# chrischoy/DeepGlobalRegistration

Hardware: AMD Instinct MI355X
Metric: pair registrations/sec (FCGF x2 + 1-NN + 6-D inlier net + gate + weighted Procrustes + SE(3) refinement) (higher is better)
Workload: dtype f32 results via 2 x f16 split operands (3 f16 MFMA products per MAC, f32 accumulate); k = 1 convs, kNN re-evaluation and registration in exact f32, SVD in f64

## Files before the change

### deepglobalregistration_amd/csrc/conv.hip

```cpp
#include <stdlib.h>

#include <map>

#include "dgr_internal.h"
#include <algorithm>
#include "hash.h"
#include "split.h"

typedef float f32x16 __attribute__((ext_vector_type(16)));
typedef float f32x4 __attribute__((ext_vector_type(4)));
typedef _Float16 f16x4 __attribute__((ext_vector_type(4)));
typedef int i32x4 __attribute__((ext_vector_type(4)));
typedef unsigned int u32x2 __attribute__((ext_vector_type(2)));
typedef unsigned int u32x4 __attribute__((ext_vector_type(4)));

struct ConvKArgs {
  const float *in;
  float *out;
  float *y;
  const float *shift;
  const float *w;
  const int32_t *pair_in, *pair_out, *tile_ptr, *rule_ptr, *n_rows_dev;
  const int4 *tile_desc;
  int in_ld, out_ld, in_relu, y_ld;
// ... 104 lines not shown
    float *dst = As + (q & 1) * TM * LDA;
#pragma unroll
    for (int i = 0; i < NCH; ++i) {
      const int ch = tid + i * THREADS;
      f32x4 v = G[i];
      if (a.in_relu) { v.x = fmaxf(v.x, 0.f); v.y = fmaxf(v.y, 0.f); v.z = fmaxf(v.z, 0.f); v.w = fmaxf(v.w, 0.f); }
      const bool ok = (g_ok >> i) & 1u;
      v.x = ok ? v.x : 0.f;
      v.y = ok ? v.y : 0.f;
      v.z = ok ? v.z : 0.f;
      v.w = ok ? v.w : 0.f;
      *reinterpret_cast<f32x4 *>(dst + (ch / C4K) * LDA + (ch % C4K) * 4) = v;
    }
  };

  {
    const int i0 = load_idx(0), i1 = load_idx(1), i2 = load_idx(2);
    if (tid < TM) { idxbuf[tid] = i0; idxbuf[TM + tid] = i1; idxbuf[2 * TM + tid] = i2; }
  }
  int next_pub = 3;
  int idx_reg = load_idx(3);
  int k, pstart, count;
  locate(0, k, pstart, count);
  f32x4 b[RING][NB];
  {
    const f32x4 *w0 = reinterpret_cast<const f32x4 *>(a.w) + ((int64_t)k * S * NBLK + wn * NB) * 64 + lane;
#pragma unroll
    for (int r = 0; r < RING - 1; ++r)
      if (r < S) {
#pragma unroll
        for (int j = 0; j < NB; ++j) b[r][j] = w0[((int64_t)r * NBLK + j) * 64];
      }
  }
  __syncthreads();
  gather(0);
  land(0);
  if (1 < NQ) gather(1);
  __syncthreads();

  f32x16 acc[MB][NB];
  for (int q = 0; q < NQ; ++q) {
    const int h = q % PPT;
    if (q + 1 < NQ) land(q + 1);
    if (q + 2 < NQ) gather(q + 2);
    if ((q + 3) / PPT >= next_pub && next_pub < n_my) {
      if (tid < TM) idxbuf[(next_pub & 3) * TM + tid] = idx_reg;
      ++next_pub;
      idx_reg = load_idx(next_pub);
    }
    if (h == 0) {
#pragma unroll
      for (int i = 0; i < MB; ++i)
#pragma unroll
        for (int j = 0; j < NB; ++j)
#pragma unroll
          for (int e = 0; e < 16; ++e) acc[i][j][e] = 0.f;
    }
    const f32x4 *wk = reinterpret_cast<const f32x4 *>(a.w) + ((int64_t)k * S * NBLK + wn * NB) * 64 + lane;
    const float *arow = As + (q & 1) * TM * LDA + (32 * wm * MB + (lane & 31)) * LDA + 4 * (lane >> 5);
    const int s0 = h * SK;
#pragma unroll
    for (int s = 0; s < SK; ++s) {
      if (s0 + s + RING - 1 < S) {
#pragma unroll
        for (int j = 0; j < NB; ++j) b[(s + RING - 1) % RING][j] = wk[((int64_t)(s0 + s + RING - 1) * NBLK + j) * 64];
      }
      __builtin_amdgcn_sched_barrier(0);
      f32x4 av[MB];
#pragma unroll
      for (int i = 0; i < MB; ++i) av[i] = *reinterpret_cast<const f32x4 *>(arow + i * 32 * LDA + s * 8);
#pragma unroll
      for (int c = 0; c < 4; ++c)
#pragma unroll
        for (int i = 0; i < MB; ++i)
#pragma unroll
          for (int j = 0; j < NB; ++j)
            acc[i][j] = __builtin_amdgcn_mfma_f32_32x32x2f32(b[s % RING][j][c], av[i][c], acc[i][j], 0, 0, 0);
    }
    if (h == PPT - 1) {
      const int pst = pstart, cnt = count;
      const int i_next = q / PPT + 1;
      if (i_next < n_my) {
        locate(i_next, k, pstart, count);
        const f32x4 *w1 = reinterpret_cast<const f32x4 *>(a.w) + ((int64_t)k * S * NBLK + wn * NB) * 64 + lane;
#pragma unroll
        for (int r = 0; r < RING - 1; ++r)
          if (r < S) {
#pragma unroll
            for (int j = 0; j < NB; ++j) b[r][j] = w1[((int64_t)r * NBLK + j) * 64];
          }
      }
#pragma unroll
      for (int i = 0; i < MB; ++i) {
        const int r = 32 * (wm * MB + i) + (lane & 31);
        if (identity && a.l2_normalize) {
          float ss = 0.f;
#pragma unroll
          for (int g = 0; g < 4; ++g)
#pragma unroll
            for (int u = 0; u < 4; ++u) {
              const int col = 8 * g + 4 * (lane >> 5) + u;
              float v = acc[i][0][4 * g + u] + ((a.shift && col < a.cout) ? a.shift[col] : 0.f);
              if (col >= a.cout) v = 0.f;
              acc[i][0][4 * g + u] = v;
              ss += v * v;
            }
          ss += __shfl_xor(ss, 32, 64);
          const float den = sqrtf(ss) + 1e-8f;
#pragma unroll
          for (int e = 0; e < 16; ++e) acc[i][0][e] = acc[i][0][e] / den;
        }
        if (r < cnt) {
          float *dst = identity ? a.out + (int64_t)(pst + r) * a.out_ld : a.y + (int64_t)(pst + r) * a.y_ld;
#pragma unroll
          for (int j = 0; j < NB; ++j) {
#pragma unroll
            for (int g = 0; g < 4; ++g) {
              const int col = 32 * (wn * NB + j) + 8 * g + 4 * (lane >> 5);
              f32x4 v = {acc[i][j][4 * g], acc[i][j][4 * g + 1], acc[i][j][4 * g + 2], acc[i][j][4 * g + 3]};
              if (identity) {
                if (col + 3 < a.cout && (a.out_ld & 3) == 0) {
                  if (a.shift && !a.l2_normalize) v += *reinterpret_cast<const f32x4 *>(a.shift + col);
                  *reinterpret_cast<f32x4 *>(dst + col) = v;
                } else {
#pragma unroll
                  for (int u = 0; u < 4; ++u)
                    if (col + u < a.cout) dst[col + u] = v[u] + ((a.shift && !a.l2_normalize) ? a.shift[col + u] : 0.f);
                }
              } else if (col < a.cout) {
                *reinterpret_cast<f32x4 *>(dst + col) = v;
              }
            }
          }
        }
      }
    }
    __syncthreads();
  }
}

template <int CP, int WM, int WN, int MB, int NB, bool VEC>
static int launch_v2(const ConvKArgs &ka, int64_t tile_bound, int num_cus, hipStream_t stream) {
  constexpr int THREADS = 64 * WM * WN;
  constexpr int CKL = conv_phase_width(CP, MB * NB);
  const size_t lds_bytes = (size_t)2 * DGR_TILE_M * (CKL + 4) * sizeof(float) + 4 * DGR_TILE_M * sizeof(int);
  static int per_cu = 0;
  if (per_cu == 0) {
    DGR_HIP_CHECK(hipFuncSetAttribute((const void *)sparse_conv_mfma_v2<CP, WM, WN, MB, NB, VEC>,
                                      hipFuncAttributeMaxDynamicSharedMemorySize, 160 * 1024));
    int n = 0;
    DGR_HIP_CHECK(hipOccupancyMaxActiveBlocksPerMultiprocessor(&n, sparse_conv_mfma_v2<CP, WM, WN, MB, NB, VEC>,
                                                               THREADS, lds_bytes));
    per_cu = n < 1 ? 1 : (n > 2048 / THREADS ? 2048 / THREADS : n);
  }
  int64_t grid = (int64_t)num_cus * per_cu;
  if (tile_bound < grid) grid = tile_bound;
  grid = (grid + 7) / 8 * 8;
  if (grid < 8) grid = 8;
  sparse_conv_mfma_v2<CP, WM, WN, MB, NB, VEC><<<(int)grid, THREADS, lds_bytes, stream>>>(ka);
  DGR_LAUNCH_CHECK();
  return DGR_OK;
}

template <int CP, int NBLK>
__global__ void __launch_bounds__(256) identity_conv_kernel(ConvKArgs a) {
  constexpr int S = CP / 8;
  const int lane = threadIdx.x & 63;
  const int n_rows = *a.n_rows_dev;
  const int n_tiles = (n_rows + 31) >> 5;
  const int wave_id = (int)((blockIdx.x * blockDim.x + threadIdx.x) >> 6), n_waves = (int)((gridDim.x * blockDim.x) >> 6);
  f32x4 w[S][NBLK];
  {
    const f32x4 *wp = reinterpret_cast<const f32x4 *>(a.w) + lane;
#pragma unroll
    for (int s = 0; s < S; ++s)
#pragma unroll
      for (int j = 0; j < NBLK; ++j) w[s][j] = wp[(s * NBLK + j) * 64];
  }
  const int relu_lo = a.in_relu ? 0 : (int)0x80000000;
  auto request = [&](int t, f32x4 (&x)[S]) {
    const int64_t row = min((int64_t)t * 32 + (lane & 31), (int64_t)n_rows - 1);
    const float *src = a.in + row * a.in_ld + 4 * (lane >> 5);
#pragma unroll
    for (int s = 0; s < S; ++s) x[s] = *reinterpret_cast<const f32x4 *>(src + 8 * s);
  };
  f32x4 xa[S], xb[S];
  auto tile = [&](int t, f32x4 (&x)[S]) {
    f32x16 acc[NBLK];
#pragma unroll
    for (int j = 0; j < NBLK; ++j)
#pragma unroll
      for (int e = 0; e < 16; ++e) acc[j][e] = 0.f;
#pragma unroll
    for (int s = 0; s < S; ++s) {
      i32x4 v = __builtin_bit_cast(i32x4, x[s]);
      v.x = max(v.x, relu_lo); v.y = max(v.y, relu_lo); v.z = max(v.z, relu_lo); v.w = max(v.w, relu_lo);
      const f32x4 xv = __builtin_bit_cast(f32x4, v);
#pragma unroll
      for (int c = 0; c < 4; ++c)
#pragma unroll
        for (int j = 0; j < NBLK; ++j) acc[j] = __builtin_amdgcn_mfma_f32_32x32x2f32(w[s][j][c], xv[c], acc[j], 0, 0, 0);
    }
    const int64_t row = (int64_t)t * 32 + (lane & 31);
    if (a.l2_normalize) {
      float ss = 0.f;
#pragma unroll
      for (int g = 0; g < 4; ++g)
#pragma unroll
        for (int u = 0; u < 4; ++u) {
          const int col = 8 * g + 4 * (lane >> 5) + u;
          float v = acc[0][4 * g + u] + ((a.shift && col < a.cout) ? a.shift[col] : 0.f);
          if (col >= a.cout) v = 0.f;
          acc[0][4 * g + u] = v;
          ss += v * v;
        }
      ss += __shfl_xor(ss, 32, 64);
      const float den = sqrtf(ss) + 1e-8f;
#pragma unroll
      for (int e = 0; e < 16; ++e) acc[0][e] = acc[0][e] / den;
    }
    if (row < n_rows) {
      float *dst = a.out + row * a.out_ld;
#pragma unroll
      for (int j = 0; j < NBLK; ++j)
#pragma unroll
        for (int g = 0; g < 4; ++g) {
          const int col = 32 * j + 8 * g + 4 * (lane >> 5);
          f32x4 v = {acc[j][4 * g], acc[j][4 * g + 1], acc[j][4 * g + 2], acc[j][4 * g + 3]};
          if (col + 3 < a.cout && (a.out_ld & 3) == 0) {
            if (a.shift && !a.l2_normalize) v += *reinterpret_cast<const f32x4 *>(a.shift + col);
            *reinterpret_cast<f32x4 *>(dst + col) = v;
          } else {
#pragma unroll
            for (int u = 0; u < 4; ++u)
              if (col + u < a.cout) dst[col + u] = v[u] + ((a.shift && !a.l2_normalize) ? a.shift[col + u] : 0.f);
          }
        }
    }
  };
  int t = wave_id;
  if (t < n_tiles) request(t, xa);
  for (; t < n_tiles; t += 2 * n_waves) {
    const int t1 = t + n_waves;
    if (t1 < n_tiles) request(t1, xb);
    tile(t, xa);
    if (t1 < n_tiles) {
      if (t1 + n_waves < n_tiles) request(t1 + n_waves, xa);
      tile(t1, xb);
    }
  }
}

template <int CP, int NBLK>
static int launch_identity(const ConvKArgs &ka, int64_t rows_cap, int num_cus, hipStream_t stream) {
  int64_t blocks = std::min<int64_t>((int64_t)num_cus * 4, std::max<int64_t>(1, dgr_ceil_div(rows_cap, 32 * 4 * 2)));
  identity_conv_kernel<CP, NBLK><<<(int)blocks, 256, 0, stream>>>(ka);
  DGR_LAUNCH_CHECK();
  return DGR_OK;
}

int dgr_conv_launch(const DgrConvLaunch &a, int num_cus, hipStream_t stream, const char **kernel_name) {
  ConvKArgs ka;
  ka.in = a.in; ka.out = a.out; ka.w = a.w; ka.y = a.y; ka.shift = a.shift; ka.y_ld = a.cout;
  ka.pair_in = a.pair_in; ka.pair_out = a.pair_out; ka.tile_ptr = a.tile_ptr; ka.rule_ptr = a.rule_ptr;
  ka.n_rows_dev = a.n_rows_dev; ka.tile_desc = a.tile_desc;
  ka.in_ld = a.in_ld; ka.out_ld = a.out_ld; ka.in_relu = a.in_relu;
  ka.cin = a.cin; ka.cin_pad = a.cin_pad; ka.cout = a.cout; ka.K = a.K;
  ka.l2_normalize = a.l2_normalize;
  DGR_REQUIRE(!a.l2_normalize || (a.pair_in == nullptr && a.cout <= 32 && a.cout_pad == 32),
              "fused l2 normalisation needs an identity map and Cout <= 32 (got %d)", a.cout);
  DGR_REQUIRE(a.cin_pad % 8 == 0 && a.cin_pad >= a.cin && a.cin_pad <= 256, "bad cin_pad %d", a.cin_pad);
  const int64_t tile_bound = a.tile_bound > 0 ? a.tile_bound : (int64_t)num_cus * 4;
  const bool vec = ((a.cin | a.in_ld) & 3) == 0;
  if (a.pair_in == nullptr && vec && a.cin == a.cin_pad && a.tile_bound > 0) {
#define DGR_ID(CPV, NBV)                                                                          \
  if (a.cin_pad == CPV && a.cout_pad == 32 * NBV) {                                               \
    if (kernel_name) *kernel_name = "identity_conv_kernel<" #CPV ", " #NBV ">";                   \
    return launch_identity<CPV, NBV>(ka, a.tile_bound * DGR_TILE_M, num_cus, stream);             \
  }
    DGR_ID(64, 1) DGR_ID(64, 2) DGR_ID(96, 2)
#undef DGR_ID
  }
#define DGR_V2(CPV, WMV, WNV, MBV, NBV)                                                                        \
  if (a.cin_pad == CPV) {                                                                                       \
    if (kernel_name)                                                                                            \
      *kernel_name = vec ? "sparse_conv_mfma_v2<" #CPV ", " #WMV ", " #WNV ", " #MBV ", " #NBV ", true>"        \
                         : "sparse_conv_mfma_v2<" #CPV ", " #WMV ", " #WNV ", " #MBV ", " #NBV ", false>";      \
    return vec ? launch_v2<CPV, WMV, WNV, MBV, NBV, true>(ka, tile_bound, num_cus, stream)                     \
               : launch_v2<CPV, WMV, WNV, MBV, NBV, false>(ka, tile_bound, num_cus, stream);                   \
  }
  switch (a.cout_pad) {
    case 32: DGR_V2(8, 2, 1, 1, 1) DGR_V2(32, 2, 1, 1, 1) DGR_V2(64, 2, 1, 1, 1) break;
    case 64: DGR_V2(32, 2, 2, 1, 1) DGR_V2(64, 2, 2, 1, 1) DGR_V2(96, 2, 2, 1, 1) DGR_V2(128, 2, 2, 1, 1)
             DGR_V2(256, 2, 2, 1, 1) break;
    case 128: DGR_V2(64, 1, 4, 2, 1) DGR_V2(128, 1, 4, 2, 1) DGR_V2(256, 1, 4, 2, 1) break;
    case 256: DGR_V2(128, 1, 4, 2, 2) DGR_V2(256, 1, 4, 2, 2) break;
    default: break;
  }
#undef DGR_V2
  dgr_set_error("sparse conv: no kernel instantiation for Cin (padded) %d -> Cout (padded) %d", a.cin_pad, a.cout_pad);
  return DGR_EINVAL;
}

template <int LPR, bool SPLIT>
__global__ void __launch_bounds__(256)
    reduce_rows_kernel(const float *__restrict__ y, int y_ld, const int32_t *__restrict__ ptr,
                       const int32_t *__restrict__ pos, const int32_t *n_dev, float *__restrict__ out, int out_ld,
                       const float *__restrict__ shift, const float *__restrict__ res, int res_ld, int res_relu,
                       unsigned char *__restrict__ planes, float *__restrict__ scale_out, int out_relu) {
  constexpr int ROWS = 256 / LPR;
  const int n = *n_dev;
  const int sub = threadIdx.x / LPR, c = (threadIdx.x % LPR) * 4;
  for (int64_t row = (int64_t)blockIdx.x * ROWS + sub; row < n; row += (int64_t)gridDim.x * ROWS) {
    f32x4 acc = shift ? *reinterpret_cast<const f32x4 *>(shift + c) : f32x4{0.f, 0.f, 0.f, 0.f};
    if (res) {
      f32x4 r = *reinterpret_cast<const f32x4 *>(res + row * res_ld + c);
      if (res_relu) { r.x = fmaxf(r.x, 0.f); r.y = fmaxf(r.y, 0.f); r.z = fmaxf(r.z, 0.f); r.w = fmaxf(r.w, 0.f); }
      acc += r;
    }
    int j = ptr[row];
    const int end = ptr[row + 1];
    for (; j + 8 <= end; j += 8) {
      int p[8];
#pragma unroll
      for (int u = 0; u < 8; ++u) p[u] = pos[j + u];
      f32x4 v[8];
#pragma unroll
      for (int u = 0; u < 8; ++u) v[u] = dgr_y_load<LPR == 64>(y + (int64_t)p[u] * y_ld + c);
#pragma unroll
      for (int u = 0; u < 8; ++u) acc += v[u];
    }
    for (; j + 4 <= end; j += 4) {
      const int p0 = pos[j], p1 = pos[j + 1], p2 = pos[j + 2], p3 = pos[j + 3];
      const f32x4 v0 = dgr_y_load<LPR == 64>(y + (int64_t)p0 * y_ld + c);
      const f32x4 v1 = dgr_y_load<LPR == 64>(y + (int64_t)p1 * y_ld + c);
      const f32x4 v2 = dgr_y_load<LPR == 64>(y + (int64_t)p2 * y_ld + c);
      const f32x4 v3 = dgr_y_load<LPR == 64>(y + (int64_t)p3 * y_ld + c);
      acc += v0; acc += v1; acc += v2; acc += v3;
    }
    for (; j < end; ++j) acc += dgr_y_load<LPR == 64>(y + (int64_t)pos[j] * y_ld + c);
    if (!SPLIT || out) *reinterpret_cast<f32x4 *>(out + row * out_ld + c) = acc;
    if constexpr (SPLIT) {
      const int lo = out_relu ? 0 : (int)0x80000000;
      const i32x4 ab = __builtin_bit_cast(i32x4, acc);
      int xb[4];
      uint32_t mx = 0;
#pragma unroll
      for (int u = 0; u < 4; ++u) {
        xb[u] = max(ab[u], lo);
        mx = max(mx, (uint32_t)xb[u] & 0x7fffffffu);
      }
#pragma unroll
      for (int d = LPR / 2; d >= 1; d >>= 1) mx = max(mx, (uint32_t)__shfl_xor((int)mx, d, 64));
      const float sx = dgr_row_scale_of(mx);
      f16x4 h, m;
#pragma unroll
      for (int u = 0; u < 4; ++u) {
        _Float16 hh, mm;
        dgr_split2(__builtin_bit_cast(float, xb[u]), sx, hh, mm);
        h[u] = hh; m[u] = mm;
      }
      const bool odd = threadIdx.x & 1;
      const u32x2 hb = __builtin_bit_cast(u32x2, h), mb = __builtin_bit_cast(u32x2, m);
      const u32x2 give = odd ? hb : mb;
      u32x2 got;
      got.x = (uint32_t)__shfl_xor((int)give.x, 1, 64);
      got.y = (uint32_t)__shfl_xor((int)give.y, 1, 64);
      const u32x4 st = odd ? u32x4{got.x, got.y, mb.x, mb.y} : u32x4{hb.x, hb.y, got.x, got.y};
      unsigned char *dst = planes + row * (LPR * 16);
      *reinterpret_cast<u32x4 *>(dst + dgr_split_row_offset(c & ~7, odd ? 1 : 0)) = st;
      if (c == 0) scale_out[row] = sx;
    }
  }
}

int dgr_reduce_rows(const float *y, int cout, const int32_t *ptr, const int32_t *pos, const int32_t *n_dev,
                    int64_t n_cap, float *out, int out_ld, const float *shift, const float *res, int res_ld,
                    int res_relu, hipStream_t stream, const DgrSplitRows *split, int out_relu) {
  DGR_REQUIRE((out_ld & 3) == 0 && (res == nullptr || (res_ld & 3) == 0), "reduce_rows: row strides must be x4");
  DGR_REQUIRE(out || split, "reduce_rows: no output");
  DGR_REQUIRE(!split || (split->planes && split->scale && split->channels == cout && cout % 64 == 0),
              "reduce_rows: split rows need planes, scales and the layer's width (a multiple of 64)");
  const int lpr = cout / 4;
  const int64_t want = std::max<int64_t>(1, dgr_ceil_div(n_cap, 256 / lpr));
#define DGR_RR1(L, SP)                                                                                         \
  do {                                                                                                         \
    static int resident = 0;                                                                                   \
    if (resident == 0) {                                                                                       \
      int per_cu = 0, dev = 0, cus = 0;                                                                        \
      DGR_HIP_CHECK(hipOccupancyMaxActiveBlocksPerMultiprocessor(&per_cu, reduce_rows_kernel<L, SP>, 256, 0)); \
      DGR_HIP_CHECK(hipGetDevice(&dev));                                                                       \
      DGR_HIP_CHECK(hipDeviceGetAttribute(&cus, hipDeviceAttributeMultiprocessorCount, dev));                  \
      resident = (per_cu < 1 ? 1 : per_cu) * (cus < 1 ? 1 : cus);                                              \
    }                                                                                                          \
    const int64_t blocks = want > resident ? (int64_t)resident * std::min<int64_t>(4, want / resident) : want; \
    reduce_rows_kernel<L, SP><<<(int)blocks, 256, 0, stream>>>(y, cout, ptr, pos, n_dev, out, out_ld, shift,   \
                                                               res, res_ld, res_relu, split ? split->planes : nullptr, \
                                                               split ? split->scale : nullptr, out_relu);      \
  } while (0)
#define DGR_RR(L)                       \
  do {                                  \
    if (split) DGR_RR1(L, true);        \
    else DGR_RR1(L, false);             \
  } while (0)
  switch (cout) {
    case 32: DGR_RR1(8, false); break;
    case 64: DGR_RR(16); break;
    case 128: DGR_RR(32); break;
    case 256: DGR_RR(64); break;
    default:
      dgr_set_error("reduce_rows: unsupported width %d", cout);
      return DGR_EINVAL;
  }
#undef DGR_RR1
#undef DGR_RR
  DGR_LAUNCH_CHECK();
  return DGR_OK;
}

__global__ void __launch_bounds__(256)
    conv_small_cin_kernel(const float *__restrict__ in, int in_ld, int in_relu, int cin,
                          const float *__restrict__ w, const float *__restrict__ shift,
                          const int32_t *__restrict__ out_ptr, const int32_t *__restrict__ out_pos,
                          const int32_t *__restrict__ pair_in, const uint16_t *__restrict__ pair_k,
                          const int32_t *n_out_dev, float *__restrict__ out, int out_ld) {
  const int n = *n_out_dev;
  const int co = threadIdx.x & 31;
  for (int64_t o = (int64_t)blockIdx.x * 8 + (threadIdx.x >> 5); o < n; o += (int64_t)gridDim.x * 8) {
    float acc = shift ? shift[co] : 0.f;
    const int end = out_ptr[o + 1];
    int j = out_ptr[o];
    for (; j + 8 <= end; j += 8) {
      int pos[8], row[8], kk[8];
#pragma unroll
      for (int u = 0; u < 8; ++u) pos[u] = out_pos[j + u];
#pragma unroll
      for (int u = 0; u < 8; ++u) { row[u] = pair_in[pos[u]]; kk[u] = pair_k[pos[u]]; }
      float y[8];
#pragma unroll
      for (int u = 0; u < 8; ++u) {
        const float *wk = w + (int64_t)kk[u] * 256;
        float t = 0.f;
        for (int ci = 0; ci < cin; ++ci) {
          float x = in[(int64_t)row[u] * in_ld + ci];
          if (in_relu) x = fmaxf(x, 0.f);
          t = fmaf(x, wk[(32 * (ci >> 2) + co) * 4 + (ci & 3)], t);
        }
        y[u] = t;
      }
#pragma unroll
      for (int u = 0; u < 8; ++u) acc += y[u];
    }
    for (; j < end; ++j) {
      const int pos = out_pos[j];
      const int row = pair_in[pos];
      const float *wk = w + (int64_t)pair_k[pos] * 256;
      float y = 0.f;
      for (int ci = 0; ci < cin; ++ci) {
        float x = in[(int64_t)row * in_ld + ci];
        if (in_relu) x = fmaxf(x, 0.f);
        y = fmaf(x, wk[(32 * (ci >> 2) + co) * 4 + (ci & 3)], y);
      }
      acc += y;
    }
    out[o * out_ld + co] = acc;
  }
}

template <int CIN>
__global__ void __launch_bounds__(256)
    conv_small_cin_row_kernel(const float *__restrict__ in, int in_ld, int in_relu, const float *__restrict__ w,
                              const float *__restrict__ shift, const int32_t *__restrict__ out_ptr,
                              const int32_t *__restrict__ out_pos, const int32_t *__restrict__ pair_in,
                              const uint16_t *__restrict__ pair_k, const int32_t *n_out_dev, float *__restrict__ out,
                              int out_ld) {
  const int64_t o = (int64_t)blockIdx.x * blockDim.x + threadIdx.x;
  if (o >= *n_out_dev) return;
  float acc[32];
#pragma unroll
  for (int co = 0; co < 32; ++co) acc[co] = shift ? shift[co] : 0.f;
  const int end = out_ptr[o + 1];
  for (int j = out_ptr[o]; j < end; ++j) {
    const int pos = out_pos[j];
    const int row = pair_in[pos];
    const f32x4 *wk = reinterpret_cast<const f32x4 *>(w + (int64_t)pair_k[pos] * 256);
    float x[CIN];
#pragma unroll
    for (int ci = 0; ci < CIN; ++ci) {
      x[ci] = in[(int64_t)row * in_ld + ci];
      if (in_relu) x[ci] = fmaxf(x[ci], 0.f);
    }
#pragma unroll
    for (int co = 0; co < 32; ++co) {
      const f32x4 w0 = wk[co];
      float t = 0.f;
#pragma unroll
      for (int ci = 0; ci < (CIN < 4 ? CIN : 4); ++ci) t = fmaf(x[ci], w0[ci], t);
      if constexpr (CIN > 4) {
        const f32x4 w1 = wk[32 + co];
#pragma unroll
        for (int ci = 4; ci < CIN; ++ci) t = fmaf(x[ci], w1[ci - 4], t);
      }
      acc[co] += t;
    }
  }
  f32x4 *dst = reinterpret_cast<f32x4 *>(out + o * out_ld);
#pragma unroll
  for (int q = 0; q < 8; ++q) dst[q] = f32x4{acc[4 * q], acc[4 * q + 1], acc[4 * q + 2], acc[4 * q + 3]};
}

__global__ void __launch_bounds__(256)
    conv_cin6_quad_kernel(const float *__restrict__ in, int in_ld, int in_relu, const float *__restrict__ wq,
                          const float *__restrict__ shift, const int32_t *__restrict__ out_ptr,
                          const int32_t *__restrict__ out_pos, const int32_t *__restrict__ pair_in,
                          const uint16_t *__restrict__ pair_k, const int32_t *n_out_dev, float *__restrict__ out,
                          int out_ld) {
  const int64_t t = (int64_t)blockIdx.x * blockDim.x + threadIdx.x;
  const int64_t o = t >> 2;
  const int q = (int)(t & 3);
  if (o >= *n_out_dev) return;
  float acc[8];
#pragma unroll
  for (int e = 0; e < 8; ++e) acc[e] = shift ? shift[8 * q + e] : 0.f;
  const int end = out_ptr[o + 1];
  for (int j = out_ptr[o]; j < end; ++j) {
    const int pos = out_pos[j];
    const int row = pair_in[pos];
    const f32x4 *wk = reinterpret_cast<const f32x4 *>(wq + (int64_t)pair_k[pos] * 192) + q;
    float x[6];
#pragma unroll
    for (int ci = 0; ci < 6; ++ci) {
      x[ci] = in[(int64_t)row * in_ld + ci];
      if (in_relu) x[ci] = fmaxf(x[ci], 0.f);
    }
    float tt[8];
#pragma unroll
    for (int e = 0; e < 8; ++e) tt[e] = 0.f;
#pragma unroll
    for (int i = 0; i < 12; ++i) {
      const f32x4 wv = wk[4 * i];
#pragma unroll
      for (int e = 0; e < 4; ++e) tt[4 * (i & 1) + e] = fmaf(x[i >> 1], wv[e], tt[4 * (i & 1) + e]);
    }
#pragma unroll
    for (int e = 0; e < 8; ++e) acc[e] += tt[e];
  }
  f32x4 *dst = reinterpret_cast<f32x4 *>(out + o * out_ld + 8 * q);
  dst[0] = f32x4{acc[0], acc[1], acc[2], acc[3]};
  dst[1] = f32x4{acc[4], acc[5], acc[6], acc[7]};
}

int dgr_conv_small_cin(const float *in, int in_ld, int in_relu, int cin, const float *w_tiled, const float *w_quad,
                       const float *shift, const DgrKernelMap &km, const int32_t *n_out_dev, int64_t n_out_cap, float *out,
                       int out_ld, hipStream_t stream) {
  DGR_REQUIRE(cin >= 1 && cin <= 8, "small-Cin conv: cin=%d", cin);
  if ((out_ld & 3) == 0 && cin == 6 && w_quad) {
    conv_cin6_quad_kernel<<<(int)dgr_ceil_div(n_out_cap * 4, 256), 256, 0, stream>>>(
        in, in_ld, in_relu, w_quad, shift, km.out_ptr, km.out_pos, km.pair_in, km.pair_k, n_out_dev, out, out_ld);
    DGR_LAUNCH_CHECK();
    return DGR_OK;
  }
  if ((out_ld & 3) == 0 && (cin == 6 || cin == 1)) {
    const int rb = (int)dgr_ceil_div(n_out_cap, 256);
    if (cin == 6)
      conv_small_cin_row_kernel<6><<<rb, 256, 0, stream>>>(in, in_ld, in_relu, w_tiled, shift, km.out_ptr, km.out_pos, km.pair_in,
                                                         km.pair_k, n_out_dev, out, out_ld);
    else
      conv_small_cin_row_kernel<1><<<rb, 256, 0, stream>>>(in, in_ld, in_relu, w_tiled, shift, km.out_ptr, km.out_pos, km.pair_in,
                                                         km.pair_k, n_out_dev, out, out_ld);
    DGR_LAUNCH_CHECK();
    return DGR_OK;
  }
  int64_t blocks = dgr_ceil_div(n_out_cap, 8);
  if (blocks > 16384) blocks = 16384;
  conv_small_cin_kernel<<<(int)blocks, 256, 0, stream>>>(in, in_ld, in_relu, cin, w_tiled, shift, km.out_ptr,
                                                          km.out_pos, km.pair_in, km.pair_k, n_out_dev, out, out_ld);
  DGR_LAUNCH_CHECK();
  return DGR_OK;
}

__global__ void __launch_bounds__(256)
    conv1_probe_kernel(const int32_t *__restrict__ coords, const int32_t *n_dev, const int32_t *__restrict__ table,
                       uint32_t mask, int ks, const float *__restrict__ in, int in_ld, int cin,
                       const float *__restrict__ w, const float *__restrict__ shift, float *__restrict__ out,
                       int out_ld, int32_t *pair_count, const int32_t *skip_flag, uint32_t *__restrict__ out_amax) {
  if (skip_flag && *skip_flag) return;
  const int n = *n_dev;
  const int lane = threadIdx.x & 63;
  const int co = lane & 31;
  const int K = ks * ks * ks, half = ks >> 1;
  const int64_t wave_id = ((int64_t)blockIdx.x * blockDim.x + threadIdx.x) >> 6;
  const int64_t n_waves = ((int64_t)gridDim.x * blockDim.x) >> 6;
  int pairs = 0;
  for (int64_t o = wave_id; o < n; o += n_waves) {
    const int32_t b = coords[o * 4], x = coords[o * 4 + 1], y = coords[o * 4 + 2], z = coords[o * 4 + 3];
    float acc = shift ? shift[co] : 0.f;
    for (int k0 = 0; k0 < K; k0 += 64) {
      const int k = k0 + lane;
      int hit = -1;
      if (k < K) {
        int32_t q[4] = {b, x + (k % ks) - half, y + ((k / ks) % ks) - half, z + (k / (ks * ks)) - half};
        hit = dgr_lookup<4>(table, mask, coords, q);
      }
      float xv[8];
      const int64_t hrow = (int64_t)max(hit, 0) * in_ld;
#pragma unroll
      for (int ci = 0; ci < 8; ++ci) {
        xv[ci] = 0.f;
        if (ci < cin) xv[ci] = in[hrow + ci];
      }
      unsigned long long live = __ballot(hit >= 0);
      pairs += __popcll(live);
      while (live) {
        const int src = __ffsll((long long)live) - 1;
        live &= live - 1;
        float t = 0.f;
#pragma unroll
        for (int ci = 0; ci < 8; ++ci) {
          if (ci < cin) {
            const float xs = __builtin_bit_cast(float, __builtin_amdgcn_readlane(__builtin_bit_cast(int, xv[ci]), src));
            const float wv = w[(int64_t)(k0 + src) * 256 + (32 * (ci >> 2) + co) * 4 + (ci & 3)];
            t = fmaf(xs, wv, t);
          }
        }
        acc += t;
      }
    }
    if (lane < 32) out[o * out_ld + co] = acc;
    if (out_amax) {
      uint32_t mx = __builtin_bit_cast(uint32_t, acc) & 0x7fffffffu;
#pragma unroll
      for (int d = 16; d >= 1; d >>= 1) mx = max(mx, (uint32_t)__shfl_xor((int)mx, d, 64));
      if (lane == 0) atomicMax(out_amax + o, mx);
    }
  }
  if (lane == 0 && pair_count) atomicAdd(pair_count, pairs);
}

constexpr int GRID_MAXB = 64;
struct DgrGridMeta {
  int32_t ok, bad;
  long long total;
  int32_t mn[GRID_MAXB][3], mx[GRID_MAXB][3], dim[GRID_MAXB][3];
  long long base[GRID_MAXB];
};

__global__ void grid_init_kernel(DgrGridMeta *m, int32_t *pair_count) {
  const int b = threadIdx.x;
  if (b == 0) { m->ok = 0; m->bad = 0; m->total = 0; if (pair_count) *pair_count = 0; }
  if (b < GRID_MAXB) {
    for (int d = 0; d < 3; ++d) { m->mn[b][d] = INT32_MAX; m->mx[b][d] = INT32_MIN; m->dim[b][d] = 0; }
    m->base[b] = 0;
  }
}

__global__ void __launch_bounds__(256)
    grid_bbox_kernel(const int32_t *__restrict__ coords, const int32_t *n_dev, DgrGridMeta *m) {
  __shared__ int32_t red[6][256 / 64];
  __shared__ int32_t b0s, mixed;
  const int n = *n_dev;
  const int64_t o = (int64_t)blockIdx.x * 256 + threadIdx.x;
  if ((int64_t)blockIdx.x * 256 >= n) return;
  const bool live = o < n;
  const int4 c = live ? *reinterpret_cast<const int4 *>(coords + o * 4) : make_int4(0, 0, 0, 0);
  if (threadIdx.x == 0) { b0s = c.x; mixed = 0; }
  __syncthreads();
  if (live && c.x != b0s) mixed = 1;
  if (live && (c.x < 0 || c.x >= GRID_MAXB)) m->bad = 1;
  __syncthreads();
  auto wave_minmax = [&](bool mine, int32_t (&v)[6]) {
    v[0] = mine ? c.y : INT32_MAX; v[1] = mine ? c.z : INT32_MAX; v[2] = mine ? c.w : INT32_MAX;
    v[3] = mine ? c.y : INT32_MIN; v[4] = mine ? c.z : INT32_MIN; v[5] = mine ? c.w : INT32_MIN;
#pragma unroll
    for (int s = 32; s >= 1; s >>= 1) {
#pragma unroll
      for (int d = 0; d < 3; ++d) {
        v[d] = min(v[d], __shfl_xor(v[d], s, 64));
        v[3 + d] = max(v[3 + d], __shfl_xor(v[3 + d], s, 64));
      }
    }
  };
  int32_t v[6];
  if (mixed) {
    const bool ok = live && c.x >= 0 && c.x < GRID_MAXB;
    unsigned long long todo = __ballot(ok);
    while (todo) {
      const int leader = __ffsll((long long)todo) - 1;
      const int b = __shfl(c.x, leader, 64);
      const bool mine = ok && c.x == b;
      wave_minmax(mine, v);
      if ((int)(threadIdx.x & 63) == leader) {
#pragma unroll
        for (int d = 0; d < 3; ++d) { atomicMin(&m->mn[b][d], v[d]); atomicMax(&m->mx[b][d], v[3 + d]); }
      }
      todo &= ~__ballot(mine);
    }
    return;
  }
  wave_minmax(live, v);
  if ((threadIdx.x & 63) == 0)
    for (int d = 0; d < 6; ++d) red[d][threadIdx.x >> 6] = v[d];
  __syncthreads();
  if (threadIdx.x < 6) {
    const int d = threadIdx.x;
    int32_t r = red[d][0];
    for (int w = 1; w < 4; ++w) r = d < 3 ? min(r, red[d][w]) : max(r, red[d][w]);
    const int b = b0s;
    if (b >= 0 && b < GRID_MAXB) {
      if (d < 3) atomicMin(&m->mn[b][d], r); else atomicMax(&m->mx[b][d - 3], r);
    }
  }
}

__global__ void grid_layout_kernel(DgrGridMeta *m, int pad, long long cap) {
  static_assert(GRID_MAXB == 64, "one lane per batch element");
  const int b = threadIdx.x;
  long long vol = 0;
  if (m->mx[b][0] >= m->mn[b][0]) {
    vol = 1;
    for (int d = 0; d < 3; ++d) {
      const long long e = (long long)m->mx[b][d] - m->mn[b][d] + 1 + 2 * pad;
      m->dim[b][d] = (int32_t)(e < (1ll << 30) ? e : (1ll << 30));
      vol = (vol <= cap && e <= cap) ? vol * e : cap + 1;
    }
  }
  long long incl = vol;
#pragma unroll
  for (int s = 1; s < 64; s <<= 1) {
    const long long up = __shfl_up(incl, s, 64);
    if (b >= s) incl += up;
  }
  m->base[b] = incl - vol;
  const long long total = __shfl(incl, 63, 64);
  if (b == 0) {
    m->total = total <= cap ? total : cap + 1;
    m->ok = (!m->bad && total <= cap) ? 1 : 0;
  }
}

__global__ void grid_clear_kernel(const DgrGridMeta *m, int32_t *__restrict__ cells) {
  if (!m->ok) return;
  const long long total = m->total;
  for (long long i = ((long long)blockIdx.x * blockDim.x + threadIdx.x) * 4; i < total; i += (long long)gridDim.x * blockDim.x * 4)
    *reinterpret_cast<int4 *>(cells + i) = make_int4(-1, -1, -1, -1);
}

__device__ __forceinline__ long long grid_cell(const DgrGridMeta *m, int b, int x, int y, int z, int pad) {
  const long long dx = m->dim[b][0], dy = m->dim[b][1];
  return m->base[b] + ((long long)(z - m->mn[b][2] + pad) * dy + (y - m->mn[b][1] + pad)) * dx + (x - m->mn[b][0] + pad);
}

constexpr uint32_t GRID_EMPTY = 0xffffffffu;
__global__ void grid_fill_kernel(const int32_t *__restrict__ coords, const int32_t *n_dev, const DgrGridMeta *m, int pad,
                                 int32_t *__restrict__ cells, const float *__restrict__ values, int values_ld) {
  if (!m->ok) return;
  const int64_t o = (int64_t)blockIdx.x * blockDim.x + threadIdx.x;
  if (o >= *n_dev) return;
  const int4 c = *reinterpret_cast<const int4 *>(coords + o * 4);
  cells[grid_cell(m, c.x, c.y, c.z, c.w, pad)] = values ? __builtin_bit_cast(int32_t, values[o * values_ld]) : (int32_t)o;
}

constexpr int C1_MAXK = 343;
__global__ void __launch_bounds__(256)
    conv1_grid_kernel(const int32_t *__restrict__ coords, const int32_t *n_dev, const DgrGridMeta *__restrict__ m,
                      const int32_t *__restrict__ cells, int ks, const float *__restrict__ in, int in_ld, int cin,
                      const float *__restrict__ w, const float *__restrict__ shift, float *__restrict__ out,
                      int out_ld, int32_t *pair_count, uint32_t *__restrict__ out_amax) {
  __shared__ int2 lists[256 / 64][2][C1_MAXK + 1];
  if (!m->ok) return;
  const int n = *n_dev;
  const int lane = threadIdx.x & 63, wv = threadIdx.x >> 6;
  const int half = ks >> 1, ks2 = ks * ks;
  const int ky = lane % ks, kz = lane / ks;
  const int vsel = lane >> 5, co = lane & 31;
  const unsigned long long below = (1ull << lane) - 1ull;
  const int64_t wave_id = ((int64_t)blockIdx.x * blockDim.x + threadIdx.x) >> 6;
  const int64_t n_waves = ((int64_t)gridDim.x * blockDim.x) >> 6;
  int pairs = 0;
  for (int64_t o0 = wave_id * 2; o0 < n; o0 += n_waves * 2) {
    int nh[2] = {0, 0};
#pragma unroll
    for (int v = 0; v < 2; ++v) {
      const int64_t o = o0 + v;
      if (o >= n) break;
      const int4 c = *reinterpret_cast<const int4 *>(coords + o * 4);
      int hit[7];
#pragma unroll
      for (int kx = 0; kx < 7; ++kx) hit[kx] = -1;
      if (lane < ks2) {
        const long long c0 = grid_cell(m, c.x, c.y - half, c.z + ky - half, c.w + kz - half, half);
#pragma unroll
        for (int kx = 0; kx < 7; ++kx)
          if (kx < ks) hit[kx] = cells[c0 + kx];
      }
      unsigned long long mk[7];
      int before = 0;
#pragma unroll
      for (int kx = 0; kx < 7; ++kx) {
        mk[kx] = __ballot(hit[kx] >= 0);
        before += __popcll(mk[kx] & below);
        nh[v] += __popcll(mk[kx]);
      }
      int r = before;
#pragma unroll
      for (int kx = 0; kx < 7; ++kx)
        if (hit[kx] >= 0) lists[wv][v][r++] = make_int2(kx + ks * lane, hit[kx]);
    }
    __builtin_amdgcn_fence(__ATOMIC_RELEASE, "wavefront");
    __builtin_amdgcn_wave_barrier();
    __builtin_amdgcn_fence(__ATOMIC_ACQUIRE, "wavefront");
    pairs += nh[0] + nh[1];
    const int my_n = vsel ? nh[1] : nh[0];
    const int trips = max(nh[0], nh[1]);
    float acc = shift ? shift[co] : 0.f;
    for (int r0 = 0; r0 < trips; r0 += 8) {
      int2 e[8];
      float t[8];
#pragma unroll
      for (int u = 0; u < 8; ++u) {
        e[u] = (r0 + u < my_n) ? lists[wv][vsel][r0 + u] : make_int2(0, 0);
        t[u] = 0.f;
      }
      for (int ci = 0; ci < cin; ++ci) {
        float xs[8], ws[8];
        const int wofs = (32 * (ci >> 2) + co) * 4 + (ci & 3);
#pragma unroll
        for (int u = 0; u < 8; ++u) {
          xs[u] = in[(int64_t)e[u].y * in_ld + ci];
          ws[u] = w[(int64_t)e[u].x * 256 + wofs];
        }
#pragma unroll
        for (int u = 0; u < 8; ++u) t[u] = fmaf(xs[u], ws[u], t[u]);
      }
#pragma unroll
      for (int u = 0; u < 8; ++u) acc = (r0 + u < my_n) ? acc + t[u] : acc;
    }
    const int64_t o = o0 + vsel;
    if (o < n) out[o * out_ld + co] = acc;
    if (out_amax) {
      uint32_t mx = o < n ? (__builtin_bit_cast(uint32_t, acc) & 0x7fffffffu) : 0u;
#pragma unroll
      for (int d = 16; d >= 1; d >>= 1) mx = max(mx, (uint32_t)__shfl_xor((int)mx, d, 64));
      if (co == 0 && o < n) atomicMax(out_amax + o, mx);
    }
    __builtin_amdgcn_fence(__ATOMIC_RELEASE, "wavefront");
    __builtin_amdgcn_wave_barrier();
  }
  if (lane == 0 && pair_count) atomicAdd(pair_count, pairs);
}

template <int KS>
__global__ void __launch_bounds__(256)
    conv1_grid_mfma(const int32_t *__restrict__ coords, const int32_t *n_dev, const DgrGridMeta *__restrict__ m,
                    const int32_t *__restrict__ cells, const float *__restrict__ wt, const float *__restrict__ shift,
                    float *__restrict__ out, int out_ld, int32_t *pair_count, uint32_t *__restrict__ out_amax) {
  constexpr int KS2 = KS * KS, HALF = KS / 2;
  constexpr int RS = (KS2 + 3) / 4 * 4;
  constexpr int LDG = RS + 1;
// ... 181 lines not shown
```

### deepglobalregistration_amd/csrc/conv_wide.hip

```cpp
#include <stdlib.h>

#include <type_traits>

#include "dgr_internal.h"
#include "split.h"

typedef _Float16 f16x8 __attribute__((ext_vector_type(8)));
typedef float f32x16 __attribute__((ext_vector_type(16)));
typedef float f32x4 __attribute__((ext_vector_type(4)));

struct ConvWideArgs {
  const unsigned char *planes;
  const float *row_scale;
  float *y;
  const uint4 *wb;
  int64_t piece_stride;
  const int32_t *pair_in, *tile_ptr;
  int cout, K;
  float w_unscale;
  unsigned long long *clk;
};

#define DGR_LDS_PTR(off) ((__attribute__((address_space(3))) void *)(lds + (off)))
#define DGR_GLOBAL_PTR(p) ((const __attribute__((address_space(1))) void *)(p))

template <int N>
__device__ __forceinline__ void dgr_wait_vmcnt() {
  static_assert(N >= 0 && N < 64, "vmcnt is a 6-bit counter");
  asm volatile("s_waitcnt vmcnt(%0)" ::"n"(N) : "memory");
}
__device__ __forceinline__ void dgr_phase_barrier() {
  asm volatile("s_waitcnt lgkmcnt(0)\n\ts_barrier" ::: "memory");
}

__host__ __device__ constexpr int dgr_wide_passes(int h, int npass, int nsp) {
  return h < nsp ? npass / nsp + (h < npass % nsp ? 1 : 0) : 0;
}
__host__ __device__ constexpr int dgr_wide_pass_base(int h, int npass, int nsp) {
  int b = 0;
  for (int i = 0; i < h; ++i) b += dgr_wide_passes(i, npass, nsp);
  return b;
}

template <int CP, int NB, int WM>
__global__ void __launch_bounds__(512, 1) sparse_conv_wide_f16x2(ConvWideArgs a, const int4 *__restrict__ tdesc) {
  constexpr int NCW = 4;
  constexpr int NP = 2, MB = 2 / WM, WN = NCW / WM, PW = 4, TM = 64, CK = 64, SK = CK / 16;
  static_assert(WM == 1 || WM == 2, "row split of the compute waves");
  static_assert(TM == DGR_TILE_M && CP % CK == 0, "shape");
  constexpr int PPT = CP / CK, S = CP / 16, NBLK = NB * WN, COUT = 32 * NBLK;
  static_assert(PPT == 1 || PPT == 2 || PPT == 4, "a round of NSET phases is a whole number of tiles");
  constexpr int ROWB = 4 * CP;
  constexpr int NBUF = 3;
  constexpr int NSET = 4;
  constexpr int LEAD = NSET + 2;
  constexpr int BUFB = TM * 256;
  constexpr int RING = 16;
  constexpr int AH_I = 8, AH_S = 4;
  static_assert(RING >= 2 * AH_I && AH_I > LEAD && AH_S >= 3 && AH_S < AH_I, "ring distances");
  constexpr int WD = NB >= 2 ? 2 : 4;
  static_assert(SK % WD == 0, "the weight ring turns a whole number of times per phase (static register indexing)");
  constexpr int LDS_ST = COUT + 4;
  constexpr int NSTG = PPT == 1 ? 2 : 1;
  constexpr int HB = PPT / 2;
  constexpr int RPH = TM / PPT;
  constexpr int PD = 2;
  constexpr int PTH = 64 * (PW - PD);
  constexpr int CPR = COUT / 4;
  constexpr int RPP = PTH / CPR;
  constexpr int NPS = RPH / RPP;
  static_assert(RPH % RPP == 0, "store passes");
  constexpr int OFF_STAGE = NBUF * BUFB;
  constexpr int OFF_IDX = OFF_STAGE + NSTG * TM * LDS_ST * 4;
  constexpr int OFF_SC = OFF_IDX + RING * TM * 4;
  constexpr int LDS_BYTES = OFF_SC + RING * TM * 4;
  static_assert(LDS_BYTES <= 160 * 1024, "LDS budget");
  __shared__ __attribute__((aligned(16))) unsigned char lds[LDS_BYTES];

  const int tid = threadIdx.x;
  const int lane = tid & 63;
  const int wave = __builtin_amdgcn_readfirstlane(tid >> 6);
  if (a.clk && tid == 0) atomicMin(a.clk, (unsigned long long)wall_clock64());
  const int T = a.tile_ptr[a.K];
  const int per = (T + 7) >> 3;
  const int xcd = blockIdx.x & 7;
  const int t_end = min(T, (xcd + 1) * per);
  const int nj = gridDim.x >> 3;
  const int t_first = xcd * per + (blockIdx.x >> 3);
  if (t_first >= t_end) return;
  const int n_my = (t_end - t_first + nj - 1) / nj;
  const int n_loop = n_my + 2;
  auto desc = [&](int i) -> int4 { return tdesc[t_first + min(max(i, 0), n_my - 1) * nj]; };
  auto stage_of = [&](int t) -> float * {
    return reinterpret_cast<float *>(lds + OFF_STAGE) + (NSTG == 2 ? (t & 1) : 0) * TM * LDS_ST;
  };

  if (wave >= NCW) {
    const int pw = wave - NCW;
    if (pw < PD) {
      constexpr int RW = TM / PD, NI = RW / 4;
      f32x4 G[NSET][NI];
      const unsigned char *rb[NI];
      auto row_bases = [&](int i) {
        const int *idx = reinterpret_cast<const int *>(lds + OFF_IDX + (i & (RING - 1)) * TM * 4);
#pragma unroll
        for (int jj = 0; jj < NI; ++jj) {
          const int r = RW * pw + 4 * jj + (lane >> 4);
          rb[jj] = a.planes + (int64_t)idx[r] * ROWB + 16 * ((lane & 15) ^ (r & 15));
        }
      };
      auto request = [&](int p, f32x4 *Gs) {
        if (p % PPT == 0) row_bases(p / PPT);
#pragma unroll
        for (int jj = 0; jj < NI; ++jj) Gs[jj] = *reinterpret_cast<const f32x4 *>(rb[jj] + (p % PPT) * 256);
      };
      auto land = [&](int p, const f32x4 *Gs) {
        unsigned char *dst = lds + (p % NBUF) * BUFB + (NI * pw) * 1024 + lane * 16;
#pragma unroll
        for (int jj = 0; jj < NI; ++jj) *reinterpret_cast<f32x4 *>(dst + jj * 1024) = Gs[jj];
      };
      int *ring_i = reinterpret_cast<int *>(lds + OFF_IDX);
      float *ring_s = reinterpret_cast<float *>(lds + OFF_SC);
      auto load_idx = [&](int i) -> int {
        const int4 d = desc(i);
        return a.pair_in[d.y + min(lane, d.z - 1)];
      };
#pragma unroll
      for (int i = 0; i < AH_I - 1; ++i) ring_i[i * TM + lane] = load_idx(i);
#pragma unroll
      for (int i = 0; i < AH_S - 1; ++i) ring_s[i * TM + lane] = a.row_scale[ring_i[i * TM + lane]];
      int idx_reg = load_idx(AH_I - 1);
      float sc_reg = a.row_scale[ring_i[(AH_S - 1) * TM + lane]];
      auto rings = [&](int t) {
        ring_i[((t + AH_I - 1) & (RING - 1)) * TM + lane] = idx_reg;
        ring_s[((t + AH_S - 1) & (RING - 1)) * TM + lane] = sc_reg;
        idx_reg = load_idx(t + AH_I);
        sc_reg = a.row_scale[ring_i[((t + AH_S) & (RING - 1)) * TM + lane]];
      };
      dgr_phase_barrier();
#pragma unroll
      for (int j = 0; j < NSET; ++j) request(j, G[j]);
      land(0, G[0]); request(NSET, G[0]);
      land(1, G[1]); request(NSET + 1, G[1]);
      dgr_phase_barrier();
      auto phase = [&](int q, f32x4 *Gs) {
        if (q % PPT == 0) rings(q / PPT);
        land(q + 2, Gs);
        request(q + LEAD, Gs);
        dgr_phase_barrier();
      };
      for (int q = 0; q < n_loop * PPT; q += NSET) {
        phase(q, G[2]);
        if (q + 1 < n_loop * PPT) phase(q + 1, G[3]);
        if (q + 2 < n_loop * PPT) phase(q + 2, G[0]);
        if (q + 3 < n_loop * PPT) phase(q + 3, G[1]);
      }
      return;
    }
    const int ptid = tid - 64 * (NCW + PD);
    auto store_rows = [&](int u, int r0) {
      if (u < 0 || u >= n_my) return;
      const int4 d = desc(u);
      const float *sc = reinterpret_cast<const float *>(lds + OFF_SC + (u & (RING - 1)) * TM * 4);
      const float *st = stage_of(u);
      const int c4 = (ptid % CPR) * 4;
      f32x4 v[NPS];
#pragma unroll
      for (int i = 0; i < NPS; ++i) {
        const int r = r0 + i * RPP + ptid / CPR;
        v[i] = *reinterpret_cast<const f32x4 *>(st + r * LDS_ST + c4);
        v[i] *= dgr_inv_pow2(sc[r]) * a.w_unscale;
      }
#pragma unroll
      for (int i = 0; i < NPS; ++i) {
        const int r = r0 + i * RPP + ptid / CPR;
        if (r < d.z) __builtin_nontemporal_store(v[i], reinterpret_cast<f32x4 *>(a.y + (int64_t)(d.y + r) * COUT + c4));
      }
    };
    dgr_phase_barrier();
    dgr_phase_barrier();
    auto sphase = [&](int t, auto hc) {
      constexpr int h = decltype(hc)::value;
      if constexpr (h == 0) store_rows(t - 2, (PPT - 1) * RPH);
      else store_rows(t - 1, (h - 1) * RPH);
      dgr_phase_barrier();
    };
    for (int t = 0; t < n_loop; ++t) {
      sphase(t, std::integral_constant<int, 0>());
      if constexpr (PPT > 1) sphase(t, std::integral_constant<int, 1>());
      if constexpr (PPT > 2) {
        sphase(t, std::integral_constant<int, 2>());
        sphase(t, std::integral_constant<int, 3>());
      }
    }
    if (a.clk && lane == 0) {
      dgr_wait_vmcnt<0>();
      atomicMax(a.clk + 1, (unsigned long long)wall_clock64());
    }
    return;
  }

  const int wn = wave % WN, wm = wave / WN;
  int4 dc = desc(0), dn = desc(1);
  uint4 w[WD][NB][NP];
  auto wload = [&](int k, int s, uint4 (*ws)[NP]) {
    const uint4 *p = a.wb + ((int64_t)(k * S + s) * NBLK + wn * NB) * 64 + lane;
#pragma unroll
    for (int j = 0; j < NB; ++j)
#pragma unroll
      for (int pc = 0; pc < NP; ++pc) ws[j][pc] = p[(int64_t)pc * a.piece_stride + j * 64];
  };
#pragma unroll
  for (int g = 0; g < WD - 1; ++g) wload(dc.x, g % S, w[g]);
  dgr_phase_barrier();
  dgr_phase_barrier();
  uint4 op[2][MB][NP];
  const int lofs0 = (32 * MB * wm + (lane & 31)) * 256 + 16 * ((lane >> 5) ^ (lane & 15));
  auto oload = [&](int b, int s, uint4 (*o)[NP]) {
    const unsigned char *p = lds + b * BUFB + (lofs0 ^ (32 * s));
    const unsigned char *pm = lds + b * BUFB + (lofs0 ^ (32 * s) ^ 128);
#pragma unroll
    for (int i = 0; i < MB; ++i) {
      o[i][0] = *reinterpret_cast<const uint4 *>(p + i * 32 * 256);
      o[i][1] = *reinterpret_cast<const uint4 *>(pm + i * 32 * 256);
    }
  };
  oload(0, 0, op[0]);
  int buf = 0;
  constexpr int NPC = (4 * NB + SK - 1) / SK;
  auto stage_pieces = [&](float *st, const f32x16 (&ac)[MB][NB], int i, int s) {
    float *dst = st + (32 * (MB * wm + i) + (lane & 31)) * LDS_ST;
#pragma unroll
    for (int u = 0; u < NPC; ++u) {
      const int wq = s * NPC + u, j = wq / 4, g = wq % 4;
      if (wq < 4 * NB) {
        const int col = 32 * (wn * NB + j) + 8 * g + 4 * (lane >> 5);
        *reinterpret_cast<f32x4 *>(dst + col) = f32x4{ac[i][j][4 * g], ac[i][j][4 * g + 1], ac[i][j][4 * g + 2], ac[i][j][4 * g + 3]};
      }
    }
  };
  auto ctile = [&](int t, f32x16 (&ac)[MB][NB], const f32x16 (&ad)[MB][NB]) {
    const bool stage_prev = t >= 1 && t <= n_my;
    float *st = stage_of(t - 1);
#pragma unroll
    for (int h = 0; h < PPT; ++h) {
      if (h == 0) {
#pragma unroll
        for (int i = 0; i < MB; ++i)
#pragma unroll
          for (int j = 0; j < NB; ++j)
#pragma unroll
            for (int e = 0; e < 16; ++e) ac[i][j][e] = 0.f;
      }
      const int nbuf = buf == NBUF - 1 ? 0 : buf + 1;
      const int s0 = h * SK;
#pragma unroll
      for (int s = 0; s < SK; ++s) {
        {
          const int sg = s0 + s + WD - 1;
          wload(sg < S ? dc.x : dn.x, sg < S ? sg : sg - S, w[(s + WD - 1) % WD]);
        }
        if (s + 1 < SK) oload(buf, s + 1, op[(s + 1) & 1]);
        else oload(nbuf, 0, op[0]);
        __builtin_amdgcn_sched_barrier(0);
        uint4 (*wc)[NP] = w[s % WD];
        uint4 (*oc)[NP] = op[s & 1];
#define DGR_WIDE_TERM(WP, OP)                                                                                         \
  _Pragma("unroll") for (int i = 0; i < MB; ++i) _Pragma("unroll") for (int j = 0; j < NB; ++j)                       \
      ac[i][j] = __builtin_amdgcn_mfma_f32_32x32x16_f16(__builtin_bit_cast(f16x8, wc[j][WP]),                          \
                                                        __builtin_bit_cast(f16x8, oc[i][OP]), ac[i][j], 0, 0, 0);
        DGR_WIDE_TERM(1, 0)
        DGR_WIDE_TERM(0, 1)
        DGR_WIDE_TERM(0, 0)
#undef DGR_WIDE_TERM
        if (stage_prev) {
          if (h == 0) stage_pieces(st, ad, 0, s);
          if constexpr (MB > 1) {
            if (h == HB) stage_pieces(st, ad, 1, s);
          }
        }
      }
      if (h == PPT - 1) {
        dc = dn;
        dn = desc(t + 2);
      }
      buf = nbuf;
      dgr_phase_barrier();
    }
  };
  f32x16 accA[MB][NB], accB[MB][NB];
  for (int t = 0; t < n_loop; t += 2) {
    ctile(t, accA, accB);
    if (t + 1 < n_loop) ctile(t + 1, accB, accA);
  }
  if (a.clk && lane == 0) atomicMax(a.clk + 1, (unsigned long long)wall_clock64());
}

template <int CP, int NB, int WM>
static int launch_wide(const ConvWideArgs &ka, const int4 *tile_desc, int64_t tile_bound, int num_cus, hipStream_t stream) {
  int64_t grid = num_cus;
  if (tile_bound < grid) grid = tile_bound;
  grid = (grid + 7) / 8 * 8;
  if (grid < 8) grid = 8;
  sparse_conv_wide_f16x2<CP, NB, WM><<<(int)grid, 512, 0, stream>>>(ka, tile_desc);
  DGR_LAUNCH_CHECK();
  return DGR_OK;
}

bool dgr_conv_wide_supported(int cin_pad, int cin, int cout) {
  if (cin != cin_pad) return false;
  return (cout == 64 && cin == 64) || (cout == 128 && (cin == 64 || cin == 128 || cin == 256)) ||
         (cout == 256 && (cin == 128 || cin == 256));
}

int dgr_conv_wide_launch(const DgrConvLaunch &a, const DgrSplitRows &in, const void *wb, int64_t piece_stride,
                         float w_unscale, int num_cus, hipStream_t stream, const char **kernel_name) {
  DGR_REQUIRE(a.pair_in && wb && in.planes && in.scale && dgr_conv_wide_supported(a.cin_pad, a.cin, a.cout),
              "wide conv: unsupported layer (Cin %d, Cout %d) or no split input rows", a.cin, a.cout);
  DGR_REQUIRE(in.channels == a.cin, "wide conv: the split rows have %d channels, the layer %d", in.channels, a.cin);
  DGR_REQUIRE(a.y, "wide conv: no product-row buffer");
  ConvWideArgs ka;
  ka.planes = in.planes; ka.row_scale = in.scale; ka.y = a.y;
  ka.wb = static_cast<const uint4 *>(wb); ka.piece_stride = piece_stride;
  ka.pair_in = a.pair_in; ka.tile_ptr = a.tile_ptr; ka.cout = a.cout; ka.K = a.K; ka.w_unscale = w_unscale;
  ka.clk = a.clk;
  const int64_t tile_bound = a.tile_bound > 0 ? a.tile_bound : (int64_t)num_cus * 4;
#define DGR_WIDE(CPV, NBV, WMV)                                                                 \
  do {                                                                                          \
    if (kernel_name) *kernel_name = "sparse_conv_wide_f16x2<" #CPV ", " #NBV ", " #WMV ">";     \
    return launch_wide<CPV, NBV, WMV>(ka, a.tile_desc, tile_bound, num_cus, stream);            \
  } while (0)
  if (a.cout == 64 && a.cin == 64) DGR_WIDE(64, 1, 2);
  if (a.cout == 128 && a.cin == 64) DGR_WIDE(64, 1, 1);
  if (a.cout == 128 && a.cin == 128) DGR_WIDE(128, 1, 1);
  if (a.cout == 128 && a.cin == 256) DGR_WIDE(256, 1, 1);
  if (a.cout == 256 && a.cin == 128) DGR_WIDE(128, 2, 1);
  if (a.cout == 256 && a.cin == 256) DGR_WIDE(256, 2, 1);
#undef DGR_WIDE
  dgr_set_error("wide conv: no kernel for Cin %d, Cout %d", a.cin, a.cout);
  return DGR_EINVAL;
}

typedef int i32x4 __attribute__((ext_vector_type(4)));
typedef _Float16 f16x4 __attribute__((ext_vector_type(4)));

template <int LPR, bool SPLIT>
__global__ void __launch_bounds__(256) row_scale_kernel(const float *__restrict__ in, int in_ld, int cin, int relu,
                                                        const int32_t *__restrict__ n_dev, float *__restrict__ out,
                                                        unsigned char *__restrict__ planes, uint32_t *__restrict__ amax_out) {
  constexpr int RPW = 64 / LPR;
  const int lane = threadIdx.x & 63;
  const int sub = lane / LPR, l = lane % LPR;
  const int n = *n_dev;
  const int relu_lo = relu ? 0 : (int)0x80000000;
  const int64_t stride = (int64_t)gridDim.x * 4 * RPW;
  for (int64_t r0 = ((int64_t)blockIdx.x * 4 + (threadIdx.x >> 6)) * RPW; r0 < n; r0 += stride) {
    const int64_t r = r0 + sub;
    uint32_t mx = 0;
    if (r < n) {
      const float *row = in + r * in_ld;
      for (int c = l * 4; c < cin; c += LPR * 4) {
        const i32x4 v = __builtin_bit_cast(i32x4, *reinterpret_cast<const f32x4 *>(row + c));
#pragma unroll
        for (int u = 0; u < 4; ++u) mx = max(mx, (uint32_t)max(v[u], relu_lo) & 0x7fffffffu);
      }
    }
#pragma unroll
    for (int d = LPR / 2; d >= 1; d >>= 1) mx = max(mx, (uint32_t)__shfl_xor((int)mx, d, 64));
    const float sx = dgr_row_scale_of(mx);
    if (l == 0 && r < n) {
      if (out) out[r] = sx;
      if (amax_out) amax_out[r] = mx;
    }
    if constexpr (SPLIT) {
      if (r < n) {
        const float *row = in + r * in_ld;
        unsigned char *dst = planes + r * 4 * cin;
        for (int c = l * 4; c < cin; c += LPR * 4) {
          const i32x4 v = __builtin_bit_cast(i32x4, *reinterpret_cast<const f32x4 *>(row + c));
          f16x4 h, m;
#pragma unroll
          for (int u = 0; u < 4; ++u) {
            _Float16 hh, mm;
            dgr_split2(__builtin_bit_cast(float, max(v[u], relu_lo)), sx, hh, mm);
            h[u] = hh; m[u] = mm;
          }
          *reinterpret_cast<f16x4 *>(dst + dgr_split_row_offset(c, 0)) = h;
          *reinterpret_cast<f16x4 *>(dst + dgr_split_row_offset(c, 1)) = m;
        }
      }
    }
  }
}

static int row_scale_launch(const float *in, int in_ld, int cin, int relu, const int32_t *n_dev, int64_t n_cap, float *out,
                            unsigned char *planes, uint32_t *amax_out, hipStream_t stream) {
  DGR_REQUIRE((cin & 3) == 0 && (in_ld & 3) == 0 && cin >= 4, "row scale: channel count and row stride must be multiples of 4");
  const int lpr = cin >= 256 ? 64 : cin >= 128 ? 32 : cin >= 64 ? 16 : cin >= 32 ? 8 : 4;
  int64_t grid = dgr_ceil_div(n_cap, 4 * (64 / lpr));
  if (grid > 4096) grid = 4096;
  if (grid < 1) grid = 1;
#define DGR_RS(L)                                                                                                   \
  do {                                                                                                              \
    if (planes) row_scale_kernel<L, true><<<(int)grid, 256, 0, stream>>>(in, in_ld, cin, relu, n_dev, out, planes, amax_out); \
    else row_scale_kernel<L, false><<<(int)grid, 256, 0, stream>>>(in, in_ld, cin, relu, n_dev, out, nullptr, amax_out);      \
  } while (0)
  switch (lpr) {
    case 64: DGR_RS(64); break;
    case 32: DGR_RS(32); break;
    case 16: DGR_RS(16); break;
    case 8: DGR_RS(8); break;
    default: DGR_RS(4); break;
  }
#undef DGR_RS
  DGR_LAUNCH_CHECK();
  return DGR_OK;
}

int dgr_row_amax(const float *in, int in_ld, int cin, int relu, const int32_t *n_dev, int64_t n_cap, uint32_t *out,
                 hipStream_t stream) {
  return row_scale_launch(in, in_ld, cin, relu, n_dev, n_cap, nullptr, nullptr, out, stream);
}

int dgr_split_rows(const float *in, int in_ld, int relu, const int32_t *n_dev, int64_t n_cap, const DgrSplitRows &out,
                   hipStream_t stream) {
  DGR_REQUIRE(out.planes && out.scale && out.channels % 64 == 0, "split rows: need planes, scales and a multiple of 64 channels");
  return row_scale_launch(in, in_ld, out.channels, relu, n_dev, n_cap, out.scale, out.planes, nullptr, stream);
}
```

### deepglobalregistration_amd/csrc/dgr_internal.h

```cpp
#pragma once
#include <hip/hip_runtime.h>
#include <stdint.h>
#include <stdio.h>
#include <stdlib.h>
#include <string>
#include <vector>

#include "../../include/dgr_hip.h"

void dgr_set_error(const char *fmt, ...);

#define DGR_HIP_CHECK(expr)                                                                  \
  do {                                                                                       \
    hipError_t _e = (expr);                                                                  \
    if (_e != hipSuccess) {                                                                  \
      dgr_set_error("%s:%d: %s failed: %s", __FILE__, __LINE__, #expr, hipGetErrorString(_e)); \
      return DGR_EHIP;                                                                       \
    }                                                                                        \
  } while (0)

#define DGR_CHECK(expr)          \
  do {                           \
    int _r = (expr);             \
    if (_r != DGR_OK) return _r; \
  } while (0)

#define DGR_REQUIRE(cond, ...)     \
  do {                             \
    if (!(cond)) {                 \
      dgr_set_error(__VA_ARGS__);  \
      return DGR_EINVAL;           \
    }                              \
  } while (0)

#define DGR_LAUNCH_CHECK() DGR_HIP_CHECK(hipGetLastError())

inline bool dgr_exact_f32() {
  static const bool on = getenv("DGR_EXACT_F32") != nullptr;
  return on;
}

struct DgrArena {
  struct Chunk {
    char *base;
    size_t size;
  };
  std::vector<Chunk> chunks;
  size_t cur = 0;
  size_t offset = 0;
  size_t high_water = 0, used_total = 0;
  uint64_t generation = 0;

  struct Mark {
    size_t cur, offset, used_total;
  };
  Mark mark() const { return {cur, offset, used_total}; }
  void rewind(const Mark &m) { cur = m.cur; offset = m.offset; used_total = m.used_total; }
  void *alloc(size_t bytes);
  int reset();
  void release();
  size_t reserved() const;
  template <typename T>
  T *get(size_t n) {
    return static_cast<T *>(alloc(n * sizeof(T)));
  }
};

#define DGR_ALLOC(ptr, arena, T, n)                       \
  do {                                                    \
    (ptr) = (arena).get<T>((size_t)(n) > 0 ? (size_t)(n) : 1); \
    if (!(ptr)) return DGR_ENOMEM;                        \
  } while (0)

constexpr int DGR_TILE_M = 64;

struct DgrCoordMap {
  int32_t *coords = nullptr;
  int32_t *n_dev = nullptr;
  int64_t n_cap = 0;
  int ts = 1;
  int32_t *table = nullptr;
  uint32_t table_mask = 0;
  int32_t *canon = nullptr;
};

struct DgrHalfBuckets {
  int32_t *bkeys = nullptr;
  int32_t *table = nullptr;
  uint32_t mask = 0;
  int32_t *start = nullptr;
  int4 *second = nullptr;
  bool built = false;
};

struct DgrKernelMap {
  int K = 0;
  int32_t *rule_ptr = nullptr;
  int32_t *tile_ptr = nullptr;
  int4 *tile_desc = nullptr;
  int64_t tile_cap = 0;
  int32_t *pair_in = nullptr;
  int32_t *pair_out = nullptr;
  int32_t *out_ptr = nullptr, *out_pos = nullptr;
  uint16_t *pair_k = nullptr;
  int32_t *in_ptr = nullptr, *in_pos = nullptr;
  int64_t pair_cap = 0;
  bool built = false;
};

constexpr int DGR_OS_ROWS = 64;
struct DgrNbrTable {
  int32_t *nbr = nullptr;
  int64_t n_pad = 0;
  int K = 27;
  bool built = false;
  int32_t *perm = nullptr, *cls_count = nullptr;
  int64_t cls_cap = 0;
};

struct DgrMapSet {
  int D = 3, nc = 4, conv1_ks = 3;
  bool use_nbr = false;
  DgrNbrTable nsame[4];
  DgrNbrTable ndown[3];
  DgrNbrTable nup[3];
  DgrCoordMap cm[4];
  DgrHalfBuckets hb[4];
  DgrKernelMap same[4];
  DgrKernelMap conv1;
  DgrKernelMap down[3];
  int32_t *overflow = nullptr;
};

int dgr_build_maps(DgrArena &arena, const int32_t *coords, int64_t N, int D, int conv1_ks,
                   DgrMapSet *ms, hipStream_t stream, bool skip_conv1_map = false, bool lean = false,
                   bool nbr_tables = false);
int dgr_nbr_counts(const DgrNbrTable &t, const int32_t *n_out_dev, int64_t counts[27]);
int dgr_conv1_probe(DgrArena &arena, const DgrCoordMap &cm, int ks, const float *in, int in_ld, int cin,
                    const float *w_tiled, const float *shift, float *out, int out_ld, int32_t *pair_count,
                    hipStream_t stream, const float *w_compact = nullptr, const char **kernel_name = nullptr,
                    uint32_t *out_amax = nullptr);
int dgr_unique_rows(DgrArena &arena, const int32_t *keys, int64_t n, int nc, int32_t *first_flag,
                    int32_t *rank, int32_t *n_unique_dev, int32_t **table_out, uint32_t *mask_out,
                    hipStream_t stream);
int dgr_exclusive_scan_i32(DgrArena &arena, const int32_t *in, int32_t *out, int64_t n,
                           int32_t *total_out, hipStream_t stream);
constexpr int DGR_SCAN_MAX = 24;
int dgr_exclusive_scan_multi(DgrArena &arena, int count, const int32_t *const *in, int32_t *const *out, const int64_t *n,
                             int32_t *const *total_out, hipStream_t stream);

struct DgrConvLaunch {
  const float *in;
  int in_ld;
  int in_relu;
  float *out;
  int out_ld;
  float *y;
  const float *shift;
  const float *w;
  int cin, cin_pad, cout, cout_pad, K;
  const int32_t *pair_in, *pair_out, *tile_ptr, *rule_ptr;
  const int4 *tile_desc;
  const int32_t *n_rows_dev;
  int64_t tile_bound;
  int l2_normalize = 0;
  unsigned long long *clk = nullptr;
};
int dgr_conv_launch(const DgrConvLaunch &a, int num_cus, hipStream_t stream, const char **kernel_name = nullptr);
struct DgrSplitRows {
  unsigned char *planes = nullptr;
  float *scale = nullptr;
  int channels = 0;
};
bool dgr_conv_wide_supported(int cin_pad, int cin, int cout);
int dgr_conv_wide_launch(const DgrConvLaunch &a, const DgrSplitRows &in, const void *wb, int64_t piece_stride,
                         float w_unscale, int num_cus, hipStream_t stream, const char **kernel_name = nullptr);
int dgr_row_amax(const float *in, int in_ld, int cin, int relu, const int32_t *n_dev, int64_t n_cap, uint32_t *out,
                 hipStream_t stream);
int dgr_split_rows(const float *in, int in_ld, int relu, const int32_t *n_dev, int64_t n_cap, const DgrSplitRows &out,
                   hipStream_t stream);
int dgr_reduce_rows(const float *y, int cout, const int32_t *ptr, const int32_t *pos, const int32_t *n_dev,
                    int64_t n_cap, float *out, int out_ld, const float *shift, const float *res, int res_ld,
                    int res_relu, hipStream_t stream, const DgrSplitRows *split = nullptr, int out_relu = 0);
int dgr_conv_small_cin(const float *in, int in_ld, int in_relu, int cin, const float *w_tiled, const float *w_quad,
                       const float *shift, const DgrKernelMap &km, const int32_t *n_out_dev, int64_t n_out_cap, float *out,
                       int out_ld, hipStream_t stream);
struct DgrConvOsLaunch {
  const float *in; int in_ld, in_relu;
  float *out; int out_ld, out_relu;
  const float *w16, *shift;
  const void *wb3; int64_t piece_stride;
  const void *wbd = nullptr;
  const uint32_t *row_amax = nullptr; float w_unscale = 1.f;
  uint32_t *out_amax = nullptr, *out_amax2 = nullptr;
  int64_t n_in_cap = 0;
  const float *res; int res_ld, res_relu;
  int rows_per_block;
  int phase_channels = 64;
  const DgrNbrTable *nbr;
  const int32_t *n_out_dev;
  int64_t n_out_cap;
  int cin, cin_pad, cout;
  bool dense = false;
  bool up = false;
  const unsigned char *in_dsplit = nullptr;
  unsigned char *out_dsplit = nullptr;
};
int dgr_conv_os_launch(const DgrConvOsLaunch &a, hipStream_t stream, const char **kernel_name = nullptr);
bool dgr_conv_dense_supported(int cin, int cin_pad, int cout);
int dgr_conv_dense_launch(const DgrConvOsLaunch &a, hipStream_t stream, const char **kernel_name = nullptr);
bool dgr_conv_up_supported(int cin, int cin_pad, int cout);
int dgr_conv_up_launch(const DgrConvOsLaunch &a, hipStream_t stream, const char **kernel_name = nullptr);
int dgr_l2_normalize_rows(const float *in, int in_ld, float *out, int out_ld, int c, int relu,
                          const int32_t *n_dev, int64_t n_cap, hipStream_t stream);

struct DgrBatchOutputs {
  const void *ptr[5] = {nullptr, nullptr, nullptr, nullptr, nullptr};
  int64_t numel[5] = {0, 0, 0, 0, 0};
  uint64_t generation = 0;
};

struct DgrEventPool {
  std::vector<hipEvent_t> ev;
  size_t used = 0;
  hipEvent_t next();
  void release();
};

struct dgr_ctx {
  int device = 0;
  int num_cus = 256;
  DgrArena arena;
  bool profiling = false;
  float stage_ms[9] = {0, 0, 0, 0, 0, 0, 0, 0, 0};
  int64_t conv_launches = 0;
  DgrBatchOutputs last;
  std::vector<double> last_T64;
  DgrEventPool events;
  std::vector<std::pair<hipEvent_t, hipEvent_t>> conv_spans, gemm_spans, map3_spans, map6_spans;
  std::vector<float> conv_span_ms, gemm_span_ms;
  std::vector<unsigned long long *> conv_clks;
  std::vector<float> conv_clk_us;
  std::vector<const char *> conv_kinds;
  int32_t *flag_dev = nullptr;
  hipEvent_t wait_ev = nullptr;
  long last_wait_ns = 0;
  double batch_ns_per_row = 0;
  unsigned char *pin = nullptr;
  size_t pin_bytes = 0;
  hipStream_t part_stream = nullptr;
  int all_cus = 256;
};

int dgr_ctx_pinned(dgr_ctx *ctx, size_t bytes, unsigned char **out);
int dgr_flag_error(int32_t flag);

int dgr_ctx_wait(dgr_ctx *ctx, hipStream_t stream, long predicted_ns = 0);

int dgr_resunet_forward_impl(dgr_ctx *ctx, dgr_net *net, const int32_t *coords, const float *feats,
                             int64_t N, float *out, hipStream_t stream);
int dgr_ctx_collect_profile(dgr_ctx *ctx);
void dgr_ctx_begin_profile(dgr_ctx *ctx);

int dgr_knn1_batch_impl(dgr_ctx *ctx, const float *F0, const int64_t *off0, const float *F1, const int64_t *off1,
                        int npairs, int C, int squared, int64_t *idx_out, float *dist_out, hipStream_t stream);
int dgr_knn1_impl(dgr_ctx *ctx, const float *F0, int64_t N0, const float *F1, int64_t N1, int C,
                  int squared, int64_t *idx_out, float *dist_out, hipStream_t stream);
int dgr_inlier_inputs_impl(const int32_t *coords0, const float *xyz0, int64_t N0,
                           const int32_t *coords1, const float *xyz1, const int64_t *idx1,
                           int feature_type, int32_t *coords6, float *feats, hipStream_t stream);
int dgr_icp_impl(dgr_ctx *ctx, const float *src, int64_t N0, const float *dst, int64_t N1, double max_dist,
                 const double *T_init, int max_iter, double rel_fitness, double rel_rmse, double *T_out,
                 double *stats_out, hipStream_t stream);
int dgr_ransac_impl(dgr_ctx *ctx, const float *X, const float *Y, int64_t N, double max_dist, int64_t num_hypotheses,
                    uint32_t seed, double *T_out, double *stats_out, hipStream_t stream);
struct DgrIcpJob {
  const float *src = nullptr, *dst = nullptr;
  int64_t N0 = 0, N1 = 0;
  double max_dist = 0;
  int nblocks = 0;
  void *st = nullptr;
  double *P = nullptr, *sorted = nullptr, *partial = nullptr;
  int32_t ncell = 0;
  double host_state[64];
};
int dgr_icp_begin(dgr_ctx *ctx, const float *src, int64_t N0, const float *dst, int64_t N1, double max_dist,
                  const double *T_init_dev , DgrIcpJob *job, hipStream_t stream);
int dgr_icp_run(dgr_ctx *ctx, DgrIcpJob *job, int max_iter, double rel_fitness, double rel_rmse, hipStream_t stream);
void dgr_icp_finish(const DgrIcpJob *job, double *T_out, double *stats_out);
constexpr int DGR_RANSAC_RESULT_DOUBLES = 19;
int dgr_ransac_begin(dgr_ctx *ctx, const float *X, const float *Y, int64_t N, double max_dist, int64_t num_hypotheses,
                     uint32_t seed, double **result_dev, hipStream_t stream);
struct DgrRegResult {
  float R[9];
  float t[3];
  float loss;
  float wsum;
  int32_t iterations;
  int32_t break_count;
  int32_t status;
  int32_t pad;
};
static inline int64_t dgr_ceil_div(int64_t a, int64_t b) { return (a + b - 1) / b; }
static inline uint32_t dgr_next_pow2(uint64_t v) {
  uint32_t p = 1;
  while (p < v) p <<= 1;
  return p;
}
```

### deepglobalregistration_amd/csrc/kmap.hip

```cpp
#include <string.h>

#include <algorithm>

#include "dgr_internal.h"
#include "hash.h"

constexpr int KM_THREADS = 256;

template <int D>
__device__ __forceinline__ void offset_of(int k, int ks, int ts, int32_t *delta) {
  const int half = ks >> 1;
#pragma unroll
  for (int d = 0; d < D; ++d) {
    delta[d] = ((k % ks) - half) * ts;
    k /= ks;
  }
}

template <int D>
__device__ __forceinline__ int probe(const int32_t *__restrict__ out_coords, int64_t o,
                                     const int32_t *delta, const int32_t *__restrict__ in_coords,
                                     const int32_t *__restrict__ in_table, uint32_t in_mask) {
  constexpr int NC = D + 1;
  int32_t q[NC];
  q[0] = out_coords[o * NC];
#pragma unroll
  for (int d = 0; d < D; ++d) q[1 + d] = out_coords[o * NC + 1 + d] + delta[d];
  return dgr_lookup<NC>(in_table, in_mask, in_coords, q);
}

template <int D>
__global__ void __launch_bounds__(KM_THREADS)
    kmap_search(const int32_t *__restrict__ out_coords, const int32_t *n_out_dev,
                const int32_t *__restrict__ in_coords, const int32_t *__restrict__ in_table,
                uint32_t in_mask, int ks, int ts_in, int RB, int64_t n_cap, int32_t *__restrict__ hits,
                int32_t *__restrict__ block_counts, int KW, uint32_t *mask_out, uint32_t *mask_in) {
  __shared__ int wave_cnt[KM_THREADS / 64];
  const int rb = blockIdx.x, k = blockIdx.y;
  const int n_out = *n_out_dev;
  if (rb * KM_THREADS >= n_out) {
    if (threadIdx.x == 0) block_counts[(int64_t)k * RB + rb] = 0;
    return;
  }
  int32_t delta[D];
  offset_of<D>(k, ks, ts_in, delta);
  const int64_t o = (int64_t)rb * KM_THREADS + threadIdx.x;
  int hit = -1;
  if (o < n_out) {
    hit = probe<D>(out_coords, o, delta, in_coords, in_table, in_mask);
    hits[(int64_t)k * n_cap + o] = hit;
    if (hit >= 0) {
      atomicOr(&mask_out[o * KW + (k >> 5)], 1u << (k & 31));
      if (mask_in) atomicOr(&mask_in[(int64_t)hit * KW + (k >> 5)], 1u << (k & 31));
    }
  }
  unsigned long long m = __ballot(hit >= 0);
  if ((threadIdx.x & 63) == 0) wave_cnt[threadIdx.x >> 6] = __popcll(m);
  __syncthreads();
  if (threadIdx.x == 0) {
    int s = 0;
#pragma unroll
    for (int w = 0; w < KM_THREADS / 64; ++w) s += wave_cnt[w];
    block_counts[(int64_t)k * RB + rb] = s;
  }
}

__device__ __forceinline__ int mask_rank(const uint32_t *__restrict__ m, int k) {
  int r = 0;
  const int w = k >> 5;
  for (int i = 0; i < w; ++i) r += __popc(m[i]);
  return r + __popc(m[w] & ((1u << (k & 31)) - 1u));
}

__global__ void mask_count_kernel(const uint32_t *__restrict__ mask, int KW, const int32_t *n_dev, int64_t n_cap,
                                  int32_t *__restrict__ cnt, unsigned short *__restrict__ wpre = nullptr) {
  const int64_t r = (int64_t)blockIdx.x * blockDim.x + threadIdx.x;
  if (r >= n_cap) return;
  int c = 0;
  if (r < *n_dev)
    for (int i = 0; i < KW; ++i) {
      if (wpre) wpre[r * KW + i] = (unsigned short)c;
      c += __popc(mask[r * KW + i]);
    }
  cnt[r] = c;
}
constexpr int KM_MC_JOBS = 8;
struct MaskCountJobs {
  const uint32_t *mask[KM_MC_JOBS];
  const int32_t *n_dev[KM_MC_JOBS];
  long long n_cap[KM_MC_JOBS];
  int32_t *cnt[KM_MC_JOBS];
  unsigned short *wpre[KM_MC_JOBS];
};
template <int KW>
__global__ void mask_count_multi(MaskCountJobs J) {
  const int m = blockIdx.y;
  const int64_t r = (int64_t)blockIdx.x * blockDim.x + threadIdx.x;
  if (r >= J.n_cap[m]) return;
  int c = 0;
  if (r < *J.n_dev[m]) {
    uint32_t w[KW];
#pragma unroll
    for (int i = 0; i < KW; ++i) w[i] = J.mask[m][r * KW + i];
#pragma unroll
    for (int i = 0; i < KW; ++i) {
      J.wpre[m][r * KW + i] = (unsigned short)c;
      c += __popc(w[i]);
    }
  }
  J.cnt[m][r] = c;
}
__device__ __forceinline__ int mask_rank_pre(const uint32_t *__restrict__ m, const unsigned short *__restrict__ pre, int k) {
  return pre[k >> 5] + __popc(m[k >> 5] & ((1u << (k & 31)) - 1u));
}


__device__ __forceinline__ unsigned long long hit_pack(int k, int64_t o, int64_t in) {
  return ((unsigned long long)k << 54) | ((unsigned long long)o << 27) | (unsigned long long)in;
}
constexpr int KM_REGION = 512;
constexpr int KM_JOBS6 = 8;
struct HitList {
  unsigned long long *recs;
  int32_t *wave_count;
  int region;
};
__device__ __forceinline__ void hit_begin(volatile int *cur) {
  if ((threadIdx.x & 63) == 0) cur[threadIdx.x >> 6] = 0;
}
__device__ __forceinline__ int64_t hit_slots(int n, const HitList &h, volatile int *cur, int wave_id) {
  const unsigned long long act = __ballot(1), two = __ballot(n == 2);
  const int lane = threadIdx.x & 63, w = threadIdx.x >> 6;
  const unsigned long long below = (1ull << lane) - 1ull;
  int base = 0;
  if (lane == __ffsll((long long)act) - 1) {
    base = cur[w];
    const int need = __popcll(act) + __popcll(two);
    if (base >= 0 && base + need <= h.region) {
      cur[w] = base + need;
    } else {
      cur[w] = -1;
      base = -1;
    }
  }
  base = __builtin_amdgcn_readfirstlane(base);
  if (base < 0) return -1;
  return (int64_t)wave_id * h.region + base + __popcll(act & below) + __popcll(two & below);
}
__device__ __forceinline__ void hit_end(const HitList &h, volatile int *cur, int wave_id) {
  if ((threadIdx.x & 63) == 0) h.wave_count[wave_id] = cur[threadIdx.x >> 6];
}

struct PrunedArgs {
  const int32_t *out_coords, *n_out_dev;
  const int4 *out_order;
  int64_t n_cap;
  DgrHalfBuckets hb;
  int ts_in, symmetric;
};
template <class Emit>
__device__ __forceinline__ void pruned_search6(const PrunedArgs &a, int64_t t, Emit &&emit) {
  const int NJ = a.symmetric ? 14 : 27;
  const int ts_in = a.ts_in;
  const int ja = (int)(t / a.n_cap);
  const int64_t p = t - (int64_t)ja * a.n_cap;
  int b = -1;
  int64_t o = 0;
  int c4 = 0, c5 = 0, c6 = 0;
  if (ja < NJ && p < *a.n_out_dev) {
    const int4 me = a.out_order[p];
    o = me.w; c4 = me.x; c5 = me.y; c6 = me.z;
    const int32_t *co = a.out_coords + o * 7;
    int32_t q[4];
    q[0] = co[0];
    q[1] = co[1] + ((ja % 3) - 1) * ts_in;
    q[2] = co[2] + (((ja / 3) % 3) - 1) * ts_in;
    q[3] = co[3] + ((ja / 9) - 1) * ts_in;
    b = dgr_lookup<4>(a.hb.table, a.hb.mask, a.hb.bkeys, q);
  }
  const int beg = b >= 0 ? a.hb.start[b] : 0, end = b >= 0 ? a.hb.start[b + 1] : 0;
  for (int p0 = beg; p0 < end; p0 += 4) {
    int4 e[4];
#pragma unroll
    for (int u = 0; u < 4; ++u) e[u] = a.hb.second[min(p0 + u, end - 1)];
#pragma unroll
    for (int u = 0; u < 4; ++u) {
      if (p0 + u >= end) break;
      const int d4 = e[u].x - c4, d5 = e[u].y - c5, d6 = e[u].z - c6;
      if (abs(d4) <= ts_in && abs(d5) <= ts_in && abs(d6) <= ts_in) {
        const int k = ja + 27 * ((d4 / ts_in + 1) + 3 * (d5 / ts_in + 1) + 9 * (d6 / ts_in + 1));
        if (a.symmetric && ja == 13 && k > 364) continue;
        emit(k, o, e[u].w);
      }
    }
  }
}

struct Bits6Jobs {
  PrunedArgs pa[KM_JOBS6];
  uint32_t *mask_out[KM_JOBS6], *mask_in[KM_JOBS6];
  HitList hl[KM_JOBS6];
  int blocks[KM_JOBS6];
};
__global__ void __launch_bounds__(KM_THREADS)
    kmap_bits_pruned6(Bits6Jobs J, int KW) {
  __shared__ int hit_cur[KM_THREADS / 64];
  const int jm = blockIdx.y;
  if ((int)blockIdx.x >= J.blocks[jm]) return;
  const PrunedArgs a = J.pa[jm];
  uint32_t *const mask_out = J.mask_out[jm], *const mask_in = J.mask_in[jm];
  const HitList hl = J.hl[jm];
  hit_begin(hit_cur);
  const int wid = (int)(blockIdx.x * (KM_THREADS / 64) + (threadIdx.x >> 6));
  pruned_search6(a, (int64_t)blockIdx.x * KM_THREADS + threadIdx.x, [&](int k, int64_t o, int in) {
    atomicOr(&mask_out[o * KW + (k >> 5)], 1u << (k & 31));
    const int km = 728 - k;
    if (a.symmetric) {
      if (km != k) atomicOr(&mask_out[(int64_t)in * KW + (km >> 5)], 1u << (km & 31));
    } else if (mask_in) {
      atomicOr(&mask_in[(int64_t)in * KW + (k >> 5)], 1u << (k & 31));
    }
    const int n = (a.symmetric && km != k) ? 2 : 1;
    const int64_t s = hit_slots(n, hl, hit_cur, wid);
    if (s >= 0) {
      hl.recs[s] = hit_pack(k, o, in);
      if (n == 2) hl.recs[s + 1] = hit_pack(km, in, o);
    }
  });
  hit_end(hl, hit_cur, wid);
}

constexpr int KM_KMAX = 736;
struct Colmask6Jobs {
  const uint32_t *mask_out[KM_JOBS6];
  const int32_t *n_out_dev[KM_JOBS6];
  int RB[KM_JOBS6];
  int4 *cell[KM_JOBS6];
  int32_t *counts[KM_JOBS6], *row_cnt[KM_JOBS6];
  unsigned short *wpre[KM_JOBS6];
};
__global__ void __launch_bounds__(KM_THREADS)
    kmap_colmask(Colmask6Jobs J, int K, int KW) {
  __shared__ unsigned long long bal[KM_THREADS / 64][KM_KMAX];
  const int jm = blockIdx.y;
  const int RB = J.RB[jm];
  if ((int)blockIdx.x >= RB) return;
  const uint32_t *__restrict__ mask_out = J.mask_out[jm];
  const int32_t *n_out_dev = J.n_out_dev[jm];
  int4 *__restrict__ cell = J.cell[jm];
  int32_t *__restrict__ counts = J.counts[jm], *__restrict__ row_cnt = J.row_cnt[jm];
  unsigned short *__restrict__ wpre = J.wpre[jm];
  const int rb = blockIdx.x;
  const int lane = threadIdx.x & 63, wave = threadIdx.x >> 6;
  const int n_out = *n_out_dev;
  const int64_t o = (int64_t)rb * KM_THREADS + threadIdx.x;
  int row_pairs = 0;
  constexpr int KW_MAX = (KM_KMAX + 31) / 32;
  uint32_t words[KW_MAX];
#pragma unroll
  for (int w = 0; w < KW_MAX; ++w) words[w] = (w < KW && o < n_out) ? mask_out[o * KW + w] : 0u;
#pragma unroll
  for (int w = 0; w < KW_MAX; ++w) {
    if (w < KW) {
      const uint32_t word = words[w];
      if (o < n_out) wpre[o * KW + w] = (unsigned short)row_pairs;
      row_pairs += __popc(word);
      unsigned long long mine = 0;
#pragma unroll
      for (int b = 0; b < 32; ++b) {
        const unsigned long long m = __ballot((word >> b) & 1u);
        if (lane == b) mine = m;
      }
      if (lane < 32 && 32 * w + lane < KM_KMAX) bal[wave][32 * w + lane] = mine;
    }
  }
  if (o < n_out) row_cnt[o] = row_pairs;
  __syncthreads();
  for (int k = threadIdx.x; k < K; k += KM_THREADS) {
    int run = 0;
#pragma unroll
    for (int g = 0; g < KM_THREADS / 64; ++g) {
      const unsigned long long m = bal[g][k];
      cell[((int64_t)rb * (KM_THREADS / 64) + g) * K + k] = make_int4((int)(m & 0xffffffffull), (int)(m >> 32), run, 0);
      run += __popcll(m);
    }
    counts[(int64_t)k * RB + rb] = run;
  }
}

struct PlaceArgs {
  int K, KW, RB;
  const uint32_t *mask_out;
  const int32_t *out_ptr;
  const int4 *cell;
  const int32_t *base;
  int32_t *pair_in, *pair_out;
  uint16_t *pair_k;
  int32_t *out_pos;
  int64_t pair_cap;
  int32_t *overflow;
  const uint32_t *mask_in;
  const int32_t *in_ptr;
  int32_t *in_pos;
  const unsigned short *wpre_out, *wpre_in;
};
__device__ __forceinline__ void place_pair(const PlaceArgs &p, int k, int64_t o, int64_t in) {
  const int64_t slot = (int64_t)p.out_ptr[o] + mask_rank_pre(p.mask_out + o * p.KW, p.wpre_out + o * p.KW, k);
  const int64_t g = o >> 6;
  const int4 c = p.cell[g * p.K + k];
  const unsigned long long cm = ((unsigned long long)(uint32_t)c.y << 32) | (uint32_t)c.x;
  const int64_t pos = (int64_t)p.base[(int64_t)k * p.RB + (g >> 2)] + c.z + __popcll(cm & ((1ull << (o & 63)) - 1ull));
  if (pos < p.pair_cap && slot < p.pair_cap) {
    p.pair_in[pos] = (int32_t)in;
    if (p.pair_out) p.pair_out[pos] = (int32_t)o;
    if (p.pair_k) p.pair_k[pos] = (uint16_t)k;
    p.out_pos[slot] = (int32_t)pos;
    if (p.mask_in) p.in_pos[p.in_ptr[in] + mask_rank_pre(p.mask_in + in * p.KW, p.wpre_in + in * p.KW, k)] = (int32_t)pos;
  } else {
    *p.overflow = 2;
  }
}

struct Place6Jobs {
  HitList h[KM_JOBS6];
  PlaceArgs p[KM_JOBS6];
  PrunedArgs replay[KM_JOBS6];
  int n_waves[KM_JOBS6], blocks[KM_JOBS6];
};
__global__ void __launch_bounds__(KM_THREADS)
    kmap_place_hits(Place6Jobs J) {
  const int jm = blockIdx.y;
  const int nblk = J.blocks[jm];
  if ((int)blockIdx.x >= nblk) return;
  const HitList h = J.h[jm];
  const PlaceArgs p = J.p[jm];
  const PrunedArgs replay = J.replay[jm];
  const int n_waves = J.n_waves[jm];
  const int lane = threadIdx.x & 63;
  for (int r = blockIdx.x * (KM_THREADS / 64) + (threadIdx.x >> 6); r < n_waves; r += nblk * (KM_THREADS / 64)) {
    const int n = h.wave_count[r];
    if (n < 0) {
      pruned_search6(replay, (int64_t)r * 64 + lane, [&](int k, int64_t o, int in) {
        place_pair(p, k, o, in);
        if (replay.symmetric && 728 - k != k) place_pair(p, 728 - k, in, o);
      });
      continue;
    }
    for (int e = lane; e < n; e += 64) {
      const unsigned long long rec = h.recs[(int64_t)r * h.region + e];
      place_pair(p, (int)(rec >> 54), (int64_t)((rec >> 27) & 0x7ffffffull), (int64_t)(rec & 0x7ffffffull));
    }
  }
}

constexpr int KM_KGROUP = 8;
__global__ void __launch_bounds__(KM_THREADS)
    kmap_fill(const int32_t *n_out_dev, int RB, int K, int64_t n_cap, const int32_t *__restrict__ hits,
              const int32_t *__restrict__ block_counts, const int32_t *__restrict__ block_base,
              int32_t *__restrict__ pair_in, int32_t *__restrict__ pair_out, int64_t pair_cap,
              int32_t *overflow, int KW, const uint32_t *__restrict__ mask_out,
              const int32_t *__restrict__ out_ptr, int32_t *__restrict__ out_pos,
              const uint32_t *__restrict__ mask_in, const int32_t *__restrict__ in_ptr,
              int32_t *__restrict__ in_pos, uint16_t *__restrict__ pair_k) {
  __shared__ int wave_cnt[2][KM_THREADS / 64];
  const int rb = blockIdx.x;
  const int n_out = *n_out_dev;
  if (rb * KM_THREADS >= n_out) return;
  const int lane = threadIdx.x & 63, wave = threadIdx.x >> 6;
  const int64_t o = (int64_t)rb * KM_THREADS + threadIdx.x;
  int parity = 0;
  for (int kk = 0; kk < KM_KGROUP; ++kk) {
    const int k = blockIdx.y * KM_KGROUP + kk;
    if (k >= K) break;
    const int64_t cell = (int64_t)k * RB + rb;
    if (block_counts[cell] == 0) continue;
    int hit = -1;
    if (o < n_out) hit = hits[(int64_t)k * n_cap + o];
    const unsigned long long m = __ballot(hit >= 0);
    if (lane == 0) wave_cnt[parity][wave] = __popcll(m);
    __syncthreads();
    if (hit >= 0) {
      int base = block_base[cell];
      for (int w = 0; w < wave; ++w) base += wave_cnt[parity][w];
      const int64_t pos = base + __popcll(m & ((1ull << lane) - 1ull));
      if (pos < pair_cap) {
        pair_in[pos] = hit;
        if (pair_out) pair_out[pos] = (int32_t)o;
        if (pair_k) pair_k[pos] = (uint16_t)k;
        out_pos[out_ptr[o] + mask_rank(mask_out + o * KW, k)] = (int32_t)pos;
        if (mask_in) in_pos[in_ptr[hit] + mask_rank(mask_in + (int64_t)hit * KW, k)] = (int32_t)pos;
      } else {
        *overflow = 2;
      }
    }
    parity ^= 1;
  }
}

constexpr int KM_MAXJOBS = 8;
struct FinalizeJobs {
  const int32_t *base[KM_MAXJOBS], *total[KM_MAXJOBS];
  int32_t *rule_ptr[KM_MAXJOBS], *tile_ptr[KM_MAXJOBS];
  int4 *desc[KM_MAXJOBS];
  long long tile_cap[KM_MAXJOBS];
  int K[KM_MAXJOBS], RB[KM_MAXJOBS];
};
__global__ void __launch_bounds__(1024) kmap_finalize(FinalizeJobs j) {
  __shared__ int s[1024];
  const int m = blockIdx.x, K = j.K[m], RB = j.RB[m];
  const int32_t *block_base = j.base[m];
  const int k = threadIdx.x;
  int start = 0, end = 0;
  if (k < K) {
    start = block_base[(int64_t)k * RB];
    end = (k + 1 < K) ? block_base[(int64_t)(k + 1) * RB] : *j.total[m];
    j.rule_ptr[m][k] = start;
    if (k == K - 1) j.rule_ptr[m][K] = end;
  }
  const int tiles = (end - start + DGR_TILE_M - 1) / DGR_TILE_M;
  s[k] = tiles;
  __syncthreads();
  for (int d = 1; d < 1024; d <<= 1) {
    const int v = (k >= d) ? s[k - d] : 0;
    __syncthreads();
    s[k] += v;
    __syncthreads();
  }
  if (k < K) j.tile_ptr[m][k] = s[k] - tiles;
  if (k == K - 1) j.tile_ptr[m][K] = s[k];
}

__device__ __forceinline__ void tile_desc_one(const int32_t *__restrict__ tile_ptr, const int32_t *__restrict__ rule_ptr, int K,
                                              int4 *__restrict__ desc, int64_t tile_cap, int64_t t, int tile_m) {
  if (t >= tile_cap || t >= tile_ptr[K]) return;
  int lo = 0, hi = K;
  while (hi - lo > 1) {
    const int mid = (lo + hi) >> 1;
    if (tile_ptr[mid] <= t) lo = mid; else hi = mid;
  }
  const int pstart = rule_ptr[lo] + ((int)t - tile_ptr[lo]) * tile_m;
  desc[t] = make_int4(lo, pstart, min(tile_m, rule_ptr[lo + 1] - pstart), 0);
}
__global__ void tile_desc_kernel(FinalizeJobs j) {
  const int m = blockIdx.y;
  const int64_t t = (int64_t)blockIdx.x * blockDim.x + threadIdx.x;
  tile_desc_one(j.tile_ptr[m], j.rule_ptr[m], j.K[m], j.desc[m], j.tile_cap[m], t, DGR_TILE_M);
}

static int alloc_kernel_map(DgrArena &arena, int K, int64_t n_cap, int64_t n_in_cap, int max_pairs_per_row, bool need_in_csr,
                            bool want_pair_out, bool want_pair_k, DgrKernelMap *km) {
  DGR_REQUIRE(K <= 1024, "kernel volume %d > 1024 not supported", K);
  km->K = K;
  const int64_t per_row = K < max_pairs_per_row ? K : max_pairs_per_row;
  km->pair_cap = per_row * n_cap;
  DGR_REQUIRE(km->pair_cap < (1ll << 31), "kernel map too large (%lld pairs)", (long long)km->pair_cap);
  DGR_ALLOC(km->rule_ptr, arena, int32_t, K + 1);
  DGR_ALLOC(km->tile_ptr, arena, int32_t, K + 1);
  DGR_ALLOC(km->pair_in, arena, int32_t, km->pair_cap);
  km->pair_out = nullptr;
  if (want_pair_out) DGR_ALLOC(km->pair_out, arena, int32_t, km->pair_cap);
  km->tile_cap = km->pair_cap / DGR_TILE_M + K;
  DGR_ALLOC(km->tile_desc, arena, int4, km->tile_cap);
  DGR_ALLOC(km->out_ptr, arena, int32_t, n_cap + 1);
  DGR_ALLOC(km->out_pos, arena, int32_t, km->pair_cap);
  km->pair_k = nullptr;
  if (want_pair_k) DGR_ALLOC(km->pair_k, arena, uint16_t, km->pair_cap);
  if (need_in_csr) {
    DGR_ALLOC(km->in_ptr, arena, int32_t, n_in_cap + 1);
    DGR_ALLOC(km->in_pos, arena, int32_t, km->pair_cap);
  }
  return DGR_OK;
}

static void finalize_job(FinalizeJobs &fj, int m, const int32_t *base, const int32_t *total, int K, int RB, DgrKernelMap *km) {
  fj.base[m] = base; fj.total[m] = total; fj.K[m] = K; fj.RB[m] = RB;
  fj.rule_ptr[m] = km->rule_ptr; fj.tile_ptr[m] = km->tile_ptr;
  fj.desc[m] = km->tile_desc; fj.tile_cap[m] = km->tile_cap;
}

static int build_kernel_map3(DgrArena &arena, const DgrCoordMap &in, const DgrCoordMap &out, int ks, int max_pairs_per_row,
                             bool need_in_csr, bool want_pair_out, bool want_pair_k, DgrKernelMap *km,
                             int32_t *overflow, hipStream_t stream) {
  constexpr int D = 3;
  const int K = ks * ks * ks;
  const int64_t n_cap = out.n_cap, n_in_cap = in.n_cap;
  const int RB = (int)dgr_ceil_div(n_cap, KM_THREADS);
  DGR_CHECK(alloc_kernel_map(arena, K, n_cap, n_in_cap, max_pairs_per_row, need_in_csr, want_pair_out, want_pair_k, km));
  const int KW = (K + 31) / 32;
  DgrArena::Mark mk = arena.mark();
  int32_t *counts, *base, *total;
  DGR_ALLOC(counts, arena, int32_t, (int64_t)K * RB);
  DGR_ALLOC(base, arena, int32_t, (int64_t)K * RB);
  DGR_ALLOC(total, arena, int32_t, 1);
  uint32_t *mask_out, *mask_in = nullptr;
  int32_t *cnt_out, *cnt_in = nullptr;
  {
    const size_t w_out = (size_t)(n_cap + 1) * KW, w_in = need_in_csr ? (size_t)(n_in_cap + 1) * KW : 0;
    DGR_ALLOC(mask_out, arena, uint32_t, w_out + w_in);
    if (need_in_csr) mask_in = mask_out + w_out;
    DGR_HIP_CHECK(hipMemsetAsync(mask_out, 0, (w_out + w_in) * sizeof(uint32_t), stream));
  }
  DGR_ALLOC(cnt_out, arena, int32_t, n_cap + 1);
  if (need_in_csr) DGR_ALLOC(cnt_in, arena, int32_t, n_in_cap + 1);
  int32_t *hits;
  DGR_ALLOC(hits, arena, int32_t, (int64_t)K * n_cap);
  kmap_search<D><<<dim3(RB, K), KM_THREADS, 0, stream>>>(out.coords, out.n_dev, in.coords, in.table, in.table_mask, ks,
                                                         in.ts, RB, n_cap, hits, counts, KW, mask_out, mask_in);
  DGR_LAUNCH_CHECK();
  mask_count_kernel<<<(int)dgr_ceil_div(n_cap + 1, 256), 256, 0, stream>>>(mask_out, KW, out.n_dev, n_cap + 1, cnt_out);
  if (need_in_csr)
    mask_count_kernel<<<(int)dgr_ceil_div(n_in_cap + 1, 256), 256, 0, stream>>>(mask_in, KW, in.n_dev, n_in_cap + 1, cnt_in);
  {
    const int32_t *ins[3] = {cnt_out, counts, cnt_in};
    int32_t *outs[3] = {km->out_ptr, base, km->in_ptr}, *tots[3] = {nullptr, total, nullptr};
    const int64_t ns[3] = {n_cap + 1, (int64_t)K * RB, n_in_cap + 1};
    DGR_CHECK(dgr_exclusive_scan_multi(arena, need_in_csr ? 3 : 2, ins, outs, ns, tots, stream));
  }
  FinalizeJobs fj = {};
  finalize_job(fj, 0, base, total, K, RB, km);
  kmap_finalize<<<1, 1024, 0, stream>>>(fj);
  tile_desc_kernel<<<dim3((unsigned)dgr_ceil_div(km->tile_cap, 256), 1), 256, 0, stream>>>(fj);
  kmap_fill<<<dim3(RB, (K + KM_KGROUP - 1) / KM_KGROUP), KM_THREADS, 0, stream>>>(
      out.n_dev, RB, K, n_cap, hits, counts, base, km->pair_in, km->pair_out, km->pair_cap, overflow, KW, mask_out,
      km->out_ptr, km->out_pos, mask_in, km->in_ptr, km->in_pos, km->pair_k);
  DGR_LAUNCH_CHECK();
  arena.rewind(mk);
  km->built = true;
  return DGR_OK;
}

struct Kmap6Job {
  const DgrCoordMap *in, *out;
  const DgrHalfBuckets *hb;
  const DgrHalfBuckets *hb_out;
  bool need_in_csr, want_pair_out, want_pair_k;
  DgrKernelMap *km;
};
static int build_kernel_maps6(DgrArena &arena, const Kmap6Job *jobs, int nj, int max_pairs_per_row, int32_t *overflow,
                              hipStream_t stream) {
  constexpr int K = 729, KW = (K + 31) / 32;
  DGR_REQUIRE(nj >= 1 && nj <= KM_MAXJOBS, "6-D kernel maps: %d jobs", nj);
  struct Tr {
    int RB, symmetric;
    int64_t n_cap, n_in_cap, hit_waves;
    int32_t *counts, *base, *total, *cnt_out, *cnt_in;
    uint32_t *mask_out, *mask_in;
    int4 *cell;
    HitList hl;
    unsigned short *wpre_out, *wpre_in;
  } t[KM_MAXJOBS];
  for (int m = 0; m < nj; ++m) {
    const Kmap6Job &J = jobs[m];
    t[m].n_cap = J.out->n_cap; t[m].n_in_cap = J.in->n_cap;
    DGR_REQUIRE(t[m].n_cap < (1ll << 27) && t[m].n_in_cap < (1ll << 27), "6-D kernel maps: more than 2^27 rows");
    DGR_CHECK(alloc_kernel_map(arena, K, t[m].n_cap, t[m].n_in_cap, max_pairs_per_row, J.need_in_csr, J.want_pair_out,
                               J.want_pair_k, J.km));
  }
  DgrArena::Mark mk = arena.mark();
  {
    size_t words = 0;
    for (int m = 0; m < nj; ++m)
      words += (size_t)(t[m].n_cap + 1) * KW + (jobs[m].need_in_csr ? (size_t)(t[m].n_in_cap + 1) * KW : 0) + (size_t)(t[m].n_cap + 1);
    uint32_t *pool;
    DGR_ALLOC(pool, arena, uint32_t, words);
    DGR_HIP_CHECK(hipMemsetAsync(pool, 0, words * sizeof(uint32_t), stream));
    for (int m = 0; m < nj; ++m) {
      t[m].mask_out = pool; pool += (size_t)(t[m].n_cap + 1) * KW;
      t[m].mask_in = nullptr;
      if (jobs[m].need_in_csr) { t[m].mask_in = pool; pool += (size_t)(t[m].n_in_cap + 1) * KW; }
      t[m].cnt_out = reinterpret_cast<int32_t *>(pool); pool += (size_t)(t[m].n_cap + 1);
    }
  }
  for (int m = 0; m < nj; ++m) {
    const Kmap6Job &J = jobs[m];
    Tr &r = t[m];
    r.RB = (int)dgr_ceil_div(r.n_cap, KM_THREADS);
    r.symmetric = (J.in->coords == J.out->coords && !J.need_in_csr) ? 1 : 0;
    DGR_REQUIRE(J.hb && J.hb->built && J.hb_out && J.hb_out->built, "6-D kernel map: first-half buckets missing");
    DGR_ALLOC(r.counts, arena, int32_t, (int64_t)K * r.RB);
    DGR_ALLOC(r.base, arena, int32_t, (int64_t)K * r.RB);
    DGR_ALLOC(r.total, arena, int32_t, 1);
    r.cnt_in = nullptr;
    if (J.need_in_csr) DGR_ALLOC(r.cnt_in, arena, int32_t, r.n_in_cap + 1);
    DGR_ALLOC(r.cell, arena, int4, (int64_t)r.RB * (KM_THREADS / 64) * K);
    const int64_t search_blocks = dgr_ceil_div(r.n_cap * (r.symmetric ? 14 : 27), KM_THREADS);
    r.hit_waves = search_blocks * (KM_THREADS / 64);
    r.hl.region = (J.in->ts >= 8 && r.symmetric) ? 2 * KM_REGION : KM_REGION / 2;
    DGR_REQUIRE(r.hit_waves < (1ll << 31), "6-D kernel map: too many search waves");
    DGR_ALLOC(r.hl.recs, arena, unsigned long long, r.hit_waves * r.hl.region);
    DGR_ALLOC(r.hl.wave_count, arena, int32_t, r.hit_waves);
    DGR_ALLOC(r.wpre_out, arena, unsigned short, (r.n_cap + 1) * KW);
    r.wpre_in = nullptr;
    if (J.need_in_csr) DGR_ALLOC(r.wpre_in, arena, unsigned short, (r.n_in_cap + 1) * KW);
  }
  static_assert(KM_JOBS6 >= KM_MAXJOBS, "multi-job launch tables");
  {
    Bits6Jobs bj = {};
    Colmask6Jobs cj = {};
    int max_sb = 0, max_rb = 0;
    for (int m = 0; m < nj; ++m) {
      const Kmap6Job &J = jobs[m];
      Tr &r = t[m];
      bj.pa[m] = PrunedArgs{J.out->coords, J.out->n_dev, J.hb_out->second, r.n_cap, *J.hb, J.in->ts, r.symmetric};
      bj.mask_out[m] = r.mask_out; bj.mask_in[m] = r.mask_in; bj.hl[m] = r.hl;
      bj.blocks[m] = (int)(r.hit_waves / (KM_THREADS / 64));
      max_sb = std::max(max_sb, bj.blocks[m]);
      cj.mask_out[m] = r.mask_out; cj.n_out_dev[m] = J.out->n_dev; cj.RB[m] = r.RB; cj.cell[m] = r.cell;
      cj.counts[m] = r.counts; cj.row_cnt[m] = r.cnt_out; cj.wpre[m] = r.wpre_out;
      max_rb = std::max(max_rb, r.RB);
    }
    kmap_bits_pruned6<<<dim3((unsigned)max_sb, (unsigned)nj), KM_THREADS, 0, stream>>>(bj, KW);
    kmap_colmask<<<dim3((unsigned)max_rb, (unsigned)nj), KM_THREADS, 0, stream>>>(cj, K, KW);
    {
      MaskCountJobs mj = {};
      int nm = 0;
      long long max_rows = 0;
      for (int m = 0; m < nj; ++m)
        if (jobs[m].need_in_csr) {
          mj.mask[nm] = t[m].mask_in; mj.n_dev[nm] = jobs[m].in->n_dev; mj.n_cap[nm] = t[m].n_in_cap + 1;
          mj.cnt[nm] = t[m].cnt_in; mj.wpre[nm] = t[m].wpre_in;
          max_rows = std::max(max_rows, mj.n_cap[nm]);
          ++nm;
        }
      static_assert(KM_MC_JOBS >= KM_MAXJOBS, "mask-count job table");
      if (nm) mask_count_multi<KW><<<dim3((unsigned)dgr_ceil_div(max_rows, 256), (unsigned)nm), 256, 0, stream>>>(mj);
    }
  }
  DGR_LAUNCH_CHECK();
  {
    const int32_t *ins[DGR_SCAN_MAX];
    int32_t *outs[DGR_SCAN_MAX], *tots[DGR_SCAN_MAX];
    int64_t ns[DGR_SCAN_MAX];
    int c = 0;
    for (int m = 0; m < nj; ++m) {
      ins[c] = t[m].cnt_out; outs[c] = jobs[m].km->out_ptr; tots[c] = nullptr; ns[c++] = t[m].n_cap + 1;
      ins[c] = t[m].counts; outs[c] = t[m].base; tots[c] = t[m].total; ns[c++] = (int64_t)K * t[m].RB;
      if (jobs[m].need_in_csr) { ins[c] = t[m].cnt_in; outs[c] = jobs[m].km->in_ptr; tots[c] = nullptr; ns[c++] = t[m].n_in_cap + 1; }
    }
    DGR_CHECK(dgr_exclusive_scan_multi(arena, c, ins, outs, ns, tots, stream));
  }
  FinalizeJobs fj = {};
  int64_t max_tiles = 0;
  for (int m = 0; m < nj; ++m) {
    finalize_job(fj, m, t[m].base, t[m].total, K, t[m].RB, jobs[m].km);
    max_tiles = std::max<int64_t>(max_tiles, jobs[m].km->tile_cap);
  }
  kmap_finalize<<<nj, 1024, 0, stream>>>(fj);
  tile_desc_kernel<<<dim3((unsigned)dgr_ceil_div(max_tiles, 256), nj), 256, 0, stream>>>(fj);
  {
    Place6Jobs pj = {};
    int max_pb = 0;
    for (int m = 0; m < nj; ++m) {
      const Kmap6Job &J = jobs[m];
      Tr &r = t[m];
      DgrKernelMap *km = J.km;
      pj.p[m] = PlaceArgs{K, KW, r.RB, r.mask_out, km->out_ptr, r.cell, r.base, km->pair_in, km->pair_out, km->pair_k, km->out_pos,
                          km->pair_cap, overflow, r.mask_in, km->in_ptr, km->in_pos, r.wpre_out, r.wpre_in};
      pj.replay[m] = PrunedArgs{J.out->coords, J.out->n_dev, J.hb_out->second, r.n_cap, *J.hb, J.in->ts, r.symmetric};
      pj.h[m] = r.hl;
      pj.n_waves[m] = (int)r.hit_waves;
      pj.blocks[m] = (int)std::min<int64_t>(dgr_ceil_div(r.hit_waves, KM_THREADS / 64), 16384);
      max_pb = std::max(max_pb, pj.blocks[m]);
      km->built = true;
    }
    kmap_place_hits<<<dim3((unsigned)max_pb, (unsigned)nj), KM_THREADS, 0, stream>>>(pj);
  }
  DGR_LAUNCH_CHECK();
  arena.rewind(mk);
  return DGR_OK;
}

constexpr int NBR_JOBS = 10;
struct NbrJobs {
  const int32_t *out_coords[NBR_JOBS], *n_out_dev[NBR_JOBS], *in_coords[NBR_JOBS], *in_table[NBR_JOBS];
  uint32_t in_mask[NBR_JOBS];
  int ts[NBR_JOBS];
  long long n_pad[NBR_JOBS];
  int32_t *nbr[NBR_JOBS];
};
__global__ void __launch_bounds__(KM_THREADS) nbr_search3(NbrJobs J) {
  const int jm = blockIdx.z;
  const int64_t n_pad = J.n_pad[jm];
  const int64_t o = (int64_t)blockIdx.x * KM_THREADS + threadIdx.x;
  if (o >= n_pad) return;
  int32_t *__restrict__ nbr = J.nbr[jm];
  const int kz = blockIdx.y;
  if (o >= *J.n_out_dev[jm]) {
#pragma unroll
    for (int u = 0; u < 9; ++u) nbr[(int64_t)(9 * kz + u) * n_pad + o] = -1;
    return;
  }
  const int sts = J.ts[jm];
  const int4 c = *reinterpret_cast<const int4 *>(J.out_coords[jm] + o * 4);
  int32_t q[9][4];
#pragma unroll
  for (int u = 0; u < 9; ++u) {
    q[u][0] = c.x;
    q[u][1] = c.y + ((u % 3) - 1) * sts;
    q[u][2] = c.z + ((u / 3) - 1) * sts;
    q[u][3] = c.w + (kz - 1) * sts;
  }
  int hit[9];
  dgr_lookup_many<4, 9>(J.in_table[jm], J.in_mask[jm], J.in_coords[jm], q, hit);
#pragma unroll
  for (int u = 0; u < 9; ++u) nbr[(int64_t)(9 * kz + u) * n_pad + o] = hit[u];
}

struct ClsJobs {
  const int32_t *coords[3], *n_dev[3];
  int ts[3], nb[3];
  int32_t *blk_cnt[3], *perm[3], *cls_count[3];
  long long cls_cap[3];
};
__device__ __forceinline__ int parity_class(const int32_t *coords, int64_t o, int ts) {
  const int4 c = *reinterpret_cast<const int4 *>(coords + o * 4);
  return ((c.y / ts) & 1) | (((c.z / ts) & 1) << 1) | (((c.w / ts) & 1) << 2);
}
__global__ void __launch_bounds__(KM_THREADS) cls_count_kernel(ClsJobs J) {
  __shared__ int wcnt[KM_THREADS / 64][8];
  const int l = blockIdx.y, b = blockIdx.x;
  if (b >= J.nb[l]) return;
  const int64_t o = (int64_t)b * KM_THREADS + threadIdx.x;
  const int cls = o < *J.n_dev[l] ? parity_class(J.coords[l], o, J.ts[l]) : 8;
#pragma unroll
  for (int c = 0; c < 8; ++c) {
    const unsigned long long m = __ballot(cls == c);
    if ((threadIdx.x & 63) == 0) wcnt[threadIdx.x >> 6][c] = __popcll(m);
  }
  __syncthreads();
  if (threadIdx.x < 8) {
    int n = 0;
    for (int w = 0; w < KM_THREADS / 64; ++w) n += wcnt[w][threadIdx.x];
    J.blk_cnt[l][b * 8 + threadIdx.x] = n;
  }
}
__global__ void __launch_bounds__(KM_THREADS) cls_fill_kernel(ClsJobs J) {
  __shared__ int part[KM_THREADS / 64][8], before[8], wcnt[KM_THREADS / 64][8];
  const int l = blockIdx.y, b = blockIdx.x;
  if (b >= J.nb[l]) return;
  const int lane = threadIdx.x & 63, wave = threadIdx.x >> 6;
  int acc[8] = {0, 0, 0, 0, 0, 0, 0, 0};
  for (int bb = threadIdx.x; bb < b; bb += KM_THREADS) {
    const int4 lo = *reinterpret_cast<const int4 *>(J.blk_cnt[l] + bb * 8), hi = *reinterpret_cast<const int4 *>(J.blk_cnt[l] + bb * 8 + 4);
    acc[0] += lo.x; acc[1] += lo.y; acc[2] += lo.z; acc[3] += lo.w;
    acc[4] += hi.x; acc[5] += hi.y; acc[6] += hi.z; acc[7] += hi.w;
  }
#pragma unroll
  for (int c = 0; c < 8; ++c) {
    int v = acc[c];
    for (int d = 32; d > 0; d >>= 1) v += __shfl_down(v, d, 64);
    if (lane == 0) part[wave][c] = v;
  }
  const int64_t o = (int64_t)b * KM_THREADS + threadIdx.x;
  const int cls = o < *J.n_dev[l] ? parity_class(J.coords[l], o, J.ts[l]) : 8;
  int rank = 0;
#pragma unroll
  for (int c = 0; c < 8; ++c) {
    const unsigned long long m = __ballot(cls == c);
    if (lane == 0) wcnt[wave][c] = __popcll(m);
    if (cls == c) rank = __popcll(m & ((1ull << lane) - 1ull));
  }
  __syncthreads();
  if (threadIdx.x < 8) {
    int n = 0;
    for (int w = 0; w < KM_THREADS / 64; ++w) n += part[w][threadIdx.x];
    before[threadIdx.x] = n;
    if (b == J.nb[l] - 1) {
      for (int w = 0; w < KM_THREADS / 64; ++w) n += wcnt[w][threadIdx.x];
      J.cls_count[l][threadIdx.x] = n;
    }
  }
  __syncthreads();
  if (cls < 8) {
    int pos = before[cls] + rank;
    for (int w = 0; w < wave; ++w) pos += wcnt[w][cls];
    J.perm[l][(int64_t)cls * J.cls_cap[l] + pos] = (int32_t)o;
  }
}

static int build_nbr_table(DgrArena &arena, const DgrCoordMap &in, const DgrCoordMap &out, int ts, int sign,
                           DgrNbrTable *t, NbrJobs *jobs, int *nj, int32_t *cls_count = nullptr) {
  t->K = 27;
  t->n_pad = dgr_ceil_div(out.n_cap, DGR_OS_ROWS) * DGR_OS_ROWS;
  DGR_ALLOC(t->nbr, arena, int32_t, t->n_pad * 27);
  t->perm = nullptr; t->cls_count = nullptr; t->cls_cap = 0;
  if (cls_count) {
    t->cls_cap = t->n_pad;
    t->cls_count = cls_count;
    DGR_ALLOC(t->perm, arena, int32_t, 8 * t->cls_cap);
  }
  DGR_REQUIRE(*nj < NBR_JOBS, "neighbour tables: more than %d per launch", NBR_JOBS);
  const int m = (*nj)++;
  jobs->out_coords[m] = out.coords; jobs->n_out_dev[m] = out.n_dev; jobs->in_coords[m] = in.coords;
  jobs->in_table[m] = in.table; jobs->in_mask[m] = in.table_mask; jobs->ts[m] = sign > 0 ? ts : -ts;
  jobs->n_pad[m] = t->n_pad; jobs->nbr[m] = t->nbr;
  t->built = true;
  return DGR_OK;
}
static int nbr_tables_launch(const NbrJobs &jobs, int nj, hipStream_t stream) {
  long long n_max = 0;
  for (int m = 0; m < nj; ++m) n_max = std::max(n_max, jobs.n_pad[m]);
  if (nj == 0) return DGR_OK;
  nbr_search3<<<dim3((unsigned)dgr_ceil_div(n_max, KM_THREADS), 3, (unsigned)nj), KM_THREADS, 0, stream>>>(jobs);
  DGR_LAUNCH_CHECK();
  return DGR_OK;
}

__global__ void nbr_count_kernel(const int32_t *__restrict__ nbr, int64_t n_pad, const int32_t *n_out_dev,
                                 unsigned long long *__restrict__ counts) {
  const int k = blockIdx.y;
  const int n = *n_out_dev;
  int c = 0;
  for (int64_t o = (int64_t)blockIdx.x * blockDim.x + threadIdx.x; o < n; o += (int64_t)gridDim.x * blockDim.x)
    c += nbr[(int64_t)k * n_pad + o] >= 0;
  for (int d = 32; d > 0; d >>= 1) c += __shfl_down(c, d, 64);
  if ((threadIdx.x & 63) == 0 && c) atomicAdd(&counts[k], (unsigned long long)c);
}

int dgr_nbr_counts(const DgrNbrTable &t, const int32_t *n_out_dev, int64_t counts[27]) {
  unsigned long long *dev;
  DGR_HIP_CHECK(hipMalloc((void **)&dev, 27 * sizeof(unsigned long long)));
  DGR_HIP_CHECK(hipMemset(dev, 0, 27 * sizeof(unsigned long long)));
  nbr_count_kernel<<<dim3(64, 27), 256>>>(t.nbr, t.n_pad, n_out_dev, dev);
  unsigned long long host[27];
  hipError_t e = hipMemcpy(host, dev, sizeof(host), hipMemcpyDeviceToHost);
  (void)hipFree(dev);
  DGR_HIP_CHECK(e);
  for (int k = 0; k < 27; ++k) counts[k] = (int64_t)host[k];
  return DGR_OK;
}

int dgr_build_coord_maps(DgrArena &arena, const int32_t *coords, int64_t N, DgrMapSet *ms,
                         hipStream_t stream);
int dgr_build_half_buckets(DgrArena &arena, DgrCoordMap *cm, DgrHalfBuckets *hb, int levels, int renumber_from, hipStream_t stream);

int dgr_build_maps(DgrArena &arena, const int32_t *coords, int64_t N, int D, int conv1_ks,
                   DgrMapSet *ms, hipStream_t stream, bool skip_conv1_map, bool lean, bool nbr_tables) {
  DGR_REQUIRE(D == 3 || D == 6, "D=%d not supported (the DGR path uses D=3 and D=6)", D);
  DGR_REQUIRE(conv1_ks % 2 == 1 && conv1_ks >= 1, "conv1 kernel size must be odd");
  DGR_REQUIRE(N > 0 && N < (1ll << 30), "N=%lld out of range", (long long)N);
  ms->D = D;
  ms->nc = D + 1;
  ms->conv1_ks = conv1_ks;
  if (!ms->overflow) {
    DGR_ALLOC(ms->overflow, arena, int32_t, 1);
    DGR_HIP_CHECK(hipMemsetAsync(ms->overflow, 0, sizeof(int32_t), stream));
  }
  DGR_CHECK(dgr_build_coord_maps(arena, coords, N, ms, stream));
  if (nbr_tables) {
    DGR_REQUIRE(D == 3, "neighbour tables are a D = 3 structure");
    ms->use_nbr = true;
    NbrJobs nbj = {};
    int n_nbj = 0;
    int32_t *cls;
    DGR_ALLOC(cls, arena, int32_t, 3 * 8);
    for (int l = 0; l < 4; ++l) DGR_CHECK(build_nbr_table(arena, ms->cm[l], ms->cm[l], ms->cm[l].ts, +1, &ms->nsame[l], &nbj, &n_nbj));
    for (int l = 0; l < 3; ++l) {
      DGR_CHECK(build_nbr_table(arena, ms->cm[l], ms->cm[l + 1], ms->cm[l].ts, +1, &ms->ndown[l], &nbj, &n_nbj));
      DGR_CHECK(build_nbr_table(arena, ms->cm[l + 1], ms->cm[l], ms->cm[l].ts, -1, &ms->nup[l], &nbj, &n_nbj, cls + 8 * l));
    }
    DGR_CHECK(nbr_tables_launch(nbj, n_nbj, stream));
    {
      ClsJobs cj = {};
      int max_nb = 0;
      for (int l = 0; l < 3; ++l) {
        cj.coords[l] = ms->cm[l].coords; cj.n_dev[l] = ms->cm[l].n_dev; cj.ts[l] = ms->cm[l].ts;
        cj.nb[l] = (int)dgr_ceil_div(ms->cm[l].n_cap, KM_THREADS);
        DGR_ALLOC(cj.blk_cnt[l], arena, int32_t, (int64_t)cj.nb[l] * 8);
        cj.perm[l] = ms->nup[l].perm; cj.cls_count[l] = ms->nup[l].cls_count; cj.cls_cap[l] = ms->nup[l].cls_cap;
        max_nb = std::max(max_nb, cj.nb[l]);
      }
      cls_count_kernel<<<dim3((unsigned)max_nb, 3), KM_THREADS, 0, stream>>>(cj);
      cls_fill_kernel<<<dim3((unsigned)max_nb, 3), KM_THREADS, 0, stream>>>(cj);
      DGR_LAUNCH_CHECK();
    }
    if (lean) {
      if (conv1_ks != 3 && !skip_conv1_map)
        DGR_CHECK(build_kernel_map3(arena, ms->cm[0], ms->cm[0], conv1_ks, 1024, false, false, true, &ms->conv1, ms->overflow,
                                    stream));
      return DGR_OK;
    }
  }
  const int cap_row = (D == 3) ? 1024 : 160;
  if (D == 6) {
    DGR_REQUIRE(conv1_ks == 3, "6-D kernel maps support kernel size 3 only (got %d)", conv1_ks);
    DGR_CHECK(dgr_build_half_buckets(arena, ms->cm, ms->hb, 4, 1, stream));
    Kmap6Job jobs[7];
    for (int l = 0; l < 4; ++l) jobs[l] = {&ms->cm[l], &ms->cm[l], &ms->hb[l], &ms->hb[l], false, !lean, !lean || l == 0, &ms->same[l]};
    for (int l = 0; l < 3; ++l) jobs[4 + l] = {&ms->cm[l], &ms->cm[l + 1], &ms->hb[l], &ms->hb[l + 1], true, true, !lean, &ms->down[l]};
    DGR_CHECK(build_kernel_maps6(arena, jobs, 7, cap_row, ms->overflow, stream));
    ms->conv1 = ms->same[0];
    return DGR_OK;
  }
  auto build = [&](const DgrCoordMap &in, const DgrCoordMap &out, int ks, bool rev, bool want_k, DgrKernelMap *km) -> int {
    const bool want_out = !lean || rev, want_pk = !lean || want_k;
    return build_kernel_map3(arena, in, out, ks, cap_row, rev, want_out, want_pk, km, ms->overflow, stream);
  };
  for (int l = 0; l < 4; ++l) DGR_CHECK(build(ms->cm[l], ms->cm[l], 3, false, l == 0, &ms->same[l]));
  if (conv1_ks == 3)
    ms->conv1 = ms->same[0];
  else if (!skip_conv1_map)
    DGR_CHECK(build(ms->cm[0], ms->cm[0], conv1_ks, false, true, &ms->conv1));
  for (int l = 0; l < 3; ++l) DGR_CHECK(build(ms->cm[l], ms->cm[l + 1], 3, true, false, &ms->down[l]));
  return DGR_OK;
}

struct dgr_maps {
  dgr_ctx *ctx;
  DgrArena arena;
  DgrMapSet ms;
  int32_t *coords_copy = nullptr;
  hipStream_t stream;
};

extern "C" int dgr_maps_create(dgr_ctx *ctx, const int32_t *coords, int64_t N, int D,
                               int conv1_kernel_size, dgr_maps **out, dgr_stream stream_) {
  DGR_REQUIRE(ctx && coords && out, "dgr_maps_create: NULL argument");
  hipStream_t stream = (hipStream_t)stream_;
  DGR_HIP_CHECK(hipSetDevice(ctx->device));
  dgr_maps *m = new dgr_maps();
  m->ctx = ctx;
  m->stream = stream;
  int rc = DGR_OK;
  do {
    m->coords_copy = m->arena.get<int32_t>((size_t)N * (D + 1));
    if (!m->coords_copy) { rc = DGR_ENOMEM; break; }
    if (hipMemcpyAsync(m->coords_copy, coords, (size_t)N * (D + 1) * sizeof(int32_t),
                       hipMemcpyDeviceToDevice, stream) != hipSuccess) { rc = DGR_EHIP; break; }
    rc = dgr_build_maps(m->arena, m->coords_copy, N, D, conv1_kernel_size, &m->ms, stream, false, false, D == 3);
    if (rc != DGR_OK) break;
    int32_t flag = 0;
    if (hipMemcpyAsync(&flag, m->ms.overflow, sizeof(int32_t), hipMemcpyDeviceToHost, stream) != hipSuccess ||
        hipStreamSynchronize(stream) != hipSuccess) { rc = DGR_EHIP; dgr_set_error("maps sync failed"); break; }
    if (flag == 1) { dgr_set_error("duplicate coordinates in the sparse tensor input"); rc = DGR_EINVAL; break; }
    if (flag == 2) { dgr_set_error("kernel-map capacity exceeded"); rc = DGR_ENOMEM; break; }
  } while (0);
  if (rc != DGR_OK) {
    m->arena.release();
    delete m;
    return rc;
  }
  *out = m;
  return DGR_OK;
}

extern "C" void dgr_maps_destroy(dgr_maps *m) {
  if (!m) return;
  (void)hipDeviceSynchronize();
  m->arena.release();
  delete m;
}

static int level_of(int ts) { return ts == 1 ? 0 : ts == 2 ? 1 : ts == 4 ? 2 : ts == 8 ? 3 : -1; }

extern "C" int dgr_maps_get_coords(dgr_maps *m, int ts, int32_t *host_out, int64_t capacity,
                                   int64_t *n) {
  DGR_REQUIRE(m && n, "NULL argument");
  int l = level_of(ts);
  DGR_REQUIRE(l >= 0, "tensor stride %d not in {1,2,4,8}", ts);
  int32_t n32 = 0;
  DGR_HIP_CHECK(hipMemcpy(&n32, m->ms.cm[l].n_dev, sizeof(int32_t), hipMemcpyDeviceToHost));
  *n = n32;
  if (host_out) {
    DGR_REQUIRE(capacity >= (int64_t)n32 * m->ms.nc, "host buffer too small");
    const int nc = m->ms.nc;
    if (!m->ms.cm[l].canon) {
      DGR_HIP_CHECK(hipMemcpy(host_out, m->ms.cm[l].coords, (size_t)n32 * nc * sizeof(int32_t), hipMemcpyDeviceToHost));
    } else {
      std::vector<int32_t> tmp((size_t)n32 * nc), canon(n32);
      DGR_HIP_CHECK(hipMemcpy(tmp.data(), m->ms.cm[l].coords, tmp.size() * sizeof(int32_t), hipMemcpyDeviceToHost));
      DGR_HIP_CHECK(hipMemcpy(canon.data(), m->ms.cm[l].canon, canon.size() * sizeof(int32_t), hipMemcpyDeviceToHost));
      for (int32_t p = 0; p < n32; ++p) memcpy(host_out + (size_t)canon[p] * nc, tmp.data() + (size_t)p * nc, nc * sizeof(int32_t));
    }
  }
  return DGR_OK;
}

extern "C" int dgr_maps_get_kernel_map(dgr_maps *m, int kind, int ts, int32_t *rule_ptr,
                                       int64_t rule_cap, int32_t *pair_in, int32_t *pair_out,
                                       int64_t pair_cap, int64_t *K, int64_t *P) {
  DGR_REQUIRE(m && K && P, "NULL argument");
  int l = level_of(ts);
  DGR_REQUIRE(l >= 0, "tensor stride %d not in {1,2,4,8}", ts);
  if (kind >= 3 && kind <= 5) {
    const DgrNbrTable *t = kind == 3 ? &m->ms.nsame[l] : (l < 3 ? (kind == 4 ? &m->ms.ndown[l] : &m->ms.nup[l]) : nullptr);
    DGR_REQUIRE(t && t->built, "no such neighbour table (kind %d, ts %d)", kind, ts);
    const DgrCoordMap &om = kind == 4 ? m->ms.cm[l + 1] : m->ms.cm[l];
    int32_t n_out = 0;
    DGR_HIP_CHECK(hipMemcpy(&n_out, om.n_dev, sizeof(int32_t), hipMemcpyDeviceToHost));
    std::vector<int32_t> tab((size_t)t->n_pad * 27);
    DGR_HIP_CHECK(hipMemcpy(tab.data(), t->nbr, tab.size() * sizeof(int32_t), hipMemcpyDeviceToHost));
    *K = 27;
    int64_t total = 0;
    for (int k = 0; k < 27; ++k) {
      if (rule_ptr && k < rule_cap) rule_ptr[k] = (int32_t)total;
      for (int o = 0; o < n_out; ++o) {
        const int32_t v = tab[(size_t)k * t->n_pad + o];
        if (v < 0) continue;
        if (pair_in && pair_out) {
          DGR_REQUIRE(total < pair_cap, "pair buffers too small");
          pair_in[total] = v;
          pair_out[total] = o;
        }
        ++total;
      }
    }
    if (rule_ptr) {
      DGR_REQUIRE(rule_cap >= 28, "rule_ptr buffer too small");
      rule_ptr[27] = (int32_t)total;
    }
    for (int64_t o = n_out; o < t->n_pad; ++o)
      for (int k = 0; k < 27; ++k) DGR_REQUIRE(tab[(size_t)k * t->n_pad + o] == -1, "neighbour table padding is not -1");
    *P = total;
    return DGR_OK;
  }
  const DgrKernelMap *km = nullptr;
  if (kind == 0) km = &m->ms.same[l];
  else if (kind == 1) km = &m->ms.conv1;
  else if (kind == 2 && l < 3) km = &m->ms.down[l];
  DGR_REQUIRE(km && km->built, "no such kernel map (kind %d, ts %d)", kind, ts);
  *K = km->K;
  int32_t total = 0;
  DGR_HIP_CHECK(hipMemcpy(&total, km->rule_ptr + km->K, sizeof(int32_t), hipMemcpyDeviceToHost));
  *P = total;
  if (rule_ptr) {
    DGR_REQUIRE(rule_cap >= km->K + 1, "rule_ptr buffer too small");
    DGR_HIP_CHECK(hipMemcpy(rule_ptr, km->rule_ptr, (size_t)(km->K + 1) * sizeof(int32_t),
                            hipMemcpyDeviceToHost));
  }
  if (pair_in && pair_out) {
    DGR_REQUIRE(pair_cap >= total, "pair buffers too small");
    DGR_HIP_CHECK(hipMemcpy(pair_in, km->pair_in, (size_t)total * sizeof(int32_t), hipMemcpyDeviceToHost));
    DGR_HIP_CHECK(hipMemcpy(pair_out, km->pair_out, (size_t)total * sizeof(int32_t), hipMemcpyDeviceToHost));
    const DgrCoordMap &cin = m->ms.cm[l], &cout = m->ms.cm[kind == 2 ? l + 1 : l];
    if (cin.canon || cout.canon) {
      auto fetch = [&](const DgrCoordMap &c, std::vector<int32_t> &v) -> int {
        if (!c.canon) return DGR_OK;
        int32_t n = 0;
        DGR_HIP_CHECK(hipMemcpy(&n, c.n_dev, sizeof(int32_t), hipMemcpyDeviceToHost));
        v.resize(n);
        DGR_HIP_CHECK(hipMemcpy(v.data(), c.canon, (size_t)n * sizeof(int32_t), hipMemcpyDeviceToHost));
        return DGR_OK;
      };
      std::vector<int32_t> ci, co, rp(km->K + 1);
      DGR_CHECK(fetch(cin, ci));
      DGR_CHECK(fetch(cout, co));
      DGR_HIP_CHECK(hipMemcpy(rp.data(), km->rule_ptr, rp.size() * sizeof(int32_t), hipMemcpyDeviceToHost));
      std::vector<std::pair<int32_t, int32_t>> tmp;
      for (int k = 0; k < km->K; ++k) {
        tmp.clear();
        for (int32_t q = rp[k]; q < rp[k + 1]; ++q)
          tmp.push_back({cout.canon ? co[pair_out[q]] : pair_out[q], cin.canon ? ci[pair_in[q]] : pair_in[q]});
        std::sort(tmp.begin(), tmp.end());
        for (size_t u = 0; u < tmp.size(); ++u) { pair_out[rp[k] + u] = tmp[u].first; pair_in[rp[k] + u] = tmp[u].second; }
      }
    }
  }
  return DGR_OK;
}
```

### deepglobalregistration_amd/csrc/net.hip

```cpp
#include <math.h>
#include <stdlib.h>
#include <string.h>

#include <algorithm>
#include <map>
#include <memory>
#include <string>

#include "dgr_internal.h"

static const int CH[5] = {0, 32, 64, 128, 256};
static const int TR[5] = {0, 64, 64, 64, 128};
static constexpr float BN_EPS = 1e-5f;

struct DgrLayer {
  std::string name;
  int K, cin, cout, cin_pad, cout_pad;
  float *w = nullptr;
  float *w16 = nullptr;
  void *w16b = nullptr;
  void *w16d = nullptr;
  int64_t w16b_piece = 0;
  float *wc = nullptr;
  float *wq = nullptr;
// ... 133 lines not shown
    if (hipMemcpy(small.back().data(), d->data, (size_t)d->numel * sizeof(float), hipMemcpyDeviceToHost) != hipSuccess) return nullptr;
    return small.back().data();
  };
  if (bn) {
    std::string p = std::string(bn) + ".bn.";
    const dgr_weight_desc *g = find_desc(descs, nd, p + "weight"), *b = find_desc(descs, nd, p + "bias"),
                          *m = find_desc(descs, nd, p + "running_mean"),
                          *v = find_desc(descs, nd, p + "running_var");
    DGR_REQUIRE(g && b && m && v, "state_dict is missing batch-norm tensors '%s*'", p.c_str());
    DGR_REQUIRE(g->numel == cout && b->numel == cout && m->numel == cout && v->numel == cout,
                "batch-norm '%s' has the wrong width", p.c_str());
    const float *gd = host_of(g), *bd2 = host_of(b), *md = host_of(m), *vd = host_of(v);
    DGR_REQUIRE(gd && bd2 && md && vd, "batch-norm '%s': device tensors could not be read", p.c_str());
    for (int c = 0; c < cout; ++c) {
      float s = gd[c] / sqrtf(vd[c] + BN_EPS);
      scale[c] = s;
      shift[c] = bd2[c] - md[c] * s;
    }
    has_shift = true;
  }
  if (bias) {
    const dgr_weight_desc *bd = find_desc(descs, nd, name + ".bias");
    DGR_REQUIRE(bd && bd->numel == cout, "state_dict is missing '%s.bias' [1,%d]", name.c_str(), cout);
    const float *bh = host_of(bd);
    DGR_REQUIRE(bh, "'%s.bias': device tensor could not be read", name.c_str());
    for (int c = 0; c < cout; ++c) shift[c] += bh[c];
    has_shift = true;
  }
  DgrWeights &W = *net->W;
  hipStream_t s = P.s;
  const float *src = kd->data;
  if (!P.dev) {
    const size_t n = (size_t)kd->numel;
    if (n > P.staging_n) {
      DGR_HIP_CHECK(hipStreamSynchronize(s));
      DGR_HIP_CHECK(hipFree(P.staging));
      P.staging = nullptr;
      DGR_HIP_CHECK(hipMalloc((void **)&P.staging, n * sizeof(float)));
      P.staging_n = n;
    }
    DGR_HIP_CHECK(hipMemcpyAsync(P.staging, kd->data, n * sizeof(float), hipMemcpyHostToDevice, s));
    src = P.staging;
  }
  const float *sc = P.sc;
  DGR_HIP_CHECK(hipMemcpyAsync(P.sc, scale.data(), (size_t)cout * sizeof(float), hipMemcpyHostToDevice, s));
  if (has_shift) {
    DGR_CHECK(W.alloc(&L.shift, cout));
    DGR_HIP_CHECK(hipMemcpyAsync(L.shift, shift.data(), (size_t)cout * sizeof(float), hipMemcpyHostToDevice, s));
  }
  const int64_t nw = (int64_t)K * cin * cout;
  DGR_HIP_CHECK(hipMemsetAsync(P.mxb, 0, sizeof(uint32_t), s));
  dgr_absmax_scaled_kernel<<<(int)std::min<int64_t>((nw + 255) / 256, 4096), 256, 0, s>>>(src, sc, nw, cout, P.mxb);
  DGR_LAUNCH_CHECK();
  uint32_t bits = 0;
  DGR_HIP_CHECK(hipMemcpyAsync(&bits, P.mxb, sizeof(bits), hipMemcpyDeviceToHost, s));
  DGR_HIP_CHECK(hipStreamSynchronize(s));
  float mx;
  memcpy(&mx, &bits, 4);
  int ex = 0;
  if (mx > 0.f && std::isfinite(mx)) (void)frexpf(mx, &ex);
  ex = std::min(std::max(ex, -100), 100);
  const float w_scale = ldexpf(1.f, 15 - ex);
  L.w_unscale = ldexpf(1.f, ex - 15);
  const bool use_wide = K > 1 && !dgr_exact_f32() && dgr_conv_wide_supported(L.cin_pad, cin, cout) && !(net->D == 3 && K == 27);
  if (use_wide) {
    const int S16 = cin / 16, NB32 = cout / 32;
    L.wb_piece = (int64_t)K * S16 * NB32 * 64;
    const int64_t ne = L.wb_piece * 8;
    uint16_t *dst;
    DGR_CHECK(W.alloc(&dst, (size_t)2 * ne));
    L.wb = dst;
    DGR_CHECK(dgr_fill(s, ne, [=] __device__(int64_t o) {
      const int e = (int)(o & 7), lane = (int)((o >> 3) & 63);
      const int64_t r = o >> 9;
      const int nb = (int)(r % NB32), s2 = (int)((r / NB32) % S16), k = (int)(r / ((int64_t)NB32 * S16));
      const int col = 32 * nb + (lane & 31), row = 16 * s2 + 8 * (lane >> 5) + e;
      const float xs = __fmul_rn(__fmul_rn(src[((size_t)k * cin + row) * cout + col], sc[col]), w_scale);
      dst[o] = dgr_f16_bits_dev(xs);
      dst[ne + o] = dgr_f16_bits_dev(xs - dgr_f16_val_dev(xs));
    }));
    W.param_bytes += (size_t)2 * ne * sizeof(uint16_t);
  } else {
    const int S = L.cin_pad / 8, NBLK = L.cout_pad / 32;
    const int64_t ne = (int64_t)K * S * NBLK * 256;
    DGR_CHECK(W.alloc(&L.w, ne));
    float *const dst = L.w;
    DGR_CHECK(dgr_fill(s, ne, [=] __device__(int64_t o) {
      const int c = (int)(o & 3), lane = (int)((o >> 2) & 63);
      const int64_t r = o >> 8;
      const int nb = (int)(r % NBLK), s2 = (int)((r / NBLK) % S), k = (int)(r / ((int64_t)NBLK * S));
      const int row = 8 * s2 + 4 * (lane >> 5) + c, col = 32 * nb + (lane & 31);
      dst[o] = (row < cin && col < cout) ? __fmul_rn(src[((size_t)k * cin + row) * cout + col], sc[col]) : 0.f;
    }));
    W.param_bytes += (size_t)ne * sizeof(float);
  }
  if (net->D == 3 && K == 27 && L.cin_pad % 16 == 0 && cout % 32 == 0) {
    const int GT = L.cin_pad / 16, NB = cout / 16;
    {
      const int64_t ne = (int64_t)K * GT * NB * 256;
      DGR_CHECK(W.alloc(&L.w16, ne));
      float *const dst = L.w16;
      DGR_CHECK(dgr_fill(s, ne, [=] __device__(int64_t o) {
        const int c = (int)(o & 3), lane = (int)((o >> 2) & 63);
        const int64_t r = o >> 8;
        const int jb = (int)(r % NB), g = (int)((r / NB) % GT), k = (int)(r / ((int64_t)NB * GT));
        const int col = 16 * jb + (lane & 15), row = 16 * g + 4 * (lane >> 4) + c;
        dst[o] = row < cin ? __fmul_rn(src[((size_t)k * cin + row) * cout + col], sc[col]) : 0.f;
      }));
      W.param_bytes += (size_t)ne * sizeof(float);
    }
    if (cin % 32 == 0) {
      const int S32 = cin / 32;
      L.w16b_piece = (int64_t)K * S32 * NB * 64;
      const int64_t ne = L.w16b_piece * 8;
      uint16_t *pcs;
      DGR_CHECK(W.alloc(&pcs, (size_t)2 * ne));
      L.w16b = pcs;
      DGR_CHECK(dgr_fill(s, ne, [=] __device__(int64_t o) {
        const int e = (int)(o & 7), lane = (int)((o >> 3) & 63);
        const int64_t r = o >> 9;
        const int jb = (int)(r % NB), sI = (int)((r / NB) % S32), k = (int)(r / ((int64_t)NB * S32));
        const int col = 16 * jb + (lane & 15), row = 32 * sI + 8 * (lane >> 4) + e;
        const float xs = __fmul_rn(__fmul_rn(src[((size_t)k * cin + row) * cout + col], sc[col]), w_scale);
        pcs[o] = dgr_f16_bits_dev(xs);
        pcs[ne + o] = dgr_f16_bits_dev(xs - dgr_f16_val_dev(xs));
      }));
      W.param_bytes += (size_t)2 * ne * sizeof(uint16_t);
      if (net->D == 3 && K == 27 && (dgr_conv_dense_supported(cin, L.cin_pad, cout) || dgr_conv_up_supported(cin, L.cin_pad, cout))) {
        uint16_t *pd;
        DGR_CHECK(W.alloc(&pd, (size_t)2 * ne));
        L.w16d = pd;
        DGR_CHECK(dgr_fill(s, 2 * ne, [=] __device__(int64_t o) {
          const int e = (int)(o & 3), h = (int)((o >> 2) & 1);
          const int64_t f = o >> 3, base = f & ~(int64_t)63;
          const int lane = (int)(f & 63), col = lane & 15, lq = lane >> 4;
          const int64_t srcf = base + col + 16 * ((lq >> 1) + 2 * h);
          pd[o] = pcs[srcf * 8 + 4 * (lq & 1) + e];
        }));
        W.param_bytes += (size_t)2 * ne * sizeof(uint16_t);
      }
    }
  }
  if (net->D == 3 && name == "conv1" && cin == 1 && cout == 32 && K <= 343) {
    int ks = 1;
    while (ks * ks * ks < K) ++ks;
    const int ks2 = ks * ks, steps = (ks2 + 3) / 4;
    const int64_t ne = (int64_t)ks * steps * 128;
    DGR_CHECK(W.alloc(&L.wc, ne));
    float *const dst = L.wc;
    DGR_CHECK(dgr_fill(s, ne, [=] __device__(int64_t o) {
      const int j = (int)(o & 1), lane = (int)((o >> 1) & 63);
      const int64_t r = o >> 7;
      const int s2 = (int)(r % steps), kz = (int)(r / steps);
      const int kk = 4 * s2 + (lane >> 4), col = (lane & 15) + 16 * j;
      dst[o] = kk < ks2 ? __fmul_rn(src[(size_t)(kz * ks2 + kk) * cout + col], sc[col]) : 0.f;
    }));
  }
  if (name == "conv1" && cin == 6 && cout == 32 && K > 1) {
    const int64_t ne = (int64_t)K * 192;
    DGR_CHECK(W.alloc(&L.wq, ne));
    float *const dst = L.wq;
    DGR_CHECK(dgr_fill(s, ne, [=] __device__(int64_t o) {
      const int e = (int)(o & 3), q = (int)((o >> 2) & 3);
      const int i = (int)((o >> 4) % 12), k = (int)(o / 192);
      const int ci = i >> 1, co = 8 * q + 4 * (i & 1) + e;
      dst[o] = __fmul_rn(src[((size_t)k * cin + ci) * cout + co], sc[co]);
    }));
    W.param_bytes += (size_t)ne * sizeof(float);
  }
  W.layers.push_back(L);
  return DGR_OK;
}

static int net_create(dgr_ctx *ctx, int D, int in_channels, int out_channels, int conv1_kernel_size, int normalize_feature,
                      const dgr_weight_desc *weights, int n_weights, dgr_net **out, bool dev) {
  DGR_REQUIRE(ctx && weights && out, "dgr_net_create: NULL argument");
  if (dev) {
    for (int i = 0; i < n_weights; ++i) {
      hipPointerAttribute_t at;
      const hipError_t e = hipPointerGetAttributes(&at, weights[i].data);
      if (e != hipSuccess) (void)hipGetLastError();
      DGR_REQUIRE(e == hipSuccess && at.type == hipMemoryTypeDevice && at.device == ctx->device,
                  "dgr_net_create_device: '%s' is not a device pointer on device %d (use dgr_net_create for host tensors)",
                  weights[i].name ? weights[i].name : "?", ctx->device);
    }
  }
  DGR_REQUIRE(D == 3 || D == 6, "dgr_net_create: D=%d (ResUNetBN2C is used with D=3 and D=6)", D);
  DGR_REQUIRE(in_channels >= 1 && in_channels <= 256 && out_channels >= 1 && out_channels <= 64,
              "dgr_net_create: unsupported channel counts in=%d out=%d", in_channels, out_channels);
  DGR_REQUIRE(conv1_kernel_size % 2 == 1, "conv1 kernel size must be odd");
  DGR_HIP_CHECK(hipSetDevice(ctx->device));
  WeightPrep P{dev};
  DGR_HIP_CHECK(hipStreamCreate(&P.s));
  DGR_HIP_CHECK(hipMalloc((void **)&P.sc, 256 * sizeof(float)));
  DGR_HIP_CHECK(hipMalloc((void **)&P.mxb, sizeof(uint32_t)));
  dgr_net *net = new dgr_net();
  net->ctx = ctx;
  net->W = std::make_shared<DgrWeights>();
  net->W->device = ctx->device;
  net->D = D; net->cin = in_channels; net->cout = out_channels;
  net->conv1_ks = conv1_kernel_size; net->normalize = normalize_feature;
  int k3 = 1, k1 = 1;
  for (int d = 0; d < D; ++d) { k3 *= 3; k1 *= conv1_kernel_size; }
  int rc = DGR_OK;
  auto L = [&](const std::string &name, int K, int ci, int co, const char *bn, bool bias = false) {
    if (rc == DGR_OK) rc = make_layer(net, P, weights, n_weights, name, K, ci, co, bn, bias);
  };
  auto block = [&](const std::string &b, int c) {
    L(b + ".conv1", k3, c, c, (b + ".norm1").c_str());
    L(b + ".conv2", k3, c, c, (b + ".norm2").c_str());
  };
  L("conv1", k1, in_channels, CH[1], "norm1");          block("block1", CH[1]);
  L("conv2", k3, CH[1], CH[2], "norm2");                block("block2", CH[2]);
  L("conv3", k3, CH[2], CH[3], "norm3");                block("block3", CH[3]);
  L("conv4", k3, CH[3], CH[4], "norm4");                block("block4", CH[4]);
  L("conv4_tr", k3, CH[4], TR[4], "norm4_tr");          block("block4_tr", TR[4]);
  L("conv3_tr", k3, CH[3] + TR[4], TR[3], "norm3_tr");  block("block3_tr", TR[3]);
  L("conv2_tr", k3, CH[2] + TR[3], TR[2], "norm2_tr");  block("block2_tr", TR[2]);
  L("conv1_tr", 1, CH[1] + TR[2], TR[1], nullptr);
  L("final", 1, TR[1], out_channels, nullptr, true);
  if (rc == DGR_OK) rc = [&] { DGR_HIP_CHECK(hipStreamSynchronize(P.s)); return DGR_OK; }();
  if (rc != DGR_OK) {
    dgr_net_destroy(net);
    return rc;
  }
  *out = net;
  return DGR_OK;
}

extern "C" int dgr_net_create(dgr_ctx *ctx, int D, int in_channels, int out_channels,
                              int conv1_kernel_size, int normalize_feature,
                              const dgr_weight_desc *weights, int n_weights, dgr_net **out) {
  return net_create(ctx, D, in_channels, out_channels, conv1_kernel_size, normalize_feature, weights, n_weights, out, false);
}

extern "C" int dgr_net_create_device(dgr_ctx *ctx, int D, int in_channels, int out_channels,
                                     int conv1_kernel_size, int normalize_feature,
                                     const dgr_weight_desc *weights, int n_weights, dgr_net **out) {
  return net_create(ctx, D, in_channels, out_channels, conv1_kernel_size, normalize_feature, weights, n_weights, out, true);
}

extern "C" void dgr_net_destroy(dgr_net *net) {
  if (!net) return;
  delete net;
}

extern "C" int dgr_net_share(dgr_ctx *ctx, const dgr_net *src, dgr_net **out) {
  DGR_REQUIRE(ctx && src && out, "dgr_net_share: NULL argument");
  DGR_REQUIRE(ctx->device == src->W->device, "dgr_net_share: the weights live on device %d, the context on device %d",
              src->W->device, ctx->device);
  dgr_net *net = new dgr_net();
  net->ctx = ctx;
  net->D = src->D; net->cin = src->cin; net->cout = src->cout;
  net->conv1_ks = src->conv1_ks; net->normalize = src->normalize;
  net->W = src->W;
  *out = net;
  return DGR_OK;
}

extern "C" int dgr_net_sharers(const dgr_net *net) { return net ? (int)net->W.use_count() : 0; }
extern "C" int64_t dgr_net_param_bytes(const dgr_net *net) { return net ? net->W->param_bytes : 0; }
extern "C" int dgr_net_num_layers(const dgr_net *net) { return net ? (int)net->W->layers.size() : 0; }

struct Tensor {
  float *ptr;
  int ld;
  int relu;
  DgrSplitRows split;
  bool split_only = false;
  uint32_t *amax = nullptr, *amax2 = nullptr;
  unsigned char *dsplit = nullptr;
  bool dsplit_only = false;
};

struct Fwd {
  dgr_ctx *ctx;
  dgr_net *net;
  hipStream_t stream;
  DgrMapSet ms;
  bool prof;
  bool l2_next = false;

  float *ybuf = nullptr;

  int conv(int li, const Tensor &in, const DgrKernelMap *km, bool swapped, int lvl_in, int lvl_out,
           const Tensor &out, const Tensor *res) {
    const DgrLayer &L = net->W->layers[li];
    const DgrCoordMap &cin_map = ms.cm[lvl_in], &cout_map = ms.cm[lvl_out];
    DgrConvLaunch a;
    a.in = in.ptr; a.in_ld = in.ld; a.in_relu = in.relu;
    a.out = out.ptr; a.out_ld = out.ld;
    a.y = ybuf; a.shift = L.shift;
    a.w = L.w;
    a.cin = L.cin; a.cin_pad = L.cin_pad; a.cout = L.cout; a.cout_pad = L.cout_pad; a.K = L.K;
    if (km && ms.use_nbr) {
      a.pair_in = a.pair_out = a.tile_ptr = a.rule_ptr = nullptr;
      a.tile_desc = nullptr; a.n_rows_dev = nullptr; a.tile_bound = 0;
    } else if (km) {
      a.pair_in = swapped ? km->pair_out : km->pair_in;
      a.pair_out = swapped ? km->pair_in : km->pair_out;
      a.tile_ptr = km->tile_ptr; a.rule_ptr = km->rule_ptr; a.tile_desc = km->tile_desc;
      a.n_rows_dev = nullptr;
      a.tile_bound = km->pair_cap / DGR_TILE_M + km->K;
      DGR_REQUIRE(km->K == L.K, "layer %s: kernel volume mismatch", L.name.c_str());
      DGR_REQUIRE(!swapped || km->in_ptr, "layer %s: map has no in-major CSR", L.name.c_str());
    } else {
      DGR_REQUIRE(res == nullptr, "identity conv with residual not supported");
      a.pair_in = a.pair_out = a.tile_ptr = a.rule_ptr = nullptr;
      a.tile_desc = nullptr;
      a.n_rows_dev = cout_map.n_dev;
      a.tile_bound = dgr_ceil_div(cout_map.n_cap, DGR_TILE_M);
      a.l2_normalize = l2_next ? 1 : 0;
      l2_next = false;
    }
    hipEvent_t e0 = nullptr, em = nullptr, e1 = nullptr;
    if (prof) {
      e0 = ctx->events.next(); em = ctx->events.next(); e1 = ctx->events.next();
      if (!e0 || !em || !e1) return DGR_EHIP;
      DGR_HIP_CHECK(hipEventRecord(e0, stream));
    }
    if (km && ms.use_nbr) {
      const DgrNbrTable *t = nullptr;
      for (int l = 0; l < 4; ++l)
        if (km == &ms.same[l]) t = &ms.nsame[l];
      for (int l = 0; l < 3; ++l)
        if (km == &ms.down[l]) t = swapped ? &ms.nup[l] : &ms.ndown[l];
      DGR_REQUIRE(t && t->built && L.w16, "layer %s: no neighbour table / 16x16 weights", L.name.c_str());
      DgrConvOsLaunch o;
      o.in = in.ptr; o.in_ld = in.ld; o.in_relu = in.relu;
      o.out = out.ptr; o.out_ld = out.ld; o.out_relu = out.relu;
      o.rows_per_block = lvl_out <= 1 ? 64 : lvl_out == 2 ? (L.cin_pad >= 128 ? 64 : 32) : 16;
      o.phase_channels = (L.cin_pad >= 256 || (L.cin_pad == 128 && lvl_out >= 2)) ? 128 : 64;
      if (const char *e = getenv(lvl_out == 2 ? "DGR_OS_MB2" : lvl_out == 3 ? "DGR_OS_MB3" : "DGR_OS_MB01")) o.rows_per_block = atoi(e);
      if (const char *e = getenv("DGR_OS_CK")) o.phase_channels = atoi(e);
      o.w16 = L.w16; o.shift = L.shift;
      o.wb3 = L.w16b; o.piece_stride = L.w16b_piece;
      o.wbd = L.w16d;
      o.w_unscale = L.w_unscale; o.n_in_cap = cin_map.n_cap;
      if (L.w16b && !dgr_exact_f32()) {
        o.row_amax = in.amax;
        if (!o.row_amax) {
          uint32_t *mx;
          DGR_ALLOC(mx, ctx->arena, uint32_t, cin_map.n_cap);
          DGR_CHECK(dgr_row_amax(in.ptr, in.ld, L.cin, in.relu, cin_map.n_dev, cin_map.n_cap, mx, stream));
          o.row_amax = mx;
        }
      }
      o.out_amax = out.amax; o.out_amax2 = out.amax2;
      o.res = res ? res->ptr : nullptr; o.res_ld = res ? res->ld : 0; o.res_relu = res ? res->relu : 0;
      o.nbr = t; o.n_out_dev = cout_map.n_dev; o.n_out_cap = cout_map.n_cap;
      o.cin = L.cin; o.cin_pad = L.cin_pad; o.cout = L.cout;
      static const bool os_lists = getenv("DGR_OS_LISTS") != nullptr;
      bool same_stride = false;
      for (int l = 0; l < 4; ++l) same_stride = same_stride || t == &ms.nsame[l];
      o.dense = same_stride && o.row_amax && o.wbd && !os_lists && dgr_conv_dense_supported(L.cin, L.cin_pad, L.cout) &&
                cin_map.n_cap * (int64_t)in.ld * 4 < (1ll << 31);
      DGR_REQUIRE(o.dense || (!in.dsplit_only && !out.dsplit_only), "layer %s: dense split rows outside the dense-tile kernel", L.name.c_str());
      static const bool no_up = getenv("DGR_NO_UP") != nullptr;
      o.up = swapped && !o.dense && !no_up && !os_lists && o.row_amax && o.wbd && t->perm && res == nullptr &&
             dgr_conv_up_supported(L.cin, L.cin_pad, L.cout) && cin_map.n_cap * (int64_t)in.ld * 4 < (1ll << 31);
      if (o.dense) {
        o.in_dsplit = in.dsplit;
        o.out_dsplit = out.dsplit;
        if (out.dsplit_only) o.out = nullptr;
      }
      const char *kname = "sparse_conv_os";
      DGR_CHECK(dgr_conv_os_launch(o, stream, &kname));
      if (prof) {
        DGR_HIP_CHECK(hipEventRecord(e1, stream));
        ctx->conv_spans.push_back({e0, e1});
        ctx->gemm_spans.push_back({e0, e1});
        ctx->conv_kinds.push_back(kname);
      }
      LayerRun &r = net->runs[li];
      r = LayerRun();
      r.os = true;
      r.os_launch = o;
      r.nbr = *t;
      r.os_launch.nbr = &r.nbr;
      r.n_in = cin_map.n_dev; r.n_out = cout_map.n_dev; r.K = L.K;
      r.n_out_cap = cout_map.n_cap;
      return DGR_OK;
    }
    const bool small_cin = km && !swapped && !res && L.cin <= 8 && L.cout == 32 && L.cin_pad == 8;
    const char *kname = (L.cin == 6 && L.wq) ? "conv_cin6_quad_kernel" : L.cin == 1 ? "conv_small_cin_row_kernel" : "conv_small_cin_kernel";
    unsigned long long *clk = nullptr;
    const bool wide = L.wb && km;
    if (small_cin)
      DGR_CHECK(dgr_conv_small_cin(in.ptr, in.ld, in.relu, L.cin, L.w, L.wq, L.shift, *km, cout_map.n_dev, cout_map.n_cap,
                                   out.ptr, out.ld, stream));
    else if (wide) {
      DGR_REQUIRE(in.split.planes, "layer %s: the wide-layer kernel needs its input as split rows", L.name.c_str());
      if (prof) {
        DGR_ALLOC(a.clk, ctx->arena, unsigned long long, 2);
        DGR_HIP_CHECK(hipMemsetAsync(a.clk, 0xff, sizeof(unsigned long long), stream));
        DGR_HIP_CHECK(hipMemsetAsync(a.clk + 1, 0, sizeof(unsigned long long), stream));
        clk = a.clk;
      }
      DGR_CHECK(dgr_conv_wide_launch(a, in.split, L.wb, L.wb_piece, L.w_unscale, ctx->num_cus, stream, &kname));
    } else
      DGR_CHECK(dgr_conv_launch(a, ctx->num_cus, stream, &kname));
    if (prof) DGR_HIP_CHECK(hipEventRecord(em, stream));
    DGR_REQUIRE(!out.split.planes || (km && !small_cin), "layer %s: only a reduction can write split rows", L.name.c_str());
    if (km && !small_cin)
      DGR_CHECK(dgr_reduce_rows(ybuf, L.cout, swapped ? km->in_ptr : km->out_ptr, swapped ? km->in_pos : km->out_pos,
                                cout_map.n_dev, cout_map.n_cap, out.split_only ? nullptr : out.ptr, out.ld, L.shift, res ? res->ptr : nullptr,
                                res ? res->ld : 0, res ? res->relu : 0, stream, out.split.planes ? &out.split : nullptr,
                                out.relu));
    if (prof) {
      DGR_HIP_CHECK(hipEventRecord(e1, stream));
      ctx->conv_spans.push_back({e0, e1});
      ctx->gemm_spans.push_back({e0, em});
      ctx->conv_kinds.push_back(kname);
      ctx->conv_clks.resize(ctx->conv_spans.size(), nullptr);
      ctx->conv_clks.back() = clk;
    }
    LayerRun &r = net->runs[li];
    a.clk = nullptr;
    r.launch = a;
    r.split_in = wide ? in.split : DgrSplitRows();
    r.split_out = out.split;
    r.out_relu = out.relu;
    r.split_only = out.split_only;
    r.has_reduce = km != nullptr;
    r.small_cin = small_cin;
    if (km) r.km = *km;
    if (km) {
      r.red_ptr = swapped ? km->in_ptr : km->out_ptr;
      r.red_pos = swapped ? km->in_pos : km->out_pos;
    }
    r.n_out_cap = cout_map.n_cap;
    r.res = res ? res->ptr : nullptr; r.res_ld = res ? res->ld : 0; r.res_relu = res ? res->relu : 0;
    r.rule_ptr = km ? km->rule_ptr : nullptr;
    r.n_in = cin_map.n_dev; r.n_out = cout_map.n_dev; r.K = L.K;
    return DGR_OK;
  }
};

int dgr_resunet_forward_impl(dgr_ctx *ctx, dgr_net *net, const int32_t *coords, const float *feats,
                             int64_t N, float *out, hipStream_t stream) {
  DgrArena &A = ctx->arena;
  Fwd f;
  f.ctx = ctx; f.net = net; f.stream = stream; f.prof = ctx->profiling;
  hipEvent_t m0 = nullptr, m1 = nullptr;
  if (f.prof) {
    m0 = ctx->events.next(); m1 = ctx->events.next();
    DGR_HIP_CHECK(hipEventRecord(m0, stream));
  }
  f.ms.overflow = ctx->flag_dev;
  const bool use_nbr = net->D == 3 && net->cin <= 8 && net->conv1_ks <= 7;
  const bool conv1_fused = use_nbr;
  DGR_CHECK(dgr_build_maps(A, coords, N, net->D, net->conv1_ks, &f.ms, stream, conv1_fused, true, use_nbr));
  if (f.prof) {
    DGR_HIP_CHECK(hipEventRecord(m1, stream));
    (net->D == 3 ? ctx->map3_spans : ctx->map6_spans).push_back({m0, m1});
  }
  {
    const DgrMapSet &m = f.ms;
    int64_t need = m.use_nbr ? 64 : m.conv1.pair_cap * 32;
    const int64_t same_c[4] = {64, 64, 128, 256}, down_c[3] = {64, 128, 256};
    for (int l = 0; l < 4; ++l) need = std::max(need, m.same[l].pair_cap * same_c[l]);
    for (int l = 0; l < 3; ++l) need = std::max(need, m.down[l].pair_cap * down_c[l]);
    DGR_ALLOC(f.ybuf, A, float, need);
  }
  const DgrMapSet &ms = f.ms;
  const int64_t n1 = ms.cm[0].n_cap, n2 = ms.cm[1].n_cap, n4 = ms.cm[2].n_cap, n8 = ms.cm[3].n_cap;
  auto buf = [&](int64_t rows, int cols) -> float * { return A.get<float>((size_t)rows * cols); };
  float *t1 = buf(n1, 32), *y1 = buf(n1, 32), *cat1 = buf(n1, 96);
  float *t2 = buf(n2, 64), *y2 = buf(n2, 64), *cat2 = buf(n2, 128);
  float *t4 = buf(n4, 128), *y4 = buf(n4, 128), *cat4 = buf(n4, 256);
  float *t8 = buf(n8, 256), *y8 = buf(n8, 256), *s8 = buf(n8, 256);
  float *u4 = buf(n4, 128), *v4 = buf(n4, 128);
  float *u2 = buf(n2, 64), *v2 = buf(n2, 64);
  float *u1 = buf(n1, 64), *v1 = buf(n1, 64);
  float *h = buf(n1, 64);
  const bool fuse_l2 = net->normalize && net->cout <= 32;
  float *fin = (net->normalize && !fuse_l2) ? buf(n1, net->cout) : out;
  if (!t1 || !y1 || !cat1 || !t2 || !y2 || !cat2 || !t4 || !y4 || !cat4 || !t8 || !y8 || !s8 || !u4 ||
      !v4 || !u2 || !v2 || !u1 || !v1 || !h || !fin)
    return DGR_ENOMEM;

  const Tensor X{const_cast<float *>(feats), net->cin, 0};
  Tensor T1{t1, 32, 0}, Y1{y1, 32, 1}, S1{cat1 + 64, 96, 1};
  Tensor T2{t2, 64, 0}, Y2{y2, 64, 1};
  Tensor S2{cat2 + 64, 128, 1};
  Tensor T4{t4, 128, 0}, Y4{y4, 128, 1}, S4{cat4 + 128, 256, 1};
  Tensor T8{t8, 256, 0}, Y8{y8, 256, 1}, S8{s8, 256, 1};
  Tensor U4{u4, 128, 0}, V4{v4, 128, 1};
  Tensor U2{u2, 64, 0}, V2{v2, 64, 1};
  Tensor U1{u1, 64, 0}, V1{v1, 64, 1};
  Tensor S4T{cat4, 256, 1};
  {
    struct { Tensor *t; int consumer, channels; int64_t rows; bool middle; } sp[] = {
        {&T2, 4, 64, n2, false}, {&Y2, 5, 64, n2, true},
        {&S2, 6, 64, n2, false}, {&T4, 7, 128, n4, false}, {&Y4, 8, 128, n4, true}, {&S4, 9, 128, n4, false},
        {&T8, 10, 256, n8, false}, {&Y8, 11, 256, n8, true}, {&S8, 12, 256, n8, false}, {&U4, 13, 128, n4, false},
        {&V4, 14, 128, n4, true}, {&U2, 16, 64, n2, false}, {&V2, 17, 64, n2, true}, {&U1, 19, 64, n1, false},
        {&V1, 20, 64, n1, true}};
    for (auto &e : sp) {
      if (!net->W->layers[e.consumer].wb) continue;
      e.t->split.channels = e.channels;
      e.t->split_only = e.middle;
      DGR_ALLOC(e.t->split.planes, A, unsigned char, (size_t)e.rows * 4 * e.channels);
      DGR_ALLOC(e.t->split.scale, A, float, e.rows);
    }
  }
  Tensor S2T{cat2, 128, 1};
  const Tensor S1T{cat1, 96, 1};
  const Tensor H{h, 64, 1}, FIN{fin, net->cout, 0};
  Tensor CAT4{cat4, 256, 1}, CAT2{cat2, 128, 1};
  if (use_nbr) {
    const int64_t words = 5 * n1 + 6 * n2 + 6 * n4 + 3 * n8;
    uint32_t *pool;
    DGR_ALLOC(pool, A, uint32_t, words);
    DGR_HIP_CHECK(hipMemsetAsync(pool, 0, (size_t)words * sizeof(uint32_t), stream));
    auto take = [&](int64_t n) { uint32_t *p = pool; pool += n; return p; };
    for (Tensor *t : {&T1, &Y1, &S1, &U1, &V1}) t->amax = take(n1);
    for (Tensor *t : {&T2, &Y2, &S2, &CAT2, &U2, &V2}) t->amax = take(n2);
    for (Tensor *t : {&T4, &Y4, &S4, &CAT4, &U4, &V4}) t->amax = take(n4);
    for (Tensor *t : {&T8, &Y8, &S8}) t->amax = take(n8);
    S2.amax2 = CAT2.amax; S2T.amax2 = CAT2.amax;
    S4.amax2 = CAT4.amax; S4T.amax2 = CAT4.amax;
  }

  if (use_nbr && !getenv("DGR_NO_DSPLIT")) {
    static const bool os_lists = getenv("DGR_OS_LISTS") != nullptr;
    auto dense_layer = [&](int l, int64_t rows) {
      const DgrLayer &L = net->W->layers[l];
      return L.w16b && L.w16d && !dgr_exact_f32() && !os_lists && dgr_conv_dense_supported(L.cin, L.cin_pad, L.cout) &&
             rows * (int64_t)L.cin * 4 < (1ll << 31);
    };
    struct { Tensor *t; int producer; int64_t rows; } mid[] = {{&Y1, 1, n1}, {&Y2, 4, n2}, {&V2, 16, n2}, {&V1, 19, n1}};
    for (auto &e : mid)
      if (dense_layer(e.producer, e.rows) && dense_layer(e.producer + 1, e.rows) && e.t->ld == net->W->layers[e.producer].cout) {
        e.t->dsplit = reinterpret_cast<unsigned char *>(e.t->ptr);
        e.t->dsplit_only = true;
      }
  }

  int li = 0;
  if (conv1_fused) {
    const DgrLayer &L0 = net->W->layers[0];
    int32_t *pc;
    DGR_ALLOC(pc, A, int32_t, 1);
    hipEvent_t e0 = nullptr, e1 = nullptr;
    if (f.prof) {
      e0 = ctx->events.next(); e1 = ctx->events.next();
      DGR_HIP_CHECK(hipEventRecord(e0, stream));
    }
    const char *k1name = "conv1_grid_kernel";
    DGR_CHECK(dgr_conv1_probe(A, ms.cm[0], net->conv1_ks, feats, net->cin, net->cin, L0.w, L0.shift, t1, 32, pc, stream,
                              L0.wc, &k1name, T1.amax));
    if (f.prof) {
      DGR_HIP_CHECK(hipEventRecord(e1, stream));
      ctx->conv_spans.push_back({e0, e1});
      ctx->gemm_spans.push_back({e0, e1});
      ctx->conv_kinds.push_back(k1name);
    }
    LayerRun &r0 = net->runs[0];
    r0 = LayerRun();
    r0.n_in = r0.n_out = ms.cm[0].n_dev;
    r0.K = L0.K;
    r0.fused_pairs = pc;
    li++;
  } else {
    DGR_CHECK(f.conv(li++, X, &ms.conv1, false, 0, 0, T1, nullptr));
  }
  DGR_CHECK(f.conv(li++, T1, &ms.same[0], false, 0, 0, Y1, nullptr));
  DGR_CHECK(f.conv(li++, Y1, &ms.same[0], false, 0, 0, S1, &T1));
  DGR_CHECK(f.conv(li++, S1, &ms.down[0], false, 0, 1, T2, nullptr));
  DGR_CHECK(f.conv(li++, T2, &ms.same[1], false, 1, 1, Y2, nullptr));
  DGR_CHECK(f.conv(li++, Y2, &ms.same[1], false, 1, 1, S2, &T2));
  DGR_CHECK(f.conv(li++, S2, &ms.down[1], false, 1, 2, T4, nullptr));
  DGR_CHECK(f.conv(li++, T4, &ms.same[2], false, 2, 2, Y4, nullptr));
  DGR_CHECK(f.conv(li++, Y4, &ms.same[2], false, 2, 2, S4, &T4));
  DGR_CHECK(f.conv(li++, S4, &ms.down[2], false, 2, 3, T8, nullptr));
  DGR_CHECK(f.conv(li++, T8, &ms.same[3], false, 3, 3, Y8, nullptr));
  DGR_CHECK(f.conv(li++, Y8, &ms.same[3], false, 3, 3, S8, &T8));
  DGR_CHECK(f.conv(li++, S8, &ms.down[2], true, 3, 2, U4, nullptr));
  DGR_CHECK(f.conv(li++, U4, &ms.same[2], false, 2, 2, V4, nullptr));
  DGR_CHECK(f.conv(li++, V4, &ms.same[2], false, 2, 2, S4T, &U4));
  DGR_CHECK(f.conv(li++, CAT4, &ms.down[1], true, 2, 1, U2, nullptr));
  DGR_CHECK(f.conv(li++, U2, &ms.same[1], false, 1, 1, V2, nullptr));
  DGR_CHECK(f.conv(li++, V2, &ms.same[1], false, 1, 1, S2T, &U2));
  DGR_CHECK(f.conv(li++, CAT2, &ms.down[0], true, 1, 0, U1, nullptr));
  DGR_CHECK(f.conv(li++, U1, &ms.same[0], false, 0, 0, V1, nullptr));
  DGR_CHECK(f.conv(li++, V1, &ms.same[0], false, 0, 0, S1T, &U1));
  const Tensor CAT1{cat1, 96, 1};
  DGR_CHECK(f.conv(li++, CAT1, nullptr, false, 0, 0, H, nullptr));
  f.l2_next = fuse_l2;
  DGR_CHECK(f.conv(li++, H, nullptr, false, 0, 0, FIN, nullptr));
  if (net->normalize && !fuse_l2)
    DGR_CHECK(dgr_l2_normalize_rows(fin, net->cout, out, net->cout, net->cout, 0, ms.cm[0].n_dev, n1, stream));

  auto &I = net->inter;
  net->run_generation = ctx->arena.generation;
  I.clear();
  I["s1"] = {S1.ptr, 96, 32, ms.cm[0].n_dev};
  I["s2"] = {S2.ptr, 128, 64, ms.cm[1].n_dev, ms.cm[1].canon};
  I["s4"] = {S4.ptr, 256, 128, ms.cm[2].n_dev, ms.cm[2].canon};
  I["s8"] = {S8.ptr, 256, 256, ms.cm[3].n_dev, ms.cm[3].canon};
  I["s4_tr"] = {cat4, 256, 128, ms.cm[2].n_dev, ms.cm[2].canon};
  I["s2_tr"] = {cat2, 128, 64, ms.cm[1].n_dev, ms.cm[1].canon};
  I["s1_tr"] = {cat1, 96, 64, ms.cm[0].n_dev};

  return DGR_OK;
}

void dgr_ctx_begin_profile(dgr_ctx *ctx) {
  ctx->events.used = 0;
  ctx->conv_spans.clear();
  ctx->gemm_spans.clear();
  ctx->conv_kinds.clear();
  ctx->conv_clks.clear();
  ctx->map3_spans.clear();
  ctx->map6_spans.clear();
  ctx->conv_launches = 0;
}

int dgr_ctx_collect_profile(dgr_ctx *ctx) {
  auto total = [](const std::vector<std::pair<hipEvent_t, hipEvent_t>> &v, float *out) -> int {
    float s = 0.f, t = 0.f;
    for (auto &sp : v) {
      DGR_HIP_CHECK(hipEventElapsedTime(&t, sp.first, sp.second));
      s += t;
    }
    *out = s;
    return DGR_OK;
  };
  DGR_CHECK(total(ctx->map3_spans, &ctx->stage_ms[5]));
  DGR_CHECK(total(ctx->map6_spans, &ctx->stage_ms[6]));
  DGR_CHECK(total(ctx->conv_spans, &ctx->stage_ms[7]));
  ctx->conv_launches = (int64_t)ctx->conv_spans.size();
  ctx->conv_span_ms.clear();
  ctx->gemm_span_ms.clear();
  for (auto &sp : ctx->conv_spans) {
    float t = 0.f;
    DGR_HIP_CHECK(hipEventElapsedTime(&t, sp.first, sp.second));
    ctx->conv_span_ms.push_back(t);
  }
  for (auto &sp : ctx->gemm_spans) {
    float t = 0.f;
    DGR_HIP_CHECK(hipEventElapsedTime(&t, sp.first, sp.second));
    ctx->gemm_span_ms.push_back(t);
  }
  ctx->conv_clk_us.assign(ctx->conv_spans.size(), 0.f);
  for (size_t i = 0; i < ctx->conv_clks.size() && i < ctx->conv_clk_us.size(); ++i)
    if (ctx->conv_clks[i]) {
      unsigned long long c[2] = {0, 0};
      DGR_HIP_CHECK(hipMemcpy(c, ctx->conv_clks[i], sizeof(c), hipMemcpyDeviceToHost));
      if (c[1] > c[0]) ctx->conv_clk_us[i] = (float)((double)(c[1] - c[0]) * 0.01);
    }
  return DGR_OK;
}

int dgr_flag_error(int32_t flag) {
  if (flag == 1) {
    dgr_set_error("duplicate coordinates in the sparse tensor input");
    return DGR_EINVAL;
  }
  if (flag == 2) {
    dgr_set_error("kernel-map capacity exceeded (more than the reserved pairs per output row)");
    return DGR_ENOMEM;
  }
  return DGR_OK;
}

static int check_flag(dgr_ctx *ctx, const int32_t *flag_dev, hipStream_t stream) {
  unsigned char *pin;
  DGR_CHECK(dgr_ctx_pinned(ctx, 64, &pin));
  DGR_HIP_CHECK(hipMemcpyAsync(pin, flag_dev, sizeof(int32_t), hipMemcpyDeviceToHost, stream));
  DGR_CHECK(dgr_ctx_wait(ctx, stream));
  return dgr_flag_error(*reinterpret_cast<volatile int32_t *>(pin));
}

int dgr_ctx_new_flag(dgr_ctx *ctx, hipStream_t stream) {
  DGR_ALLOC(ctx->flag_dev, ctx->arena, int32_t, 1);
  DGR_HIP_CHECK(hipMemsetAsync(ctx->flag_dev, 0, sizeof(int32_t), stream));
  return DGR_OK;
}

int dgr_ctx_check_flag(dgr_ctx *ctx, hipStream_t stream) {
  if (!ctx->flag_dev) return DGR_OK;
  return check_flag(ctx, ctx->flag_dev, stream);
}

void dgr_net_invalidate_runs(dgr_net *net) { net->run_generation = ~0ull; }
int dgr_net_out_channels(const dgr_net *net) { return net->cout; }
int dgr_net_in_channels(const dgr_net *net) { return net->cin; }
int dgr_net_dim(const dgr_net *net) { return net->D; }
const dgr_ctx *dgr_net_ctx(const dgr_net *net) { return net->ctx; }

extern "C" int dgr_resunet_forward(dgr_ctx *ctx, dgr_net *net, const int32_t *coords, const float *feats,
                                   int64_t N, float *out, dgr_stream stream_) {
  DGR_REQUIRE(ctx && net && coords && feats && out, "dgr_resunet_forward: NULL argument");
  DGR_REQUIRE(net->ctx == ctx, "dgr_resunet_forward: the net object belongs to another context (one dgr_net per context: "
                               "dgr_net_share gives a second context its own over the same weights)");
  DGR_REQUIRE(N > 0, "dgr_resunet_forward: empty sparse tensor (N=%lld)", (long long)N);
  hipStream_t stream = (hipStream_t)stream_;
  DGR_HIP_CHECK(hipSetDevice(ctx->device));
  DGR_CHECK(ctx->arena.reset());
  DGR_CHECK(dgr_ctx_new_flag(ctx, stream));
  dgr_ctx_begin_profile(ctx);
  DGR_CHECK(dgr_resunet_forward_impl(ctx, net, coords, feats, N, out, stream));
  DGR_CHECK(dgr_ctx_check_flag(ctx, stream));
  if (ctx->profiling) {
    memset(ctx->stage_ms, 0, sizeof(ctx->stage_ms));
    DGR_CHECK(dgr_ctx_collect_profile(ctx));
  }
  return DGR_OK;
}

extern "C" int dgr_debug_conv_layer(dgr_ctx *ctx, dgr_net *net, int layer, const int32_t *coords, const float *in,
                                    int in_relu, int64_t N, float *out, dgr_stream stream_) {
  DGR_REQUIRE(ctx && net && coords && in && out && N > 0, "dgr_debug_conv_layer: bad argument");
  DGR_REQUIRE(layer >= 0 && layer < (int)net->W->layers.size(), "layer %d out of range", layer);
  const DgrLayer &L = net->W->layers[layer];
  int k3 = 1;
  for (int d = 0; d < net->D; ++d) k3 *= 3;
  DGR_REQUIRE(L.K == k3 && L.cin >= 32, "dgr_debug_conv_layer: layer %s is not a 3^D conv with >= 32 input channels", L.name.c_str());
  hipStream_t stream = (hipStream_t)stream_;
  DGR_HIP_CHECK(hipSetDevice(ctx->device));
  DGR_CHECK(ctx->arena.reset());
  DGR_CHECK(dgr_ctx_new_flag(ctx, stream));
  dgr_ctx_begin_profile(ctx);
  DgrArena &A = ctx->arena;
  Fwd f;
  f.ctx = ctx; f.net = net; f.stream = stream; f.prof = false;
  f.ms.overflow = ctx->flag_dev;
  DGR_CHECK(dgr_build_maps(A, coords, N, net->D, 3, &f.ms, stream, false, true, net->D == 3));
  const int64_t n_cap = f.ms.cm[0].n_cap;
  if (!f.ms.use_nbr) DGR_ALLOC(f.ybuf, A, float, f.ms.same[0].pair_cap * L.cout);
  Tensor tin{const_cast<float *>(in), L.cin, in_relu}, tout{out, L.cout, 0};
  if (L.wb) {
    tin.split.channels = L.cin;
    DGR_ALLOC(tin.split.planes, A, unsigned char, (size_t)n_cap * 4 * L.cin);
    DGR_ALLOC(tin.split.scale, A, float, n_cap);
    DGR_CHECK(dgr_split_rows(in, L.cin, in_relu, f.ms.cm[0].n_dev, n_cap, tin.split, stream));
  }
  DGR_CHECK(f.conv(layer, tin, &f.ms.same[0], false, 0, 0, tout, nullptr));
  DGR_CHECK(dgr_ctx_check_flag(ctx, stream));
  dgr_net_invalidate_runs(net);
  return DGR_OK;
}

extern "C" int dgr_net_get_intermediate(dgr_ctx *ctx, dgr_net *net, const char *name, float *host_out,
                                        int64_t capacity, int64_t *rows, int64_t *cols) {
  DGR_REQUIRE(ctx && net && name && rows && cols, "NULL argument");
  auto it = net->inter.find(name);
  DGR_REQUIRE(it != net->inter.end() && it->second.n_dev, "no intermediate named '%s' (run a forward first)", name);
  DGR_REQUIRE(net->run_generation == ctx->arena.generation,
              "the activations of the last forward are gone: a later call on this context reused its workspace");
  const DgrTensorRef &t = it->second;
  int32_t n = 0;
  DGR_HIP_CHECK(hipDeviceSynchronize());
  DGR_HIP_CHECK(hipMemcpy(&n, t.n_dev, sizeof(int32_t), hipMemcpyDeviceToHost));
  *rows = n;
  *cols = t.cols;
  if (host_out) {
    DGR_REQUIRE(capacity >= (int64_t)n * t.cols, "host buffer too small");
    if (!t.canon) {
      DGR_HIP_CHECK(hipMemcpy2D(host_out, (size_t)t.cols * sizeof(float), t.ptr, (size_t)t.ld * sizeof(float),
                                (size_t)t.cols * sizeof(float), (size_t)n, hipMemcpyDeviceToHost));
    } else {
      std::vector<float> tmp((size_t)n * t.cols);
      std::vector<int32_t> canon(n);
      DGR_HIP_CHECK(hipMemcpy2D(tmp.data(), (size_t)t.cols * sizeof(float), t.ptr, (size_t)t.ld * sizeof(float),
                                (size_t)t.cols * sizeof(float), (size_t)n, hipMemcpyDeviceToHost));
      DGR_HIP_CHECK(hipMemcpy(canon.data(), t.canon, (size_t)n * sizeof(int32_t), hipMemcpyDeviceToHost));
      for (int32_t p = 0; p < n; ++p)
        memcpy(host_out + (size_t)canon[p] * t.cols, tmp.data() + (size_t)p * t.cols, (size_t)t.cols * sizeof(float));
    }
    for (int64_t i = 0; i < (int64_t)n * t.cols; ++i) host_out[i] = host_out[i] > 0.f ? host_out[i] : 0.f;
  }
  return DGR_OK;
}

extern "C" int dgr_net_layer_stats(dgr_ctx *ctx, dgr_net *net, int layer, int64_t stats[8]) {
  DGR_REQUIRE(ctx && net && stats, "NULL argument");
  DGR_REQUIRE(layer >= 0 && layer < (int)net->W->layers.size(), "layer %d out of range", layer);
  const LayerRun &r = net->runs[layer];
  DGR_REQUIRE(r.n_in && r.n_out, "run a forward first");
  DGR_REQUIRE(net->run_generation == ctx->arena.generation,
              "the kernel maps of the last forward are gone: a later call on this context reused its workspace");
  const DgrLayer &L = net->W->layers[layer];
  DGR_HIP_CHECK(hipDeviceSynchronize());
  int32_t n_in = 0, n_out = 0;
  DGR_HIP_CHECK(hipMemcpy(&n_in, r.n_in, sizeof(int32_t), hipMemcpyDeviceToHost));
  DGR_HIP_CHECK(hipMemcpy(&n_out, r.n_out, sizeof(int32_t), hipMemcpyDeviceToHost));
  int64_t P = n_out, kne = 1;
  if (r.os) {
    int64_t counts[27];
    DGR_CHECK(dgr_nbr_counts(r.nbr, r.n_out, counts));
    P = 0;
    kne = 0;
    for (int k = 0; k < 27; ++k) { P += counts[k]; kne += counts[k] > 0; }
  } else if (r.fused_pairs) {
    int32_t pc = 0;
    DGR_HIP_CHECK(hipMemcpy(&pc, r.fused_pairs, sizeof(int32_t), hipMemcpyDeviceToHost));
    P = pc;
    kne = r.K;
  } else if (r.rule_ptr) {
    std::vector<int32_t> rp(r.K + 1);
    DGR_HIP_CHECK(hipMemcpy(rp.data(), r.rule_ptr, (size_t)(r.K + 1) * sizeof(int32_t), hipMemcpyDeviceToHost));
    P = rp[r.K];
    kne = 0;
    for (int k = 0; k < r.K; ++k) kne += rp[k + 1] > rp[k];
  }
  stats[0] = P; stats[1] = kne; stats[2] = n_in; stats[3] = n_out;
  stats[4] = L.cin; stats[5] = L.cout; stats[6] = L.K; stats[7] = 0;
  return DGR_OK;
}

extern "C" int dgr_net_rerun_layer(dgr_ctx *ctx, dgr_net *net, int layer, int reps, float *gemm_ms, float *reduce_ms) {
  DGR_REQUIRE(ctx && net && gemm_ms && reduce_ms && reps > 0, "bad argument");
  DGR_REQUIRE(layer >= 0 && layer < (int)net->W->layers.size(), "layer %d out of range", layer);
  const LayerRun &r = net->runs[layer];
  DGR_REQUIRE(r.n_in && r.n_out, "run a forward first");
  DGR_REQUIRE(net->run_generation == ctx->arena.generation,
              "the kernel maps of the last forward are gone: a later call on this context reused its workspace");
  DGR_REQUIRE(!r.fused_pairs, "layer %d ran fused with its neighbour search; not re-runnable", layer);
  const DgrLayer &L = net->W->layers[layer];
  hipEvent_t e0, e1, e2;
  DGR_HIP_CHECK(hipEventCreate(&e0)); DGR_HIP_CHECK(hipEventCreate(&e1)); DGR_HIP_CHECK(hipEventCreate(&e2));
  float tg = 0.f, tr = 0.f;
  for (int i = 0; i < reps + 1; ++i) {
    DGR_HIP_CHECK(hipEventRecord(e0, nullptr));
    if (r.os)
      DGR_CHECK(dgr_conv_os_launch(r.os_launch, nullptr));
    else if (r.small_cin)
      DGR_CHECK(dgr_conv_small_cin(r.launch.in, r.launch.in_ld, r.launch.in_relu, L.cin, L.w, L.wq, L.shift, r.km, r.n_out,
                                   r.n_out_cap, r.launch.out, r.launch.out_ld, nullptr));
    else if (L.wb && r.has_reduce)
      DGR_CHECK(dgr_conv_wide_launch(r.launch, r.split_in, L.wb, L.wb_piece, L.w_unscale, ctx->num_cus, nullptr));
    else
      DGR_CHECK(dgr_conv_launch(r.launch, ctx->num_cus, nullptr));
    DGR_HIP_CHECK(hipEventRecord(e1, nullptr));
    if (r.has_reduce && !r.small_cin && !r.os)
      DGR_CHECK(dgr_reduce_rows(r.launch.y, L.cout, r.red_ptr, r.red_pos, r.n_out, r.n_out_cap,
                                r.split_only ? nullptr : r.launch.out, r.launch.out_ld, L.shift, r.res, r.res_ld, r.res_relu, nullptr,
                                r.split_out.planes ? &r.split_out : nullptr, r.out_relu));
    DGR_HIP_CHECK(hipEventRecord(e2, nullptr));
    DGR_HIP_CHECK(hipEventSynchronize(e2));
    float a = 0.f, b = 0.f;
    DGR_HIP_CHECK(hipEventElapsedTime(&a, e0, e1));
    DGR_HIP_CHECK(hipEventElapsedTime(&b, e1, e2));
    if (i > 0) { tg += a; tr += b; }
  }
  (void)hipEventDestroy(e0); (void)hipEventDestroy(e1); (void)hipEventDestroy(e2);
  *gemm_ms = tg / reps;
  *reduce_ms = tr / reps;
  return DGR_OK;
}
```

Before: 392.8.

## Scatter wide-conv products into CSR slot order so reduction reads rows contiguously

For the 6-D inlier net's 64->64 layers, the kernel map now records each pair's CSR slot index. The wide conv epilogue writes each product row directly to that slot, and the row reduction then sums contiguous rows without the pos[] indirection (a new CONTIG template). This replaces gathered reads in the reduction with sequential ones and drops one index array. The cost is scattered stores in the conv epilogue, an extra LDS ring and slot loads, and an extra index array written during map building.

```diff
diff --git a/deepglobalregistration_amd/csrc/conv.hip b/deepglobalregistration_amd/csrc/conv.hip
--- a/deepglobalregistration_amd/csrc/conv.hip
+++ b/deepglobalregistration_amd/csrc/conv.hip
@@ -430,7 +430,7 @@
   return DGR_EINVAL;
 }
 
-template <int LPR, bool SPLIT>
+template <int LPR, bool SPLIT, bool CONTIG>
 __global__ void __launch_bounds__(256)
     reduce_rows_kernel(const float *__restrict__ y, int y_ld, const int32_t *__restrict__ ptr,
                        const int32_t *__restrict__ pos, const int32_t *n_dev, float *__restrict__ out, int out_ld,
@@ -448,10 +448,11 @@
     }
     int j = ptr[row];
     const int end = ptr[row + 1];
+    auto at = [&](int jj) -> int { return CONTIG ? jj : pos[jj]; };
     for (; j + 8 <= end; j += 8) {
       int p[8];
 #pragma unroll
-      for (int u = 0; u < 8; ++u) p[u] = pos[j + u];
+      for (int u = 0; u < 8; ++u) p[u] = at(j + u);
       f32x4 v[8];
 #pragma unroll
       for (int u = 0; u < 8; ++u) v[u] = dgr_y_load<LPR == 64>(y + (int64_t)p[u] * y_ld + c);
@@ -459,14 +460,14 @@
       for (int u = 0; u < 8; ++u) acc += v[u];
     }
     for (; j + 4 <= end; j += 4) {
-      const int p0 = pos[j], p1 = pos[j + 1], p2 = pos[j + 2], p3 = pos[j + 3];
+      const int p0 = at(j), p1 = at(j + 1), p2 = at(j + 2), p3 = at(j + 3);
       const f32x4 v0 = dgr_y_load<LPR == 64>(y + (int64_t)p0 * y_ld + c);
       const f32x4 v1 = dgr_y_load<LPR == 64>(y + (int64_t)p1 * y_ld + c);
       const f32x4 v2 = dgr_y_load<LPR == 64>(y + (int64_t)p2 * y_ld + c);
       const f32x4 v3 = dgr_y_load<LPR == 64>(y + (int64_t)p3 * y_ld + c);
       acc += v0; acc += v1; acc += v2; acc += v3;
     }
-    for (; j < end; ++j) acc += dgr_y_load<LPR == 64>(y + (int64_t)pos[j] * y_ld + c);
+    for (; j < end; ++j) acc += dgr_y_load<LPR == 64>(y + (int64_t)at(j) * y_ld + c);
     if (!SPLIT || out) *reinterpret_cast<f32x4 *>(out + row * out_ld + c) = acc;
     if constexpr (SPLIT) {
       const int lo = out_relu ? 0 : (int)0x80000000;
@@ -511,18 +512,23 @@
               "reduce_rows: split rows need planes, scales and the layer's width (a multiple of 64)");
   const int lpr = cout / 4;
   const int64_t want = std::max<int64_t>(1, dgr_ceil_div(n_cap, 256 / lpr));
-#define DGR_RR1(L, SP)                                                                                         \
+#define DGR_RR1(L, SP) \
+  do {                 \
+    if (pos) DGR_RR2(L, SP, false); \
+    else DGR_RR2(L, SP, true);      \
+  } while (0)
+#define DGR_RR2(L, SP, CT)                                                                                     \
   do {                                                                                                         \
     static int resident = 0;                                                                                   \
     if (resident == 0) {                                                                                       \
       int per_cu = 0, dev = 0, cus = 0;                                                                        \
-      DGR_HIP_CHECK(hipOccupancyMaxActiveBlocksPerMultiprocessor(&per_cu, reduce_rows_kernel<L, SP>, 256, 0)); \
+      DGR_HIP_CHECK(hipOccupancyMaxActiveBlocksPerMultiprocessor(&per_cu, reduce_rows_kernel<L, SP, CT>, 256, 0)); \
       DGR_HIP_CHECK(hipGetDevice(&dev));                                                                       \
       DGR_HIP_CHECK(hipDeviceGetAttribute(&cus, hipDeviceAttributeMultiprocessorCount, dev));                  \
       resident = (per_cu < 1 ? 1 : per_cu) * (cus < 1 ? 1 : cus);                                              \
     }                                                                                                          \
     const int64_t blocks = want > resident ? (int64_t)resident * std::min<int64_t>(4, want / resident) : want; \
-    reduce_rows_kernel<L, SP><<<(int)blocks, 256, 0, stream>>>(y, cout, ptr, pos, n_dev, out, out_ld, shift,   \
+    reduce_rows_kernel<L, SP, CT><<<(int)blocks, 256, 0, stream>>>(y, cout, ptr, pos, n_dev, out, out_ld, shift, \
                                                                res, res_ld, res_relu, split ? split->planes : nullptr, \
                                                                split ? split->scale : nullptr, out_relu);      \
   } while (0)
@@ -540,6 +546,7 @@
       dgr_set_error("reduce_rows: unsupported width %d", cout);
       return DGR_EINVAL;
   }
+#undef DGR_RR2
 #undef DGR_RR1
 #undef DGR_RR
   DGR_LAUNCH_CHECK();
@@ -682,6 +689,7 @@
                        const float *shift, const DgrKernelMap &km, const int32_t *n_out_dev, int64_t n_out_cap, float *out,
                        int out_ld, hipStream_t stream) {
   DGR_REQUIRE(cin >= 1 && cin <= 8, "small-Cin conv: cin=%d", cin);
+  DGR_REQUIRE(km.out_pos && km.pair_k, "small-Cin conv: the map has no slot -> position index or no pair offsets");
   if ((out_ld & 3) == 0 && cin == 6 && w_quad) {
     conv_cin6_quad_kernel<<<(int)dgr_ceil_div(n_out_cap * 4, 256), 256, 0, stream>>>(
         in, in_ld, in_relu, w_quad, shift, km.out_ptr, km.out_pos, km.pair_in, km.pair_k, n_out_dev, out, out_ld);
diff --git a/deepglobalregistration_amd/csrc/conv_wide.hip b/deepglobalregistration_amd/csrc/conv_wide.hip
--- a/deepglobalregistration_amd/csrc/conv_wide.hip
+++ b/deepglobalregistration_amd/csrc/conv_wide.hip
@@ -16,6 +16,8 @@
   const uint4 *wb;
   int64_t piece_stride;
   const int32_t *pair_in, *tile_ptr;
+  const int32_t *y_slot;
+  int64_t y_rows;
   int cout, K;
   float w_unscale;
   unsigned long long *clk;
@@ -42,8 +44,8 @@
   return b;
 }
 
-template <int CP, int NB, int WM>
-__global__ void __launch_bounds__(512, 1) sparse_conv_wide_f16x2(ConvWideArgs a, const int4 *__restrict__ tdesc) {
+template <int CP, int NB, int WM, bool SLOT>
+__device__ __forceinline__ void conv_wide_body(const ConvWideArgs &a, const int4 *__restrict__ tdesc) {
   constexpr int NCW = 4;
   constexpr int NP = 2, MB = 2 / WM, WN = NCW / WM, PW = 4, TM = 64, CK = 64, SK = CK / 16;
   static_assert(WM == 1 || WM == 2, "row split of the compute waves");
@@ -73,7 +75,8 @@
   constexpr int OFF_STAGE = NBUF * BUFB;
   constexpr int OFF_IDX = OFF_STAGE + NSTG * TM * LDS_ST * 4;
   constexpr int OFF_SC = OFF_IDX + RING * TM * 4;
-  constexpr int LDS_BYTES = OFF_SC + RING * TM * 4;
+  constexpr int OFF_SLOT = OFF_SC + RING * TM * 4;
+  constexpr int LDS_BYTES = OFF_SLOT + (SLOT ? RING * TM * 4 : 0);
   static_assert(LDS_BYTES <= 160 * 1024, "LDS budget");
   __shared__ __attribute__((aligned(16))) unsigned char lds[LDS_BYTES];
 
@@ -121,6 +124,11 @@
       };
       int *ring_i = reinterpret_cast<int *>(lds + OFF_IDX);
       float *ring_s = reinterpret_cast<float *>(lds + OFF_SC);
+      int *ring_p = reinterpret_cast<int *>(lds + OFF_SLOT);
+      auto load_slot = [&](int i) -> int {
+        const int4 d = desc(i);
+        return a.y_slot[d.y + min(lane, d.z - 1)];
+      };
       auto load_idx = [&](int i) -> int {
         const int4 d = desc(i);
         return a.pair_in[d.y + min(lane, d.z - 1)];
@@ -128,14 +136,21 @@
 #pragma unroll
       for (int i = 0; i < AH_I - 1; ++i) ring_i[i * TM + lane] = load_idx(i);
 #pragma unroll
-      for (int i = 0; i < AH_S - 1; ++i) ring_s[i * TM + lane] = a.row_scale[ring_i[i * TM + lane]];
+      for (int i = 0; i < AH_S - 1; ++i) {
+        ring_s[i * TM + lane] = a.row_scale[ring_i[i * TM + lane]];
+        if constexpr (SLOT) ring_p[i * TM + lane] = load_slot(i);
+      }
       int idx_reg = load_idx(AH_I - 1);
       float sc_reg = a.row_scale[ring_i[(AH_S - 1) * TM + lane]];
+      int slot_reg = 0;
+      if constexpr (SLOT) slot_reg = load_slot(AH_S - 1);
       auto rings = [&](int t) {
         ring_i[((t + AH_I - 1) & (RING - 1)) * TM + lane] = idx_reg;
         ring_s[((t + AH_S - 1) & (RING - 1)) * TM + lane] = sc_reg;
+        if constexpr (SLOT) ring_p[((t + AH_S - 1) & (RING - 1)) * TM + lane] = slot_reg;
         idx_reg = load_idx(t + AH_I);
         sc_reg = a.row_scale[ring_i[((t + AH_S) & (RING - 1)) * TM + lane]];
+        if constexpr (SLOT) slot_reg = load_slot(t + AH_S);
       };
       dgr_phase_barrier();
 #pragma unroll
@@ -162,6 +177,7 @@
       if (u < 0 || u >= n_my) return;
       const int4 d = desc(u);
       const float *sc = reinterpret_cast<const float *>(lds + OFF_SC + (u & (RING - 1)) * TM * 4);
+      const int *sl = reinterpret_cast<const int *>(lds + OFF_SLOT + (u & (RING - 1)) * TM * 4);
       const float *st = stage_of(u);
       const int c4 = (ptid % CPR) * 4;
       f32x4 v[NPS];
@@ -174,7 +190,9 @@
 #pragma unroll
       for (int i = 0; i < NPS; ++i) {
         const int r = r0 + i * RPP + ptid / CPR;
-        if (r < d.z) __builtin_nontemporal_store(v[i], reinterpret_cast<f32x4 *>(a.y + (int64_t)(d.y + r) * COUT + c4));
+        const int64_t slot = SLOT ? sl[r] : d.y + r;
+        if (r < d.z && (!SLOT || (uint64_t)slot < (uint64_t)a.y_rows))
+          __builtin_nontemporal_store(v[i], reinterpret_cast<f32x4 *>(a.y + slot * COUT + c4));
       }
     };
     dgr_phase_barrier();
@@ -297,15 +315,33 @@
 }
 
 template <int CP, int NB, int WM>
+__global__ void __launch_bounds__(512, 1) sparse_conv_wide_f16x2(ConvWideArgs a, const int4 *__restrict__ tdesc) {
+  conv_wide_body<CP, NB, WM, false>(a, tdesc);
+}
+template <int CP, int NB, int WM>
+__global__ void __launch_bounds__(512, 1) sparse_conv_wide_f16x2_csr(ConvWideArgs a, const int4 *__restrict__ tdesc) {
+  conv_wide_body<CP, NB, WM, true>(a, tdesc);
+}
+
+template <int CP, int NB, int WM>
 static int launch_wide(const ConvWideArgs &ka, const int4 *tile_desc, int64_t tile_bound, int num_cus, hipStream_t stream) {
   int64_t grid = num_cus;
   if (tile_bound < grid) grid = tile_bound;
   grid = (grid + 7) / 8 * 8;
   if (grid < 8) grid = 8;
+  if constexpr (CP == 64 && NB == 1 && WM == 2) {
+    if (ka.y_slot) {
+      sparse_conv_wide_f16x2_csr<CP, NB, WM><<<(int)grid, 512, 0, stream>>>(ka, tile_desc);
+      DGR_LAUNCH_CHECK();
+      return DGR_OK;
+    }
+  }
   sparse_conv_wide_f16x2<CP, NB, WM><<<(int)grid, 512, 0, stream>>>(ka, tile_desc);
   DGR_LAUNCH_CHECK();
   return DGR_OK;
 }
+
+bool dgr_conv_wide_csr_rows(int cin, int cout) { return cin == 64 && cout == 64; }
 
 bool dgr_conv_wide_supported(int cin_pad, int cin, int cout) {
   if (cin != cin_pad) return false;
@@ -322,6 +358,9 @@
   ConvWideArgs ka;
   ka.planes = in.planes; ka.row_scale = in.scale; ka.y = a.y;
   ka.wb = static_cast<const uint4 *>(wb); ka.piece_stride = piece_stride;
+  DGR_REQUIRE(!a.y_slot || (dgr_conv_wide_csr_rows(a.cin, a.cout) && a.y_rows > 0),
+              "wide conv: product rows in CSR order are built for the 64 -> 64 layers only (got %d -> %d)", a.cin, a.cout);
+  ka.y_slot = a.y_slot; ka.y_rows = a.y_rows;
   ka.pair_in = a.pair_in; ka.tile_ptr = a.tile_ptr; ka.cout = a.cout; ka.K = a.K; ka.w_unscale = w_unscale;
   ka.clk = a.clk;
   const int64_t tile_bound = a.tile_bound > 0 ? a.tile_bound : (int64_t)num_cus * 4;
@@ -330,7 +369,13 @@
     if (kernel_name) *kernel_name = "sparse_conv_wide_f16x2<" #CPV ", " #NBV ", " #WMV ">";     \
     return launch_wide<CPV, NBV, WMV>(ka, a.tile_desc, tile_bound, num_cus, stream);            \
   } while (0)
-  if (a.cout == 64 && a.cin == 64) DGR_WIDE(64, 1, 2);
+  if (a.cout == 64 && a.cin == 64) {
+    if (a.y_slot && kernel_name) {
+      *kernel_name = "sparse_conv_wide_f16x2_csr<64, 1, 2>";
+      kernel_name = nullptr;
+    }
+    DGR_WIDE(64, 1, 2);
+  }
   if (a.cout == 128 && a.cin == 64) DGR_WIDE(64, 1, 1);
   if (a.cout == 128 && a.cin == 128) DGR_WIDE(128, 1, 1);
   if (a.cout == 128 && a.cin == 256) DGR_WIDE(256, 1, 1);
diff --git a/deepglobalregistration_amd/csrc/dgr_internal.h b/deepglobalregistration_amd/csrc/dgr_internal.h
--- a/deepglobalregistration_amd/csrc/dgr_internal.h
+++ b/deepglobalregistration_amd/csrc/dgr_internal.h
@@ -104,6 +104,7 @@
   int32_t *out_ptr = nullptr, *out_pos = nullptr;
   uint16_t *pair_k = nullptr;
   int32_t *in_ptr = nullptr, *in_pos = nullptr;
+  int32_t *out_slot = nullptr, *in_slot = nullptr;
   int64_t pair_cap = 0;
   bool built = false;
 };
@@ -134,7 +135,7 @@
 
 int dgr_build_maps(DgrArena &arena, const int32_t *coords, int64_t N, int D, int conv1_ks,
                    DgrMapSet *ms, hipStream_t stream, bool skip_conv1_map = false, bool lean = false,
-                   bool nbr_tables = false);
+                   bool nbr_tables = false, bool slot_rows = false);
 int dgr_nbr_counts(const DgrNbrTable &t, const int32_t *n_out_dev, int64_t counts[27]);
 int dgr_conv1_probe(DgrArena &arena, const DgrCoordMap &cm, int ks, const float *in, int in_ld, int cin,
                     const float *w_tiled, const float *shift, float *out, int out_ld, int32_t *pair_count,
@@ -156,6 +157,8 @@
   float *out;
   int out_ld;
   float *y;
+  const int32_t *y_slot = nullptr;
+  int64_t y_rows = 0;
   const float *shift;
   const float *w;
   int cin, cin_pad, cout, cout_pad, K;
@@ -173,6 +176,7 @@
   int channels = 0;
 };
 bool dgr_conv_wide_supported(int cin_pad, int cin, int cout);
+bool dgr_conv_wide_csr_rows(int cin, int cout);
 int dgr_conv_wide_launch(const DgrConvLaunch &a, const DgrSplitRows &in, const void *wb, int64_t piece_stride,
                          float w_unscale, int num_cus, hipStream_t stream, const char **kernel_name = nullptr);
 int dgr_row_amax(const float *in, int in_ld, int cin, int relu, const int32_t *n_dev, int64_t n_cap, uint32_t *out,
diff --git a/deepglobalregistration_amd/csrc/kmap.hip b/deepglobalregistration_amd/csrc/kmap.hip
--- a/deepglobalregistration_amd/csrc/kmap.hip
+++ b/deepglobalregistration_amd/csrc/kmap.hip
@@ -303,6 +303,7 @@
   const int32_t *in_ptr;
   int32_t *in_pos;
   const unsigned short *wpre_out, *wpre_in;
+  int32_t *out_slot, *in_slot;
 };
 __device__ __forceinline__ void place_pair(const PlaceArgs &p, int k, int64_t o, int64_t in) {
   const int64_t slot = (int64_t)p.out_ptr[o] + mask_rank_pre(p.mask_out + o * p.KW, p.wpre_out + o * p.KW, k);
@@ -314,8 +315,13 @@
     p.pair_in[pos] = (int32_t)in;
     if (p.pair_out) p.pair_out[pos] = (int32_t)o;
     if (p.pair_k) p.pair_k[pos] = (uint16_t)k;
-    p.out_pos[slot] = (int32_t)pos;
-    if (p.mask_in) p.in_pos[p.in_ptr[in] + mask_rank_pre(p.mask_in + in * p.KW, p.wpre_in + in * p.KW, k)] = (int32_t)pos;
+    if (p.out_pos) p.out_pos[slot] = (int32_t)pos;
+    if (p.out_slot) p.out_slot[pos] = (int32_t)slot;
+    if (p.mask_in) {
+      const int64_t islot = (int64_t)p.in_ptr[in] + mask_rank_pre(p.mask_in + in * p.KW, p.wpre_in + in * p.KW, k);
+      if (p.in_pos) p.in_pos[islot] = (int32_t)pos;
+      if (p.in_slot) p.in_slot[pos] = (int32_t)islot;
+    }
   } else {
     *p.overflow = 2;
   }
@@ -447,8 +453,12 @@
   tile_desc_one(j.tile_ptr[m], j.rule_ptr[m], j.K[m], j.desc[m], j.tile_cap[m], t, DGR_TILE_M);
 }
 
+struct CsrIndex {
+  bool out_pos = true, out_slot = false, in_pos = true, in_slot = false;
+};
+
 static int alloc_kernel_map(DgrArena &arena, int K, int64_t n_cap, int64_t n_in_cap, int max_pairs_per_row, bool need_in_csr,
-                            bool want_pair_out, bool want_pair_k, DgrKernelMap *km) {
+                            bool want_pair_out, bool want_pair_k, DgrKernelMap *km, CsrIndex csr = CsrIndex()) {
   DGR_REQUIRE(K <= 1024, "kernel volume %d > 1024 not supported", K);
   km->K = K;
   const int64_t per_row = K < max_pairs_per_row ? K : max_pairs_per_row;
@@ -462,12 +472,15 @@
   km->tile_cap = km->pair_cap / DGR_TILE_M + K;
   DGR_ALLOC(km->tile_desc, arena, int4, km->tile_cap);
   DGR_ALLOC(km->out_ptr, arena, int32_t, n_cap + 1);
-  DGR_ALLOC(km->out_pos, arena, int32_t, km->pair_cap);
+  km->out_pos = km->out_slot = km->in_pos = km->in_slot = nullptr;
+  if (csr.out_pos) DGR_ALLOC(km->out_pos, arena, int32_t, km->pair_cap);
+  if (csr.out_slot) DGR_ALLOC(km->out_slot, arena, int32_t, km->pair_cap);
   km->pair_k = nullptr;
   if (want_pair_k) DGR_ALLOC(km->pair_k, arena, uint16_t, km->pair_cap);
   if (need_in_csr) {
     DGR_ALLOC(km->in_ptr, arena, int32_t, n_in_cap + 1);
-    DGR_ALLOC(km->in_pos, arena, int32_t, km->pair_cap);
+    if (csr.in_pos) DGR_ALLOC(km->in_pos, arena, int32_t, km->pair_cap);
+    if (csr.in_slot) DGR_ALLOC(km->in_slot, arena, int32_t, km->pair_cap);
   }
   return DGR_OK;
 }
@@ -535,6 +548,7 @@
   const DgrHalfBuckets *hb_out;
   bool need_in_csr, want_pair_out, want_pair_k;
   DgrKernelMap *km;
+  CsrIndex csr;
 };
 static int build_kernel_maps6(DgrArena &arena, const Kmap6Job *jobs, int nj, int max_pairs_per_row, int32_t *overflow,
                               hipStream_t stream) {
@@ -554,7 +568,7 @@
     t[m].n_cap = J.out->n_cap; t[m].n_in_cap = J.in->n_cap;
     DGR_REQUIRE(t[m].n_cap < (1ll << 27) && t[m].n_in_cap < (1ll << 27), "6-D kernel maps: more than 2^27 rows");
     DGR_CHECK(alloc_kernel_map(arena, K, t[m].n_cap, t[m].n_in_cap, max_pairs_per_row, J.need_in_csr, J.want_pair_out,
-                               J.want_pair_k, J.km));
+                               J.want_pair_k, J.km, J.csr));
   }
   DgrArena::Mark mk = arena.mark();
   {
@@ -655,7 +669,7 @@
       Tr &r = t[m];
       DgrKernelMap *km = J.km;
       pj.p[m] = PlaceArgs{K, KW, r.RB, r.mask_out, km->out_ptr, r.cell, r.base, km->pair_in, km->pair_out, km->pair_k, km->out_pos,
-                          km->pair_cap, overflow, r.mask_in, km->in_ptr, km->in_pos, r.wpre_out, r.wpre_in};
+                          km->pair_cap, overflow, r.mask_in, km->in_ptr, km->in_pos, r.wpre_out, r.wpre_in, km->out_slot, km->in_slot};
       pj.replay[m] = PrunedArgs{J.out->coords, J.out->n_dev, J.hb_out->second, r.n_cap, *J.hb, J.in->ts, r.symmetric};
       pj.h[m] = r.hl;
       pj.n_waves[m] = (int)r.hit_waves;
@@ -835,7 +849,7 @@
 int dgr_build_half_buckets(DgrArena &arena, DgrCoordMap *cm, DgrHalfBuckets *hb, int levels, int renumber_from, hipStream_t stream);
 
 int dgr_build_maps(DgrArena &arena, const int32_t *coords, int64_t N, int D, int conv1_ks,
-                   DgrMapSet *ms, hipStream_t stream, bool skip_conv1_map, bool lean, bool nbr_tables) {
+                   DgrMapSet *ms, hipStream_t stream, bool skip_conv1_map, bool lean, bool nbr_tables, bool slot_rows) {
   DGR_REQUIRE(D == 3 || D == 6, "D=%d not supported (the DGR path uses D=3 and D=6)", D);
   DGR_REQUIRE(conv1_ks % 2 == 1 && conv1_ks >= 1, "conv1 kernel size must be odd");
   DGR_REQUIRE(N > 0 && N < (1ll << 30), "N=%lld out of range", (long long)N);
@@ -888,6 +902,10 @@
     Kmap6Job jobs[7];
     for (int l = 0; l < 4; ++l) jobs[l] = {&ms->cm[l], &ms->cm[l], &ms->hb[l], &ms->hb[l], false, !lean, !lean || l == 0, &ms->same[l]};
     for (int l = 0; l < 3; ++l) jobs[4 + l] = {&ms->cm[l], &ms->cm[l + 1], &ms->hb[l], &ms->hb[l + 1], true, true, !lean, &ms->down[l]};
+    if (lean && slot_rows) {
+      jobs[0].csr.out_slot = true;
+      jobs[1].csr.out_slot = true; jobs[1].csr.out_pos = false;
+    }
     DGR_CHECK(build_kernel_maps6(arena, jobs, 7, cap_row, ms->overflow, stream));
     ms->conv1 = ms->same[0];
     return DGR_OK;
diff --git a/deepglobalregistration_amd/csrc/net.hip b/deepglobalregistration_amd/csrc/net.hip
--- a/deepglobalregistration_amd/csrc/net.hip
+++ b/deepglobalregistration_amd/csrc/net.hip
@@ -459,6 +459,7 @@
       a.tile_ptr = km->tile_ptr; a.rule_ptr = km->rule_ptr; a.tile_desc = km->tile_desc;
       a.n_rows_dev = nullptr;
       a.tile_bound = km->pair_cap / DGR_TILE_M + km->K;
+      a.y_rows = km->pair_cap;
       DGR_REQUIRE(km->K == L.K, "layer %s: kernel volume mismatch", L.name.c_str());
       DGR_REQUIRE(!swapped || km->in_ptr, "layer %s: map has no in-major CSR", L.name.c_str());
     } else {
@@ -543,6 +544,11 @@
     const char *kname = (L.cin == 6 && L.wq) ? "conv_cin6_quad_kernel" : L.cin == 1 ? "conv_small_cin_row_kernel" : "conv_small_cin_kernel";
     unsigned long long *clk = nullptr;
     const bool wide = L.wb && km;
+    const int32_t *y_slot = (wide && !small_cin && dgr_conv_wide_csr_rows(L.cin, L.cout)) ? (swapped ? km->in_slot : km->out_slot) : nullptr;
+    const int32_t *red_pos = (km && !y_slot) ? (swapped ? km->in_pos : km->out_pos) : nullptr;
+    DGR_REQUIRE(!km || small_cin || y_slot || red_pos, "layer %s: its kernel map carries neither index of this CSR direction",
+                L.name.c_str());
+    a.y_slot = y_slot;
     if (small_cin)
       DGR_CHECK(dgr_conv_small_cin(in.ptr, in.ld, in.relu, L.cin, L.w, L.wq, L.shift, *km, cout_map.n_dev, cout_map.n_cap,
                                    out.ptr, out.ld, stream));
@@ -560,7 +566,7 @@
     if (prof) DGR_HIP_CHECK(hipEventRecord(em, stream));
     DGR_REQUIRE(!out.split.planes || (km && !small_cin), "layer %s: only a reduction can write split rows", L.name.c_str());
     if (km && !small_cin)
-      DGR_CHECK(dgr_reduce_rows(ybuf, L.cout, swapped ? km->in_ptr : km->out_ptr, swapped ? km->in_pos : km->out_pos,
+      DGR_CHECK(dgr_reduce_rows(ybuf, L.cout, swapped ? km->in_ptr : km->out_ptr, red_pos,
                                 cout_map.n_dev, cout_map.n_cap, out.split_only ? nullptr : out.ptr, out.ld, L.shift, res ? res->ptr : nullptr,
                                 res ? res->ld : 0, res ? res->relu : 0, stream, out.split.planes ? &out.split : nullptr,
                                 out.relu));
@@ -584,7 +590,7 @@
     if (km) r.km = *km;
     if (km) {
       r.red_ptr = swapped ? km->in_ptr : km->out_ptr;
-      r.red_pos = swapped ? km->in_pos : km->out_pos;
+      r.red_pos = red_pos;
     }
     r.n_out_cap = cout_map.n_cap;
     r.res = res ? res->ptr : nullptr; r.res_ld = res ? res->ld : 0; r.res_relu = res ? res->relu : 0;
@@ -607,7 +613,9 @@
   f.ms.overflow = ctx->flag_dev;
   const bool use_nbr = net->D == 3 && net->cin <= 8 && net->conv1_ks <= 7;
   const bool conv1_fused = use_nbr;
-  DGR_CHECK(dgr_build_maps(A, coords, N, net->D, net->conv1_ks, &f.ms, stream, conv1_fused, true, use_nbr));
+  static const bool rule_major_rows = getenv("DGR_RULE_MAJOR_ROWS") != nullptr;
+  const bool slot_rows = net->D == 6 && !dgr_exact_f32() && !rule_major_rows;
+  DGR_CHECK(dgr_build_maps(A, coords, N, net->D, net->conv1_ks, &f.ms, stream, conv1_fused, true, use_nbr, slot_rows));
   if (f.prof) {
     DGR_HIP_CHECK(hipEventRecord(m1, stream));
     (net->D == 3 ? ctx->map3_spans : ctx->map6_spans).push_back({m0, m1});
@@ -965,7 +973,8 @@
     for (int k = 0; k < r.K; ++k) kne += rp[k + 1] > rp[k];
   }
   stats[0] = P; stats[1] = kne; stats[2] = n_in; stats[3] = n_out;
-  stats[4] = L.cin; stats[5] = L.cout; stats[6] = L.K; stats[7] = 0;
+  stats[4] = L.cin; stats[5] = L.cout; stats[6] = L.K;
+  stats[7] = (r.has_reduce && !r.small_cin && !r.os && r.launch.y_slot) ? 1 : 0;
   return DGR_OK;
 }
 
```

Result: no change. 391.1 (-0.4%).
